# syzhang092218-source/dgppo

Hardware: AMD Instinct MI355X
Metric: env-steps/sec whole node, LidarSpread n=8 4096 envs, 1/2/4/8 GPUs (higher is better)
Workload: dtype f32

## Files before the change

dgppo_amd/csrc/nn_graph.hip:

```cpp
#include "common.h"

struct Topo {
  int n, ng, gs, os, per, lidar, spread;
  int S, Ns;
};

static Topo make_topo(const dgppo_env_cfg& c) {
  Topo t;
  t.n = c.n_agents; t.ng = c.n_goals; t.gs = cfg_goal_slots(c); t.os = cfg_obs_slots(c);
  t.lidar = cfg_is_lidar(c) ? 1 : 0; t.spread = cfg_is_spread(c) ? 1 : 0;
  t.per = t.os;
  t.S = t.n + t.gs + t.os;
  t.Ns = t.n + t.ng + cfg_obs_nodes(c);
  return t;
}

__device__ inline int sender_node(const Topo& t, int i, int s) {
  if (s < t.n) return s;
  if (s < t.n + t.gs) return t.spread ? t.n + (s - t.n) : t.n + i;
  const int m = s - t.n - t.gs;
  return t.lidar ? t.n + t.ng + i * t.per + m : t.n + t.ng + m;
}
__device__ inline int slot_of(const Topo& t, int nd, int i) {
  if (nd < t.n) return nd;
  if (nd < t.n + t.ng) {
    const int g = nd - t.n;
    return t.spread ? t.n + g : (g == i ? t.n : -1);
  }
  const int q = nd - t.n - t.ng;
  if (t.lidar) return (q / t.per == i) ? t.n + t.gs + (q - i * t.per) : -1;
  return t.n + t.gs + q;
}

struct FeatArgs {
  dgppo_env_cfg cfg;
  Topo t;
  const float* agent; long agent_se, agent_st;
  const float* goal;
  const float* obst;
  const float* hits; long hits_se, hits_st;
  const int32_t* env_ids;
  int n_env, n_time;
  float* Xa;
  float* Xo;
  float* efeat;
  float* emask;
  int Fp;
  uint32_t rcp_fp, rcp_S;
};

__device__ inline float dist_rn(float dx, float dy) { return __fsqrt_rn(__fadd_rn(__fmul_rn(dx, dx), __fmul_rn(dy, dy))); }

template <int SD>
__global__ void graph_feats_kernel(FeatArgs a) {
  extern __shared__ float sm[];
  const dgppo_env_cfg& c = a.cfg;
  const Topo& t = a.t;
  const int g = blockIdx.x;
  const int e = g / a.n_time, tt = g - e * a.n_time;
  const int env = a.env_ids ? a.env_ids[e] : e;
  const int tid = threadIdx.x, nt = blockDim.x;
  const int n = t.n, ng = t.ng, S = t.S, Fp = a.Fp;
  const int n_on = t.Ns - n - ng;
  float* s_ag = sm;
  float* s_go = s_ag + n * SD;
  float* s_ob = s_go + ng * SD;
  float* s_fa = s_ob + n_on * SD;
  float* s_fg = s_fa + n * 4;
  const float* ag = a.agent + (size_t)env * a.agent_se + (size_t)tt * a.agent_st;
  for (int i = tid; i < n * SD; i += nt) s_ag[i] = ag[i];
  for (int i = tid; i < ng * SD; i += nt) s_go[i] = a.goal[(size_t)env * ng * SD + i];
  if (n_on > 0) {
    if (t.lidar) {
      const float* hp = a.hits + (size_t)env * a.hits_se + (size_t)tt * a.hits_st;
      for (int i = tid; i < n_on * 2; i += nt) {
        const int q = i >> 1, d = i & 1;
        s_ob[q * SD + d] = hp[i];
      }
      for (int i = tid; i < n_on * (SD - 2); i += nt) {
        const int q = i / (SD - 2), d = i - q * (SD - 2);
        s_ob[q * SD + 2 + d] = 0.0f;
      }
    } else {
      for (int i = tid; i < n_on * SD; i += nt) s_ob[i] = a.obst[(size_t)env * n_on * SD + i];
    }
  }
  __syncthreads();
  for (int i = tid; i < n + ng; i += nt) {
    const float* s = (i < n) ? s_ag + i * SD : s_go + (i - n) * SD;
    float* f = (i < n) ? s_fa + i * 4 : s_fg + (i - n) * 4;
    if constexpr (SD == 5) {
      f[0] = s[0]; f[1] = s[1]; f[2] = __fmul_rn(s[4], s[2]); f[3] = __fmul_rn(s[4], s[3]);
    } else {
      f[0] = s[0]; f[1] = s[1]; f[2] = s[2]; f[3] = s[3];
    }
  }
  __syncthreads();
  constexpr int ND = SD + 3;
  for (int idx = tid; idx < t.Ns * Fp; idx += nt) {
    const int nd = (int)__umulhi((uint32_t)idx, a.rcp_fp), col = idx - nd * Fp;
    float v = 0.0f;
    if (nd < n) v = (col < SD) ? s_ag[nd * SD + col] : ((col == SD + 2) ? 1.0f : 0.0f);
    else if (nd < n + ng) v = (col < SD) ? s_go[(nd - n) * SD + col] : ((col == SD + 1) ? 1.0f : 0.0f);
    else v = (col < SD) ? s_ob[(nd - n - ng) * SD + col] : ((col == SD) ? 1.0f : 0.0f);
    if (col >= ND) v = 0.0f;
    if (nd < n) a.Xa[((size_t)g * n + nd) * Fp + col] = v;
    else a.Xo[((size_t)g * (t.Ns - n) + (nd - n)) * Fp + col] = v;
  }
  for (int idx = tid; idx < n * S; idx += nt) {
    const int i = (int)__umulhi((uint32_t)idx, a.rcp_S), s = idx - i * S;
    float4 f;
    bool mask;
    const float* fi = s_fa + i * 4;
    const float px = s_ag[i * SD], py = s_ag[i * SD + 1];
    if (s < n) {
      const float* fj = s_fa + s * 4;
      f = make_float4(__fsub_rn(fi[0], fj[0]), __fsub_rn(fi[1], fj[1]), __fsub_rn(fi[2], fj[2]), __fsub_rn(fi[3], fj[3]));
      float d = __fadd_rn(dist_rn(__fsub_rn(px, s_ag[s * SD]), __fsub_rn(py, s_ag[s * SD + 1])), (i == s) ? c.eye_offset : 0.0f);
      mask = d < c.comm_radius;
    } else if (s < n + t.gs) {
      const int gi = t.spread ? (s - n) : i;
      const float* fg = s_fg + gi * 4;
      f = make_float4(__fsub_rn(fi[0], fg[0]), __fsub_rn(fi[1], fg[1]), __fsub_rn(fi[2], fg[2]), __fsub_rn(fi[3], fg[3]));
      mask = true;
    } else {
      const int m = s - n - t.gs;
      if (t.lidar) {
        const float* hp = s_ob + (i * t.per + m) * SD;
        const float lx = __fsub_rn(px, hp[0]), ly = __fsub_rn(py, hp[1]);
        f = make_float4(lx, ly, 0.0f, 0.0f);
        mask = dist_rn(lx, ly) < c.lidar_mask_radius;
      } else {
        const float* xo = s_ob + m * SD;
        const float* xi = s_ag + i * SD;
        f = make_float4(__fsub_rn(xi[0], xo[0]), __fsub_rn(xi[1], xo[1]), __fsub_rn(xi[2], xo[2]), __fsub_rn(xi[3], xo[3]));
        mask = dist_rn(__fsub_rn(xi[0], xo[0]), __fsub_rn(xi[1], xo[1])) < c.obs_mask_radius;
      }
    }
    reinterpret_cast<float4*>(a.efeat)[(size_t)g * n * S + idx] = f;
    a.emask[(size_t)g * n * S + idx] = mask ? 1.0f : 0.0f;
  }
}

extern "C" int32_t dgppo_graph_feats(const dgppo_env_cfg* cfg, const float* agent, int64_t agent_se, int64_t agent_st,
                                     const float* goal, const float* obst, const float* hits, int64_t hits_se,
                                     int64_t hits_st, const int32_t* env_ids, int32_t n_env, int32_t n_time, float* Xa,
                                     float* Xo, float* efeat, float* emask, int32_t Fp, void* stream) {
  int32_t rc = dgppo_validate_cfg(cfg);
  if (rc) return rc;
  DGPPO_REQUIRE(n_env >= 0 && n_time >= 0, "graph_feats: negative counts");
  if (n_env == 0 || n_time == 0) return 0;
  DGPPO_REQUIRE(agent && goal && Xa && efeat && emask, "graph_feats: NULL operand");
  DGPPO_REQUIRE(Fp >= cfg->node_dim && Fp <= 32, "graph_feats: Fp must be in [node_dim, 32]");
  FeatArgs a;
  a.cfg = *cfg; a.t = make_topo(*cfg);
  const int n_on = a.t.Ns - a.t.n - a.t.ng;
  DGPPO_REQUIRE(n_on == 0 || Xo, "graph_feats: Xo is NULL");
  DGPPO_REQUIRE(a.t.Ns == a.t.n || Xo, "graph_feats: Xo is NULL");
  if (n_on > 0) {
    if (a.t.lidar) DGPPO_REQUIRE(hits, "graph_feats: hits is NULL");
    else DGPPO_REQUIRE(obst, "graph_feats: obst is NULL");
  }
  DGPPO_REQUIRE(((uintptr_t)efeat & 15) == 0, "graph_feats: efeat must be 16-byte aligned");
  a.agent = agent; a.agent_se = agent_se; a.agent_st = agent_st; a.goal = goal; a.obst = obst;
  a.hits = hits; a.hits_se = hits_se; a.hits_st = hits_st; a.env_ids = env_ids; a.n_env = n_env; a.n_time = n_time;
  a.Xa = Xa; a.Xo = Xo; a.efeat = efeat; a.emask = emask; a.Fp = Fp;
  a.rcp_fp = (uint32_t)((0x100000000ull + (uint64_t)Fp - 1) / (uint64_t)Fp);
  a.rcp_S = (uint32_t)((0x100000000ull + (uint64_t)a.t.S - 1) / (uint64_t)a.t.S);
  DGPPO_REQUIRE(Fp >= 2 && a.t.S >= 2 && (long)a.t.Ns * Fp < 65536 && (long)a.t.n * a.t.S < 65536, "graph_feats: sizes out of range");
  const int SD = cfg->state_dim;
  const size_t smem = sizeof(float) * ((size_t)a.t.n * SD + a.t.ng * SD + (size_t)n_on * SD + a.t.n * 4 + a.t.ng * 4);
  const long G = (long)n_env * n_time;
  if (SD == 5) hipLaunchKernelGGL(graph_feats_kernel<5>, dim3(G), dim3(128), smem, (hipStream_t)stream, a);
  else hipLaunchKernelGGL(graph_feats_kernel<4>, dim3(G), dim3(128), smem, (hipStream_t)stream, a);
  DGPPO_LAUNCH_CHECK();
  return 0;
}

struct AttnArgs {
  Topo t;
  int F, H, Kp;
  const float* qt;
  const float* Xa;
  const float* Xo;
  const float* efeat;
  const float* emask;
  float* zcat;
  float* attn;
  const float* dzcat;
  float* dqt;
  float* dXa;
  float* dXo;
  int relu_xo;
  int G;
  const float* Xo_raw; const float* Wo; const float* bo; int ldwo;
  float* dwo_slab;
};

__global__ void __launch_bounds__(256) attn_fwd_valu_kernel(AttnArgs a) {
  extern __shared__ float sm[];
  const Topo& t = a.t;
  const int g = blockIdx.x, tid = threadIdx.x, nt = blockDim.x;
  const int n = t.n, S = t.S, Ns = t.Ns, F = a.F, H = a.H, Fl = F + 1;
  float* s_x = sm;
  float* s_q = s_x + Ns * Fl;
  float* s_e = s_q + n * H * Fl;
  float* s_m = s_e + n * S * 4;
  float* s_a = s_m + n * S;
  for (int idx = tid; idx < Ns * F; idx += nt) {
    const int nd = idx / F, f = idx - nd * F;
    s_x[nd * Fl + f] = (nd < n) ? a.Xa[((size_t)g * n + nd) * F + f] : a.Xo[((size_t)g * (Ns - n) + (nd - n)) * F + f];
  }
  for (int idx = tid; idx < n * H * F; idx += nt) {
    const int ih = idx / F, f = idx - ih * F;
    s_q[ih * Fl + f] = a.qt[(size_t)g * n * H * F + idx];
  }
  for (int idx = tid; idx < n * S * 4; idx += nt) s_e[idx] = a.efeat[(size_t)g * n * S * 4 + idx];
  for (int idx = tid; idx < n * S; idx += nt) s_m[idx] = a.emask[(size_t)g * n * S + idx];
  __syncthreads();
  for (int idx = tid; idx < n * S * H; idx += nt) {
    const int h = idx % H, is = idx / H;
    const int i = is / S, s = is - i * S;
    const float* x = s_x + sender_node(t, i, s) * Fl;
    const float* q = s_q + (i * H + h) * Fl;
    float acc = 0.0f;
    for (int f = 0; f < F; ++f) acc = fmaf(q[f], x[f], acc);
    s_a[idx] = acc;
  }
  __syncthreads();
  for (int ih = tid; ih < n * H; ih += nt) {
    const int i = ih / H, h = ih - i * H;
    float mx = -INFINITY;
    for (int s = 0; s < S; ++s)
      if (s_m[i * S + s] != 0.0f) mx = fmaxf(mx, s_a[(i * S + s) * H + h]);
    float den = 0.0f;
    for (int s = 0; s < S; ++s) {
      float ev = 0.0f;
      if (s_m[i * S + s] != 0.0f) ev = expf(s_a[(i * S + s) * H + h] - mx);
      s_a[(i * S + s) * H + h] = ev;
      den += ev;
    }
    const float inv = (den > 0.0f) ? 1.0f / den : 0.0f;
    for (int s = 0; s < S; ++s) s_a[(i * S + s) * H + h] *= inv;
  }
  __syncthreads();
  if (a.attn != nullptr)
    for (int idx = tid; idx < n * S * H; idx += nt) a.attn[(size_t)g * n * S * H + idx] = s_a[idx];
  const int W = F + 4;
  for (int idx = tid; idx < n * H * W; idx += nt) {
    const int w = idx % W, ih = idx / W;
    const int i = ih / H, h = ih - i * H;
    float acc = 0.0f;
    if (w < F) {
      for (int s = 0; s < S; ++s) {
        const float av = s_a[(i * S + s) * H + h];
        if (av != 0.0f) acc = fmaf(av, s_x[sender_node(t, i, s) * Fl + w], acc);
      }
    } else {
      for (int s = 0; s < S; ++s) {
        const float av = s_a[(i * S + s) * H + h];
        if (av != 0.0f) acc = fmaf(av, s_e[(i * S + s) * 4 + (w - F)], acc);
      }
    }
    a.zcat[((size_t)g * n + i) * a.Kp + F + h * W + w] = acc;
  }
  for (int idx = tid; idx < n * F; idx += nt) {
    const int i = idx / F, f = idx - i * F;
    a.zcat[((size_t)g * n + i) * a.Kp + f] = s_x[i * Fl + f];
  }
  const int kc = F + H * W;
  for (int idx = tid; idx < n * (a.Kp - kc); idx += nt) {
    const int i = idx / (a.Kp - kc), c = kc + idx - i * (a.Kp - kc);
    a.zcat[((size_t)g * n + i) * a.Kp + c] = (c == kc) ? 1.0f : 0.0f;
  }
}

__global__ void __launch_bounds__(256) attn_bwd_valu_kernel(AttnArgs a) {
  extern __shared__ float sm[];
  const Topo& t = a.t;
  const int g = blockIdx.x, tid = threadIdx.x, nt = blockDim.x;
  const int n = t.n, S = t.S, Ns = t.Ns, F = a.F, H = a.H, Fl = F + 1, W = F + 4;
  float* s_x = sm;
  float* s_q = s_x + Ns * Fl;
  float* s_e = s_q + n * H * Fl;
  float* s_a = s_e + n * S * 4;
  float* s_d = s_a + n * S * H;
  float* s_z = s_d + n * S * H;
  const int Wl = W + 1;
  for (int idx = tid; idx < Ns * F; idx += nt) {
    const int nd = idx / F, f = idx - nd * F;
    s_x[nd * Fl + f] = (nd < n) ? a.Xa[((size_t)g * n + nd) * F + f] : a.Xo[((size_t)g * (Ns - n) + (nd - n)) * F + f];
  }
  for (int idx = tid; idx < n * H * F; idx += nt) {
    const int ih = idx / F, f = idx - ih * F;
    s_q[ih * Fl + f] = a.qt[(size_t)g * n * H * F + idx];
  }
  for (int idx = tid; idx < n * S * 4; idx += nt) s_e[idx] = a.efeat[(size_t)g * n * S * 4 + idx];
  for (int idx = tid; idx < n * S * H; idx += nt) s_a[idx] = a.attn[(size_t)g * n * S * H + idx];
  for (int idx = tid; idx < n * H * W; idx += nt) {
    const int w = idx % W, ih = idx / W;
    const int i = ih / H, h = ih - i * H;
    s_z[ih * Wl + w] = a.dzcat[((size_t)g * n + i) * a.Kp + F + h * W + w];
  }
  __syncthreads();
  for (int idx = tid; idx < n * S * H; idx += nt) {
    const int h = idx % H, is = idx / H;
    const int i = is / S, s = is - i * S;
    float acc = 0.0f;
    if (s_a[idx] != 0.0f) {
      const float* x = s_x + sender_node(t, i, s) * Fl;
      const float* dz = s_z + (i * H + h) * Wl;
      for (int f = 0; f < F; ++f) acc = fmaf(dz[f], x[f], acc);
      for (int c = 0; c < 4; ++c) acc = fmaf(dz[F + c], s_e[is * 4 + c], acc);
    }
    s_d[idx] = acc;
  }
  __syncthreads();
  for (int ih = tid; ih < n * H; ih += nt) {
    const int i = ih / H, h = ih - i * H;
    float dot = 0.0f;
    for (int s = 0; s < S; ++s) dot = fmaf(s_a[(i * S + s) * H + h], s_d[(i * S + s) * H + h], dot);
    for (int s = 0; s < S; ++s) {
      const int k = (i * S + s) * H + h;
      s_d[k] = s_a[k] * (s_d[k] - dot);
    }
  }
  __syncthreads();
  for (int idx = tid; idx < n * H * F; idx += nt) {
    const int f = idx % F, ih = idx / F;
    const int i = ih / H, h = ih - i * H;
    float acc = 0.0f;
    for (int s = 0; s < S; ++s) {
      const float dv = s_d[(i * S + s) * H + h];
      if (dv != 0.0f) acc = fmaf(dv, s_x[sender_node(t, i, s) * Fl + f], acc);
    }
    a.dqt[(size_t)g * n * H * F + idx] = acc;
  }
  if (a.dXa != nullptr) {
    for (int idx = tid; idx < Ns * F; idx += nt) {
      const int nd = idx / F, f = idx - nd * F;
      if (nd >= n && a.dXo == nullptr) continue;
      float acc = 0.0f;
      for (int i = 0; i < n; ++i) {
        const int s = slot_of(t, nd, i);
        if (s < 0) continue;
        for (int h = 0; h < H; ++h) {
          const int k = (i * S + s) * H + h;
          acc = fmaf(s_a[k], s_z[(i * H + h) * Wl + f], acc);
          acc = fmaf(s_d[k], s_q[(i * H + h) * Fl + f], acc);
        }
      }
      if (nd < n) a.dXa[((size_t)g * n + nd) * F + f] = acc + a.dzcat[((size_t)g * n + nd) * a.Kp + f];
      else a.dXo[((size_t)g * (Ns - n) + (nd - n)) * F + f] = acc;
    }
  }
}


using f32x4g = __attribute__((ext_vector_type(4))) float;
#ifdef DGPPO_STAMPS
__device__ unsigned long long g_astamps[32];
#define ASTAMP(i) do { if (blockIdx.x == 0 && threadIdx.x == 0) g_astamps[i] = __builtin_amdgcn_s_memtime(); } while (0)
extern "C" int32_t dgppo_debug_stamps_attn(unsigned long long* out) {
  return (int32_t)hipMemcpyFromSymbol(out, HIP_SYMBOL(g_astamps), sizeof(unsigned long long) * 32);
}
#else
#define ASTAMP(i)
#endif

struct AttnDims {
  int n, H, F, S, Ns, nH, RT, CT, Fl, Ll, W;
};
__host__ __device__ inline AttnDims attn_dims(const Topo& t, int F, int H) {
  AttnDims d;
  d.n = t.n; d.H = H; d.F = F; d.S = t.S; d.Ns = t.Ns; d.nH = t.n * H;
  d.RT = (d.nH + 15) / 16; d.CT = (d.Ns + 15) / 16;
  d.Fl = F + 1; d.Ll = d.CT * 16 + 1; d.W = (t.S > 32) ? 64 : 32;
  return d;
}
static size_t attn_mfma_smem(const AttnDims& d, bool bwd) {
  size_t fl = (size_t)d.CT * 16 * d.Fl
              + (size_t)d.RT * 16 * d.Fl
              + (size_t)d.RT * 16 * d.Ll
              + 8 + (size_t)d.n * d.S * 5
              + 2 * (size_t)d.nH * ((d.S + 3) & ~3);
  if (bwd) fl += (size_t)d.RT * 16 * d.Ll
                 + (size_t)d.RT * 16 * (d.F + 5);
  return fl * sizeof(float);
}

__device__ inline float red_max(float v, int W) {
  for (int o = W >> 1; o >= 1; o >>= 1) v = fmaxf(v, __shfl_xor(v, o, W));
  return v;
}
__device__ inline float red_sum(float v, int W) {
  for (int o = W >> 1; o >= 1; o >>= 1) v += __shfl_xor(v, o, W);
  return v;
}

template <typename FA, typename FB, typename FC>
__device__ inline void mfma_tiles(int RTn, int CTn, int K4, int wave, int lane, FA fa, FB fb, FC fc) {
  const int li = lane & 15, lq = lane >> 4;
  for (int tile = wave; tile < RTn * CTn; tile += 4) {
    const int rt = tile / CTn, ct = tile - rt * CTn;
    f32x4g acc = {0.f, 0.f, 0.f, 0.f};
    int k4 = 0;
    for (; k4 + 4 <= K4; k4 += 4) {
      float av[4], bv[4];
#pragma unroll
      for (int u = 0; u < 4; ++u) { av[u] = fa(rt * 16 + li, (k4 + u) * 4 + lq); bv[u] = fb((k4 + u) * 4 + lq, ct * 16 + li); }
#pragma unroll
      for (int u = 0; u < 4; ++u) acc = __builtin_amdgcn_mfma_f32_16x16x4f32(av[u], bv[u], acc, 0, 0, 0);
    }
    for (; k4 < K4; ++k4) acc = __builtin_amdgcn_mfma_f32_16x16x4f32(fa(rt * 16 + li, k4 * 4 + lq), fb(k4 * 4 + lq, ct * 16 + li), acc, 0, 0, 0);
#pragma unroll
    for (int r = 0; r < 4; ++r) fc(rt * 16 + lq * 4 + r, ct * 16 + li, acc[r]);
  }
}


template <int MAXIT, typename FL, typename FP>
__device__ inline void stage4(int count4, int tid, FL load, FP put) {
  float4 v[MAXIT];
#pragma unroll
  for (int it = 0; it < MAXIT; ++it) {
    const int idx = tid + it * 256;
    v[it] = (idx < count4) ? load(idx) : make_float4(0.f, 0.f, 0.f, 0.f);
  }
#pragma unroll
  for (int it = 0; it < MAXIT; ++it) {
    const int idx = tid + it * 256;
    if (idx < count4) put(idx, v[it]);
  }
  for (int idx = tid + MAXIT * 256; idx < count4; idx += 256) put(idx, load(idx));
}
__device__ inline void put4(float* d, float4 v) { d[0] = v.x; d[1] = v.y; d[2] = v.z; d[3] = v.w; }

#define ATT_SMAX 64

__global__ void __launch_bounds__(256) attn_fwd_kernel(AttnArgs a) {
  extern __shared__ float sm[];
  const Topo& t = a.t;
  const AttnDims d = attn_dims(t, a.F, a.H);
  const int g = blockIdx.x, tid = threadIdx.x, lane = tid & 63, wave = tid >> 6;
  const int n = d.n, S = d.S, Ns = d.Ns, F = d.F, H = d.H, Fl = d.Fl, Ll = d.Ll, nH = d.nH;
  const int Sp = (S + 3) & ~3;
  float* s_x = sm;
  float* s_q = s_x + d.CT * 16 * Fl;
  float* s_L = s_q + d.RT * 16 * Fl;
  float* s_e = sm + (((d.CT * 16 * Fl + d.RT * 16 * Fl + d.RT * 16 * Ll) + 3) & ~3);
  float* s_m = s_e + n * S * 4;
  float* s_a = s_m + n * S;
  ASTAMP(0);
  {
    const int F4 = F >> 2;
    const float4* xa = reinterpret_cast<const float4*>(a.Xa + (size_t)g * n * F);
    const float4* xo = reinterpret_cast<const float4*>(a.Xo + (size_t)g * (Ns - n) * F);
    const float4* q4 = reinterpret_cast<const float4*>(a.qt + (size_t)g * nH * F);
    const float4* e4 = reinterpret_cast<const float4*>(a.efeat + (size_t)g * n * S * 4);
    const float* mk = a.emask + (size_t)g * n * S;
    const int nA = n * F4, nX = Ns * F4, nXp = d.CT * 16 * F4, nQ = nH * F4, nQp = d.RT * 16 * F4, nE = n * S;
    float4 vx[4], vq[2], ve[2];
    float vm[2];
    const float4 z4 = make_float4(0.f, 0.f, 0.f, 0.f);
#pragma unroll
    for (int it = 0; it < 4; ++it) { const int idx = tid + it * 256; vx[it] = (idx < nA) ? xa[idx] : ((idx < nX) ? xo[idx - nA] : z4); }
#pragma unroll
    for (int it = 0; it < 2; ++it) { const int idx = tid + it * 256; vq[it] = (idx < nQ) ? q4[idx] : z4; ve[it] = (idx < nE) ? e4[idx] : z4; vm[it] = (idx < nE) ? mk[idx] : 0.0f; }
#pragma unroll
    for (int it = 0; it < 4; ++it) { const int idx = tid + it * 256; if (idx < nXp) { const int nd = idx / F4, q = idx - nd * F4; put4(s_x + nd * Fl + 4 * q, vx[it]); } }
#pragma unroll
    for (int it = 0; it < 2; ++it) {
      const int idx = tid + it * 256;
      if (idx < nQp) { const int row = idx / F4, q = idx - row * F4; put4(s_q + row * Fl + 4 * q, vq[it]); }
      if (idx < nE) { const float4 ev = ve[it]; reinterpret_cast<float4*>(s_e)[idx] = make_float4(ev.x, ev.y, ev.z, ev.w); s_m[idx] = vm[it]; }
    }
    for (int idx = tid + 1024; idx < nXp; idx += 256) { const int nd = idx / F4, q = idx - nd * F4; put4(s_x + nd * Fl + 4 * q, (idx < nA) ? xa[idx] : ((idx < nX) ? xo[idx - nA] : z4)); }
    for (int idx = tid + 512; idx < nQp; idx += 256) { const int row = idx / F4, q = idx - row * F4; put4(s_q + row * Fl + 4 * q, (idx < nQ) ? q4[idx] : z4); }
    for (int idx = tid + 512; idx < nE; idx += 256) { reinterpret_cast<float4*>(s_e)[idx] = e4[idx]; s_m[idx] = mk[idx]; }
  }
  __syncthreads();
  ASTAMP(1);
  mfma_tiles(d.RT, d.CT, F / 4, wave, lane,
             [&](int row, int k) { return s_q[row * Fl + k]; },
             [&](int k, int col) { return s_x[col * Fl + k]; },
             [&](int row, int col, float v) { s_L[row * Ll + col] = v; });
  __syncthreads();
  ASTAMP(2);
  for (int idx = tid; idx < nH * Sp; idx += 256) {
    const int pair = idx / Sp, s = idx - pair * Sp, i = pair / H;
    float l = -INFINITY;
    if (s < S && s_m[i * S + s] != 0.0f) l = s_L[pair * Ll + sender_node(t, i, s)];
    s_a[idx] = l;
  }
  __syncthreads();
  ASTAMP(3);
  const int Wd = F + 4;
  float* zc = a.zcat + (size_t)g * n * a.Kp;
  for (int p0 = 0; p0 < nH; p0 += 32) {
    const int pair = p0 + (tid >> 3), sub = tid & 7;
    const bool live = pair < nH;
    const int i = live ? pair / H : 0, h = live ? pair - (pair / H) * H : 0;
    float l[ATT_SMAX / 8];
    float mx = -INFINITY;
#pragma unroll
    for (int j = 0; j < ATT_SMAX / 8; ++j) {
      const int sl = sub + 8 * j;
      l[j] = (live && sl < S) ? s_a[pair * Sp + sl] : -INFINITY;
      mx = fmaxf(mx, l[j]);
    }
    mx = fmaxf(mx, __shfl_xor(mx, 1, 8)); mx = fmaxf(mx, __shfl_xor(mx, 2, 8)); mx = fmaxf(mx, __shfl_xor(mx, 4, 8));
    float den = 0.0f;
#pragma unroll
    for (int j = 0; j < ATT_SMAX / 8; ++j) {
      if (sub + 8 * j < S) { const float ev = (l[j] == -INFINITY) ? 0.0f : expf(l[j] - mx); l[j] = ev; den += ev; }
    }
    den += __shfl_xor(den, 1, 8); den += __shfl_xor(den, 2, 8); den += __shfl_xor(den, 4, 8);
    const float inv = (den > 0.0f) ? 1.0f / den : 0.0f;
    float z0 = 0.f, z1 = 0.f, z2 = 0.f, z3 = 0.f;
#pragma unroll
    for (int j = 0; j < ATT_SMAX / 8; ++j) {
      const int sl = sub + 8 * j;
      if (live && sl < S) {
        const float av = l[j] * inv;
        s_a[pair * Sp + sl] = av;
        if (av != 0.0f) {
          const float4 e = reinterpret_cast<const float4*>(s_e)[i * S + sl];
          z0 = fmaf(av, e.x, z0); z1 = fmaf(av, e.y, z1); z2 = fmaf(av, e.z, z2); z3 = fmaf(av, e.w, z3);
        }
      }
    }
#pragma unroll
    for (int o = 1; o < 8; o <<= 1) { z0 += __shfl_xor(z0, o, 8); z1 += __shfl_xor(z1, o, 8); z2 += __shfl_xor(z2, o, 8); z3 += __shfl_xor(z3, o, 8); }
    if (live && sub == 0) *reinterpret_cast<float4*>(zc + i * a.Kp + F + h * Wd + F) = make_float4(z0, z1, z2, z3);
  }
  for (int idx = tid; idx < d.RT * 16 * Ll; idx += 256) s_L[idx] = 0.0f;
  __syncthreads();
  ASTAMP(4);
  for (int idx = tid; idx < n * S * H; idx += 256) {
    const int h = idx % H, is = idx / H, i = is / S, s = is - i * S;
    const float av = s_a[(i * H + h) * Sp + s];
    if (a.attn != nullptr) a.attn[(size_t)g * n * S * H + idx] = av;
    if (av != 0.0f) s_L[(i * H + h) * Ll + sender_node(t, i, s)] = av;
  }
  __syncthreads();
  ASTAMP(5);
  mfma_tiles(d.RT, (F + 15) / 16, d.CT * 4, wave, lane,
             [&](int row, int k) { return s_L[row * Ll + k]; },
             [&](int k, int col) { return (col < F) ? s_x[k * Fl + col] : 0.0f; },
             [&](int row, int col, float v) {
               if (row < nH && col < F) { const int i = row / H, h = row - i * H; zc[i * a.Kp + F + h * Wd + col] = v; }
             });
  for (int idx = tid; idx < n * F; idx += 256) {
    const int i = idx / F, f = idx - i * F;
    zc[i * a.Kp + f] = s_x[i * Fl + f];
  }
  const int kc = F + H * Wd;
  for (int idx = tid; idx < n * (a.Kp - kc); idx += 256) {
    const int i = idx / (a.Kp - kc), c = kc + idx - i * (a.Kp - kc);
    zc[i * a.Kp + c] = (c == kc) ? 1.0f : 0.0f;
  }
  ASTAMP(6);
}

template <int CTRL> __device__ inline float dpp_f(float v) {
  return __int_as_float(__builtin_amdgcn_update_dpp(0, __float_as_int(v), CTRL, 0xf, 0xf, false));
}
__device__ inline float grp8_sum(float v) {
  v += dpp_f<0xB1>(v);
  v += dpp_f<0x4E>(v);
  v += dpp_f<0x141>(v);
  return v;
}
__device__ inline float grp8_max(float v) {
  v = fmaxf(v, dpp_f<0xB1>(v));
  v = fmaxf(v, dpp_f<0x4E>(v));
  v = fmaxf(v, dpp_f<0x141>(v));
  return v;
}

template <int H, int NPA, int SJ>
__global__ void __launch_bounds__(256) attn_fwd_slot8_kernel(AttnArgs a) {
  constexpr int F = 8, Wd = F + 4;
  const Topo& t = a.t;
  const int lane = threadIdx.x & 63, wave = threadIdx.x >> 6, sub = lane & 7, grp = lane >> 3;
  const int g = __builtin_amdgcn_readfirstlane(blockIdx.x * 4 + wave);
  if (g >= a.G) return;
  const int n = t.n, S = t.S, Ns = t.Ns, Kp = a.Kp, kc = F + H * Wd;
  const float* Xa = a.Xa + (size_t)g * n * F;
  const float* Xo = a.Xo + (size_t)g * (Ns - n) * F - (size_t)n * F;
  const float* qt = a.qt + (size_t)g * n * H * F;
  const float* ef = a.efeat + (size_t)g * n * S * 4;
  const float* mk = a.emask + (size_t)g * n * S;
  float* zc = a.zcat + (size_t)g * n * Kp;
  float* at = a.attn + (size_t)g * n * S * H;
  for (int idx = lane; idx < n * 2; idx += 64)
    *reinterpret_cast<float4*>(zc + (idx >> 1) * Kp + 4 * (idx & 1)) = reinterpret_cast<const float4*>(Xa)[idx];
  for (int i = lane; i < n; i += 64)
    for (int c = kc; c < Kp; ++c) zc[i * Kp + c] = (c == kc) ? 1.0f : 0.0f;
#pragma unroll
  for (int p = 0; p < NPA; ++p) {
    const int ia = grp + 8 * p;
    const bool live = ia < n;
    const int i = live ? ia : n - 1;
    float4 q[H][2], x[SJ][2], e[SJ];
    float m[SJ];
#pragma unroll
    for (int h = 0; h < H; ++h) {
      const float4* qp = reinterpret_cast<const float4*>(qt + (i * H + h) * F);
      q[h][0] = qp[0]; q[h][1] = qp[1];
    }
#pragma unroll
    for (int j = 0; j < SJ; ++j) {
      int sl = sub + 8 * j;
      sl = sl < S ? sl : S - 1;
      const int nd = sender_node(t, i, sl);
      const float4* xp = reinterpret_cast<const float4*>((nd < n ? Xa : Xo) + (size_t)nd * F);
      x[j][0] = xp[0]; x[j][1] = xp[1];
      e[j] = reinterpret_cast<const float4*>(ef)[i * S + sl];
      m[j] = mk[i * S + sl];
    }
    float av[SJ][H];
#pragma unroll
    for (int h = 0; h < H; ++h) {
      float mx = -INFINITY;
#pragma unroll
      for (int j = 0; j < SJ; ++j) {
        const bool ok = live && (sub + 8 * j) < S && m[j] != 0.0f;
        float acc = q[h][0].x * x[j][0].x;
        acc = fmaf(q[h][0].y, x[j][0].y, acc); acc = fmaf(q[h][0].z, x[j][0].z, acc); acc = fmaf(q[h][0].w, x[j][0].w, acc);
        acc = fmaf(q[h][1].x, x[j][1].x, acc); acc = fmaf(q[h][1].y, x[j][1].y, acc);
        acc = fmaf(q[h][1].z, x[j][1].z, acc); acc = fmaf(q[h][1].w, x[j][1].w, acc);
        av[j][h] = ok ? acc : -INFINITY;
        mx = fmaxf(mx, av[j][h]);
      }
      mx = grp8_max(mx);
      float den = 0.0f;
#pragma unroll
      for (int j = 0; j < SJ; ++j) {
        const float ev = (av[j][h] == -INFINITY) ? 0.0f : __expf(av[j][h] - mx);
        av[j][h] = ev;
        den += ev;
      }
      den = grp8_sum(den);
      const float inv = (den > 0.0f) ? 1.0f / den : 0.0f;
#pragma unroll
      for (int j = 0; j < SJ; ++j) av[j][h] *= inv;
    }
#pragma unroll
    for (int j = 0; j < SJ; ++j) {
      const int sl = sub + 8 * j;
      if (live && sl < S) {
#pragma unroll
        for (int h = 0; h < H; ++h) if (a.attn != nullptr) at[(i * S + sl) * H + h] = av[j][h];
      }
    }
#pragma unroll
    for (int h = 0; h < H; ++h) {
      float z[Wd];
#pragma unroll
      for (int c = 0; c < Wd; ++c) z[c] = 0.0f;
#pragma unroll
      for (int j = 0; j < SJ; ++j) {
        const float w = av[j][h];
        if (w != 0.0f) {
          z[0] = fmaf(w, x[j][0].x, z[0]); z[1] = fmaf(w, x[j][0].y, z[1]); z[2] = fmaf(w, x[j][0].z, z[2]); z[3] = fmaf(w, x[j][0].w, z[3]);
          z[4] = fmaf(w, x[j][1].x, z[4]); z[5] = fmaf(w, x[j][1].y, z[5]); z[6] = fmaf(w, x[j][1].z, z[6]); z[7] = fmaf(w, x[j][1].w, z[7]);
          z[8] = fmaf(w, e[j].x, z[8]); z[9] = fmaf(w, e[j].y, z[9]); z[10] = fmaf(w, e[j].z, z[10]); z[11] = fmaf(w, e[j].w, z[11]);
        }
      }
#pragma unroll
      for (int c = 0; c < Wd; ++c) z[c] = grp8_sum(z[c]);
      if (live && sub == h) {
        float4* o = reinterpret_cast<float4*>(zc + i * Kp + F + h * Wd);
        o[0] = make_float4(z[0], z[1], z[2], z[3]);
        o[1] = make_float4(z[4], z[5], z[6], z[7]);
        o[2] = make_float4(z[8], z[9], z[10], z[11]);
      }
    }
  }
}

template <int H, int NPA, int SJ>
__global__ void __launch_bounds__(256) attn_bwd_slot8_kernel(AttnArgs a) {
  constexpr int F = 8, Wd = F + 4;
  const Topo& t = a.t;
  const int lane = threadIdx.x & 63, wave = threadIdx.x >> 6, sub = lane & 7, grp = lane >> 3;
  const int g = __builtin_amdgcn_readfirstlane(blockIdx.x * 4 + wave);
  if (g >= a.G) return;
  const int n = t.n, S = t.S, Ns = t.Ns, Kp = a.Kp;
  const float* Xa = a.Xa + (size_t)g * n * F;
  const float* Xo = a.Xo + (size_t)g * (Ns - n) * F - (size_t)n * F;
  const float* ef = a.efeat + (size_t)g * n * S * 4;
  const float* at = a.attn + (size_t)g * n * S * H;
  const float* dzc = a.dzcat + (size_t)g * n * Kp;
  float* dq = a.dqt + (size_t)g * n * H * F;
#pragma unroll
  for (int p = 0; p < NPA; ++p) {
    const int ia = grp + 8 * p;
    const bool live = ia < n;
    const int i = live ? ia : n - 1;
    float4 dz[H][3], x[SJ][2], e[SJ];
    float av[SJ][H];
#pragma unroll
    for (int h = 0; h < H; ++h) {
      const float4* zp = reinterpret_cast<const float4*>(dzc + i * Kp + F + h * Wd);
      dz[h][0] = zp[0]; dz[h][1] = zp[1]; dz[h][2] = zp[2];
    }
#pragma unroll
    for (int j = 0; j < SJ; ++j) {
      int sl = sub + 8 * j;
      const bool in = live && sl < S;
      sl = sl < S ? sl : S - 1;
      const int nd = sender_node(t, i, sl);
      const float4* xp = reinterpret_cast<const float4*>((nd < n ? Xa : Xo) + (size_t)nd * F);
      x[j][0] = xp[0]; x[j][1] = xp[1];
      e[j] = reinterpret_cast<const float4*>(ef)[i * S + sl];
#pragma unroll
      for (int h = 0; h < H; ++h) {
        const float w = at[(i * S + sl) * H + h];
        av[j][h] = in ? w : 0.0f;
      }
    }
#pragma unroll
    for (int h = 0; h < H; ++h) {
      float dA[SJ];
      float dot = 0.0f;
#pragma unroll
      for (int j = 0; j < SJ; ++j) {
        float acc = 0.0f;
        if (av[j][h] != 0.0f) {
          acc = dz[h][0].x * x[j][0].x;
          acc = fmaf(dz[h][0].y, x[j][0].y, acc); acc = fmaf(dz[h][0].z, x[j][0].z, acc); acc = fmaf(dz[h][0].w, x[j][0].w, acc);
          acc = fmaf(dz[h][1].x, x[j][1].x, acc); acc = fmaf(dz[h][1].y, x[j][1].y, acc);
          acc = fmaf(dz[h][1].z, x[j][1].z, acc); acc = fmaf(dz[h][1].w, x[j][1].w, acc);
          acc = fmaf(dz[h][2].x, e[j].x, acc); acc = fmaf(dz[h][2].y, e[j].y, acc);
          acc = fmaf(dz[h][2].z, e[j].z, acc); acc = fmaf(dz[h][2].w, e[j].w, acc);
          dot = fmaf(av[j][h], acc, dot);
        }
        dA[j] = acc;
      }
      dot = grp8_sum(dot);
      float o[F];
#pragma unroll
      for (int c = 0; c < F; ++c) o[c] = 0.0f;
#pragma unroll
      for (int j = 0; j < SJ; ++j) {
        if (av[j][h] != 0.0f) {
          const float dl = av[j][h] * (dA[j] - dot);
          o[0] = fmaf(dl, x[j][0].x, o[0]); o[1] = fmaf(dl, x[j][0].y, o[1]); o[2] = fmaf(dl, x[j][0].z, o[2]); o[3] = fmaf(dl, x[j][0].w, o[3]);
          o[4] = fmaf(dl, x[j][1].x, o[4]); o[5] = fmaf(dl, x[j][1].y, o[5]); o[6] = fmaf(dl, x[j][1].z, o[6]); o[7] = fmaf(dl, x[j][1].w, o[7]);
        }
      }
#pragma unroll
      for (int c = 0; c < F; ++c) o[c] = grp8_sum(o[c]);
      if (live && sub == h) {
        float4* op = reinterpret_cast<float4*>(dq + (i * H + h) * F);
        op[0] = make_float4(o[0], o[1], o[2], o[3]);
        op[1] = make_float4(o[4], o[5], o[6], o[7]);
      }
    }
  }
}

template <int H, int NPA>
static bool launch_attn_slot8_sj(const AttnArgs& a, int SJ, int grid, hipStream_t s, bool bwd) {
#define DGPPO_SJ(J)                                                                                              \
  case J:                                                                                                        \
    if (bwd) hipLaunchKernelGGL((attn_bwd_slot8_kernel<H, NPA, J>), dim3(grid), dim3(256), 0, s, a);             \
    else hipLaunchKernelGGL((attn_fwd_slot8_kernel<H, NPA, J>), dim3(grid), dim3(256), 0, s, a);                 \
    return true;
  switch (SJ) {
    DGPPO_SJ(1) DGPPO_SJ(2) DGPPO_SJ(3) DGPPO_SJ(4) DGPPO_SJ(5) DGPPO_SJ(6) DGPPO_SJ(7) DGPPO_SJ(8)
    default: return false;
  }
#undef DGPPO_SJ
}
static bool attn_slot8_shape(const Topo& t, int F, int H) { return F == 8 && H == 3 && t.n <= 32 && t.S <= 64; }
static bool launch_attn_slot8(const AttnArgs& a, hipStream_t s, bool bwd) {
  if (!attn_slot8_shape(a.t, a.F, a.H)) return false;
  const int grid = (a.G + 3) / 4, NPA = (a.t.n + 7) / 8, SJ = (a.t.S + 7) / 8;
  switch (NPA) {
    case 1: return launch_attn_slot8_sj<3, 1>(a, SJ, grid, s, bwd);
    case 2: return launch_attn_slot8_sj<3, 2>(a, SJ, grid, s, bwd);
    case 3: return launch_attn_slot8_sj<3, 3>(a, SJ, grid, s, bwd);
    case 4: return launch_attn_slot8_sj<3, 4>(a, SJ, grid, s, bwd);
    default: return false;
  }
}

#define ABD_XL 36
#define ABD_DZL 40
typedef float4 abd_f4;
__device__ inline f32x4g mfma4(float a_, float b_, f32x4g c_) { return __builtin_amdgcn_mfma_f32_4x4x1f32(a_, b_, c_, 0, 0, 0); }
__device__ inline const float* f4e(const float4& v) { return reinterpret_cast<const float*>(&v); }
__device__ inline float4 ld4_if(bool ok, const float4* p) {
  float4 v = make_float4(0.f, 0.f, 0.f, 0.f);
  if (ok) v = *p;
  return v;
}

__device__ inline int opaque_zero(int bits) {
  asm("v_and_b32 %0, 0, %0" : "+v"(bits));
  return bits;
}
__device__ inline int f4bits(const float4& v) { return __float_as_int(v.x) | __float_as_int(v.y) | __float_as_int(v.z) | __float_as_int(v.w); }

template <int PS, bool HITS> struct AbdLds {
  static constexpr int NSP = PS * 8, PC = NSP + (HITS ? 8 : 0), PL = PC + 4;
  static constexpr int XS = NSP * ABD_XL, XH = HITS ? 64 * ABD_XL + 64 : 0;
  static constexpr int QP = (32 * ABD_XL > 32 * PL) ? 32 * ABD_XL : 32 * PL;
  static constexpr int FWD = XS + XH + QP;
  static constexpr int DZ = 32 * ABD_DZL, PTL = NSP + 1, PT = 32 * PTL, DL = 32 * PL;
  static constexpr int BWD = XS + XH + DZ + PT + DL;
};

#define ABD_KR 8
#define ABD_DW_STRIDE 320
template <int GT> struct AbdXoRegs { float ag[GT][2], ah[4][2], wo[2][2], bo[2]; };
template <int GT, bool HITS>
__device__ inline void abd_xo_load(AbdXoRegs<GT>& x, const AttnArgs& a, const float* raw, int n_shared_other, int ng, int hit0,
                                   int n_hits, int li, int lq, bool first) {
  if (first) {
#pragma unroll
    for (int s_ = 0; s_ < 2; ++s_)
#pragma unroll
      for (int ct = 0; ct < 2; ++ct) x.wo[s_][ct] = a.Wo[(lq + 4 * s_) * a.ldwo + ct * 16 + li];
#pragma unroll
    for (int ct = 0; ct < 2; ++ct) x.bo[ct] = a.bo[ct * 16 + li];
#pragma unroll
    for (int t = 0; t < GT; ++t) {
      int o = t * 16 + li;
      o = o < n_shared_other ? o : n_shared_other - 1;
      o = o < 0 ? 0 : o;
#pragma unroll
      for (int s_ = 0; s_ < 2; ++s_) x.ag[t][s_] = raw[o * ABD_KR + lq + 4 * s_];
    }
  }
  if constexpr (HITS) {
#pragma unroll
    for (int t = 0; t < 4; ++t) {
      int hb = hit0 + t * 16 + li;
      hb = hb < n_hits ? hb : n_hits - 1;
#pragma unroll
      for (int s_ = 0; s_ < 2; ++s_) x.ah[t][s_] = raw[(ng + hb) * ABD_KR + lq + 4 * s_];
    }
  }
}
template <int GT, bool HITS>
__device__ inline void abd_xo_emit(const AbdXoRegs<GT>& x, float* XS, float* XH, int n, int n_shared_other, int li, int lq, bool first) {
  auto tile = [&](const float (&ar)[2], f32x4g (&v)[2]) {
#pragma unroll
    for (int ct = 0; ct < 2; ++ct) {
      v[ct] = f32x4g{0.f, 0.f, 0.f, 0.f};
      v[ct] = __builtin_amdgcn_mfma_f32_16x16x4f32(ar[0], x.wo[0][ct], v[ct], 0, 0, 0);
      v[ct] = __builtin_amdgcn_mfma_f32_16x16x4f32(ar[1], x.wo[1][ct], v[ct], 0, 0, 0);
    }
  };
  if (first) {
#pragma unroll
    for (int t = 0; t < GT; ++t) {
      f32x4g v[2];
      tile(x.ag[t], v);
#pragma unroll
      for (int ct = 0; ct < 2; ++ct)
#pragma unroll
        for (int r = 0; r < 4; ++r) {
          const int o = t * 16 + lq * 4 + r;
          if (o < n_shared_other) XS[(n + o) * ABD_XL + ct * 16 + li] = fmaxf(v[ct][r] + x.bo[ct], 0.0f);
        }
    }
  }
  if constexpr (HITS) {
#pragma unroll
    for (int t = 0; t < 4; ++t) {
      f32x4g v[2];
      tile(x.ah[t], v);
#pragma unroll
      for (int ct = 0; ct < 2; ++ct)
#pragma unroll
        for (int r = 0; r < 4; ++r) {
          const int hr = t * 16 + lq * 4 + r;
          XH[hr * ABD_XL + (hr >> 3) * 8 + ct * 16 + li] = fmaxf(v[ct][r] + x.bo[ct], 0.0f);
        }
    }
  }
}
template <int GT> __device__ inline int abd_xo_bits(const AbdXoRegs<GT>& x, bool hits) {
  int b = 0;
#pragma unroll
  for (int t = 0; t < GT; ++t) b |= __float_as_int(x.ag[t][0]) | __float_as_int(x.ag[t][1]);
  if (hits) {
#pragma unroll
    for (int t = 0; t < 4; ++t) b |= __float_as_int(x.ah[t][0]) | __float_as_int(x.ah[t][1]);
  }
  b |= __float_as_int(x.wo[0][0]) | __float_as_int(x.wo[0][1]) | __float_as_int(x.wo[1][0]) | __float_as_int(x.wo[1][1]);
  b |= __float_as_int(x.bo[0]) | __float_as_int(x.bo[1]);
  return b;
}

template <int PS, bool HITS, int AB, bool XOF>
__global__ void __launch_bounds__(128) attn_fwd_bd_kernel(AttnArgs a) {
  extern __shared__ float4 abd_sm[];
  using L = AbdLds<PS, HITS>;
  constexpr int F = 32, NSP = L::NSP, PC = L::PC, PL = L::PL, NPR = PS + (HITS ? 1 : 0), Wd = F + 4;
  const Topo& t = a.t;
  const int lane = threadIdx.x & 63, wave = threadIdx.x >> 6;
  const int g = __builtin_amdgcn_readfirstlane(blockIdx.x * 2 + wave);
  if (g >= a.G) return;
  const int n = t.n, S = t.S, Ns = t.Ns, H = a.H, Kp = a.Kp;
  const int NSH = HITS ? t.n + t.ng : Ns;
  const int kc = F + H * Wd;
  float* XS = reinterpret_cast<float*>(abd_sm) + wave * L::FWD;
  float* XH = XS + L::XS;
  float* QP = XH + L::XH;
  const float4* Xa4 = reinterpret_cast<const float4*>(a.Xa + (size_t)g * n * F);
  const float4* Xo4 = reinterpret_cast<const float4*>(a.Xo + (size_t)g * (Ns - n) * F);
  const float4* qt4 = reinterpret_cast<const float4*>(a.qt + (size_t)g * n * H * F);
  float* zc = a.zcat + (size_t)g * n * Kp;
  const int il = lane >> 3, sub = lane & 7, g2 = (lane >> 2) & 1, c = lane & 3, hA = lane & 3;
  ASTAMP(0);
  float4 vs[PS];
#pragma unroll
  for (int p = 0; p < PS; ++p) {
    const int row = p * 8 + il;
    const int ra = row < n ? row : n - 1, ro = (row < NSH ? row : NSH - 1) - n;
    const float4* src = (XOF || row < n || NSH == n) ? Xa4 + ra * 8 + sub : Xo4 + ro * 8 + sub;
    vs[p] = *src;
  }
  constexpr int GT = (NSP + 15) / 16;
  AbdXoRegs<GT> xo;
  const float* raw = XOF ? a.Xo_raw + (size_t)g * (Ns - n) * ABD_KR : nullptr;
  const int li_ = lane & 15, lq_ = lane >> 4;
  const float* mk = a.emask + (size_t)g * n * S;
  const float4* ef4 = reinterpret_cast<const float4*>(a.efeat + (size_t)g * n * S * 4);
  float* at = a.attn + (size_t)g * n * S * H;
#pragma unroll
  for (int ab = 0; ab < AB; ++ab) {
    const int i = ab * 8 + il;
    const bool live = i < n;
    const int ic = live ? i : n - 1;
    float4 vh[HITS ? 8 : 1], vq[4];
    if constexpr (XOF) abd_xo_load<GT, HITS>(xo, a, raw, NSH - n, t.ng, ab * 64, n * 8, li_, lq_, ab == 0);
    if constexpr (HITS && !XOF) {
#pragma unroll
      for (int k = 0; k < 8; ++k) {
        int hb = ab * 64 + k * 8 + il;
        hb = hb < n * 8 ? hb : n * 8 - 1;
        vh[k] = Xo4[(t.ng + hb) * 8 + sub];
      }
    }
#pragma unroll
    for (int k = 0; k < 4; ++k) {
      const int row = k * 8 + il;
      int ri = ab * 8 + (row >> 2), rh = row & 3;
      ri = ri < n ? ri : n - 1; rh = rh < H ? rh : H - 1;
      vq[k] = qt4[(ri * H + rh) * 8 + sub];
    }
    int slot[NPR];
    float mkv[NPR];
    float4 efv[NPR];
#pragma unroll
    for (int p = 0; p < NPR; ++p) {
      int sl;
      if (HITS && p == PS) sl = n + t.gs + sub;
      else { const int j = p * 8 + sub; sl = (j < NSH) ? slot_of(t, j, ic) : -1; }
      slot[p] = live ? sl : -1;
      const int sc = sl < 0 ? 0 : sl;
      mkv[p] = mk[ic * S + sc];
      efv[p] = ef4[ic * S + sc];
    }
    ASTAMP(1);
    int pin = 0;
#pragma unroll
    for (int p = 0; p < NPR; ++p) pin |= __float_as_int(mkv[p]) | f4bits(efv[p]);
    if constexpr (XOF) pin |= abd_xo_bits<GT>(xo, HITS);
    const int pin0 = opaque_zero(pin);
    if (ab == 0) {
#pragma unroll
      for (int p = 0; p < PS; ++p) {
        float4 v = vs[p];
        if (XOF && p * 8 + il >= n) v = make_float4(0.f, 0.f, 0.f, 0.f);
        *reinterpret_cast<float4*>(XS + pin0 + (p * 8 + il) * ABD_XL + sub * 4) = v;
      }
    }
    if constexpr (XOF) abd_xo_emit<GT, HITS>(xo, XS + pin0, XH + pin0, n, NSH - n, li_, lq_, ab == 0);
    if constexpr (HITS && !XOF) {
#pragma unroll
      for (int k = 0; k < 8; ++k) *reinterpret_cast<float4*>(XH + pin0 + (k * 8 + il) * ABD_XL + k * 8 + sub * 4) = vh[k];
    }
#pragma unroll
    for (int k = 0; k < 4; ++k) *reinterpret_cast<float4*>(QP + pin0 + (k * 8 + il) * ABD_XL + sub * 4) = vq[k];
#pragma unroll
    for (int p = 0; p < NPR; ++p) mkv[p] = (slot[p] >= 0) ? mkv[p] : 0.0f;
    ASTAMP(2);
    f32x4g acc[NPR];
#pragma unroll
    for (int p = 0; p < NPR; ++p) acc[p] = f32x4g{0.f, 0.f, 0.f, 0.f};
    {
      const float* qrow = QP + (il * 4 + hA) * ABD_XL;
#pragma unroll
      for (int k = 0; k < 8; ++k) {
        const float4 q = *reinterpret_cast<const float4*>(qrow + k * 4);
        float4 x[NPR];
#pragma unroll
        for (int p = 0; p < NPR; ++p) {
          if (HITS && p == PS) x[p] = *reinterpret_cast<const float4*>(XH + lane * ABD_XL + il * 8 + k * 4);
          else x[p] = *reinterpret_cast<const float4*>(XS + (p * 8 + sub) * ABD_XL + k * 4);
        }
#pragma unroll
        for (int u = 0; u < 4; ++u)
#pragma unroll
          for (int p = 0; p < NPR; ++p) acc[p] = mfma4(f4e(q)[u], f4e(x[p])[u], acc[p]);
      }
    }
    ASTAMP(3);
    float* PT = QP;
#pragma unroll
    for (int h = 0; h < 4; ++h) {
      if (h < H) {
        float l[NPR];
        float mx = -INFINITY;
#pragma unroll
        for (int p = 0; p < NPR; ++p) { l[p] = (mkv[p] != 0.0f) ? acc[p][h] : -INFINITY; mx = fmaxf(mx, l[p]); }
        mx = grp8_max(mx);
        float den = 0.0f;
#pragma unroll
        for (int p = 0; p < NPR; ++p) { l[p] = (l[p] == -INFINITY) ? 0.0f : __expf(l[p] - mx); den += l[p]; }
        den = grp8_sum(den);
        const float inv = (den > 0.0f) ? 1.0f / den : 0.0f;
        float z0 = 0.f, z1 = 0.f, z2 = 0.f, z3 = 0.f;
#pragma unroll
        for (int p = 0; p < NPR; ++p) {
          const float av = l[p] * inv;
          acc[p][h] = av;
          if (slot[p] >= 0) {
            if (a.attn != nullptr) at[(i * S + slot[p]) * H + h] = av;
            if (av != 0.0f) {
              const float4 e = efv[p];
              z0 = fmaf(av, e.x, z0); z1 = fmaf(av, e.y, z1); z2 = fmaf(av, e.z, z2); z3 = fmaf(av, e.w, z3);
            }
          }
        }
        z0 = grp8_sum(z0); z1 = grp8_sum(z1); z2 = grp8_sum(z2); z3 = grp8_sum(z3);
        if (live && sub == 0) *reinterpret_cast<float4*>(zc + i * Kp + F + h * Wd + F) = make_float4(z0, z1, z2, z3);
      } else {
#pragma unroll
        for (int p = 0; p < NPR; ++p) acc[p][h] = 0.0f;
      }
#pragma unroll
      for (int p = 0; p < NPR; ++p) PT[(il * 4 + h) * PL + p * 8 + sub] = acc[p][h];
    }
    ASTAMP(4);
    {
      float pa[PC];
#pragma unroll
      for (int k = 0; k < PC / 4; ++k) {
        const float4 v = *reinterpret_cast<const float4*>(PT + (il * 4 + hA) * PL + k * 4);
        pa[k * 4] = v.x; pa[k * 4 + 1] = v.y; pa[k * 4 + 2] = v.z; pa[k * 4 + 3] = v.w;
      }
      f32x4g az[4];
#pragma unroll
      for (int q = 0; q < 4; ++q) az[q] = f32x4g{0.f, 0.f, 0.f, 0.f};
      const int fq = (g2 * 4 + c) * 4;
#pragma unroll
      for (int kk = 0; kk < NSP; ++kk) {
        const float4 b = *reinterpret_cast<const float4*>(XS + kk * ABD_XL + fq);
#pragma unroll
        for (int q = 0; q < 4; ++q) az[q] = mfma4(pa[kk], f4e(b)[q], az[q]);
      }
      if constexpr (HITS) {
#pragma unroll
        for (int m = 0; m < 8; ++m) {
          const float4 b = *reinterpret_cast<const float4*>(XH + (il * 8 + m) * ABD_XL + il * 8 + fq);
#pragma unroll
          for (int q = 0; q < 4; ++q) az[q] = mfma4(pa[NSP + m], f4e(b)[q], az[q]);
        }
      }
      if (live) {
#pragma unroll
        for (int h = 0; h < 4; ++h)
          if (h < H) *reinterpret_cast<float4*>(zc + i * Kp + F + h * Wd + fq) = make_float4(az[0][h], az[1][h], az[2][h], az[3][h]);
      }
    }
  }
  ASTAMP(5);
#pragma unroll
  for (int p = 0; p < PS; ++p) {
    const int row = p * 8 + il;
    if (row < n) *reinterpret_cast<float4*>(zc + row * Kp + sub * 4) = *reinterpret_cast<const float4*>(XS + row * ABD_XL + sub * 4);
  }
  {
    const int wpad = Kp - kc;
    for (int i = lane; i < n; i += 64)
      for (int cc = 0; cc < wpad; ++cc) zc[i * Kp + kc + cc] = (cc == 0) ? 1.0f : 0.0f;
  }
  ASTAMP(6);
}

template <int PS, bool HITS, bool XOF>
struct AbdFwdRegs {
  float4 vs[PS], vq[4], vh[(HITS && !XOF) ? 8 : 1];
  AbdXoRegs<(PS * 8 + 15) / 16> xo;
  float mkv[PS + (HITS ? 1 : 0)];
  float4 efv[PS + (HITS ? 1 : 0)];
};
template <int PS, bool HITS, bool XOF>
__global__ void __launch_bounds__(128) attn_fwd_bdp_kernel(AttnArgs a) {
  extern __shared__ float4 abd_sm[];
  using L = AbdLds<PS, HITS>;
  constexpr int F = 32, NSP = L::NSP, PC = L::PC, PL = L::PL, NPR = PS + (HITS ? 1 : 0), Wd = F + 4, GT = (NSP + 15) / 16;
  const Topo& t = a.t;
  const int lane = threadIdx.x & 63, wave = threadIdx.x >> 6;
  int g = __builtin_amdgcn_readfirstlane(blockIdx.x * 2 + wave);
  const int stride = gridDim.x * 2;
  if (g >= a.G) return;
  const int n = t.n, S = t.S, Ns = t.Ns, H = a.H, Kp = a.Kp;
  const int NSH = HITS ? t.n + t.ng : Ns;
  const int kc = F + H * Wd;
  float* XS = reinterpret_cast<float*>(abd_sm) + wave * L::FWD;
  float* XH = XS + L::XS;
  float* QP = XH + L::XH;
  const int il = lane >> 3, sub = lane & 7, g2 = (lane >> 2) & 1, c = lane & 3, hA = lane & 3;
  const int li_ = lane & 15, lq_ = lane >> 4;
  const int i = il;
  const bool live = i < n;
  const int ic = live ? i : n - 1;
  int slot[NPR], sc[NPR];
#pragma unroll
  for (int p = 0; p < NPR; ++p) {
    int sl;
    if (HITS && p == PS) sl = n + t.gs + sub;
    else { const int j = p * 8 + sub; sl = (j < NSH) ? slot_of(t, j, ic) : -1; }
    slot[p] = live ? sl : -1;
    sc[p] = sl < 0 ? 0 : sl;
  }
  using Regs = AbdFwdRegs<PS, HITS, XOF>;
  auto load = [&](int gg, Regs& R) {
    const float4* Xa4 = reinterpret_cast<const float4*>(a.Xa + (size_t)gg * n * F);
    const float4* Xo4 = reinterpret_cast<const float4*>(a.Xo + (size_t)gg * (Ns - n) * F);
    const float4* qt4 = reinterpret_cast<const float4*>(a.qt + (size_t)gg * n * H * F);
#pragma unroll
    for (int p = 0; p < PS; ++p) {
      const int row = p * 8 + il;
      const int ra = row < n ? row : n - 1, ro = (row < NSH ? row : NSH - 1) - n;
      const float4* src = (XOF || row < n || NSH == n) ? Xa4 + ra * 8 + sub : Xo4 + ro * 8 + sub;
      R.vs[p] = *src;
    }
    if constexpr (XOF) abd_xo_load<GT, HITS>(R.xo, a, a.Xo_raw + (size_t)gg * (Ns - n) * ABD_KR, NSH - n, t.ng, 0, n * 8, li_, lq_, true);
    if constexpr (HITS && !XOF) {
#pragma unroll
      for (int k = 0; k < 8; ++k) {
        int hb = k * 8 + il;
        hb = hb < n * 8 ? hb : n * 8 - 1;
        R.vh[k] = Xo4[(t.ng + hb) * 8 + sub];
      }
    }
#pragma unroll
    for (int k = 0; k < 4; ++k) {
      const int row = k * 8 + il;
      int ri = row >> 2, rh = row & 3;
      ri = ri < n ? ri : n - 1; rh = rh < H ? rh : H - 1;
      R.vq[k] = qt4[(ri * H + rh) * 8 + sub];
    }
    const float* mk = a.emask + (size_t)gg * n * S;
    const float4* ef4 = reinterpret_cast<const float4*>(a.efeat + (size_t)gg * n * S * 4);
#pragma unroll
    for (int p = 0; p < NPR; ++p) {
      R.mkv[p] = mk[ic * S + sc[p]];
      R.efv[p] = ef4[ic * S + sc[p]];
    }
  };
  auto stage = [&](Regs& R) {
    int pin = 0;
#pragma unroll
    for (int p = 0; p < NPR; ++p) pin |= __float_as_int(R.mkv[p]) | f4bits(R.efv[p]);
    if constexpr (XOF) pin |= abd_xo_bits<GT>(R.xo, HITS);
    const int pin0 = opaque_zero(pin);
#pragma unroll
    for (int p = 0; p < PS; ++p) {
      float4 v = R.vs[p];
      if (XOF && p * 8 + il >= n) v = make_float4(0.f, 0.f, 0.f, 0.f);
      *reinterpret_cast<float4*>(XS + pin0 + (p * 8 + il) * ABD_XL + sub * 4) = v;
    }
    if constexpr (XOF) abd_xo_emit<GT, HITS>(R.xo, XS + pin0, XH + pin0, n, NSH - n, li_, lq_, true);
    if constexpr (HITS && !XOF) {
#pragma unroll
      for (int k = 0; k < 8; ++k) *reinterpret_cast<float4*>(XH + pin0 + (k * 8 + il) * ABD_XL + k * 8 + sub * 4) = R.vh[k];
    }
#pragma unroll
    for (int k = 0; k < 4; ++k) *reinterpret_cast<float4*>(QP + pin0 + (k * 8 + il) * ABD_XL + sub * 4) = R.vq[k];
#pragma unroll
    for (int p = 0; p < NPR; ++p) R.mkv[p] = (slot[p] >= 0) ? R.mkv[p] : 0.0f;
  };
  auto compute = [&](int gg, const Regs& R) {
    float* zc = a.zcat + (size_t)gg * n * Kp;
    float* at = a.attn + (size_t)gg * n * S * H;
    f32x4g acc[NPR];
#pragma unroll
    for (int p = 0; p < NPR; ++p) acc[p] = f32x4g{0.f, 0.f, 0.f, 0.f};
    {
      const float* qrow = QP + (il * 4 + hA) * ABD_XL;
#pragma unroll
      for (int k = 0; k < 8; ++k) {
        const float4 q = *reinterpret_cast<const float4*>(qrow + k * 4);
        float4 x[NPR];
#pragma unroll
        for (int p = 0; p < NPR; ++p) {
          if (HITS && p == PS) x[p] = *reinterpret_cast<const float4*>(XH + lane * ABD_XL + il * 8 + k * 4);
          else x[p] = *reinterpret_cast<const float4*>(XS + (p * 8 + sub) * ABD_XL + k * 4);
        }
#pragma unroll
        for (int u = 0; u < 4; ++u)
#pragma unroll
          for (int p = 0; p < NPR; ++p) acc[p] = mfma4(f4e(q)[u], f4e(x[p])[u], acc[p]);
      }
    }
    float* PT = QP;
#pragma unroll
    for (int h = 0; h < 4; ++h) {
      if (h < H) {
        float l[NPR];
        float mx = -INFINITY;
#pragma unroll
        for (int p = 0; p < NPR; ++p) { l[p] = (R.mkv[p] != 0.0f) ? acc[p][h] : -INFINITY; mx = fmaxf(mx, l[p]); }
        mx = grp8_max(mx);
        float den = 0.0f;
#pragma unroll
        for (int p = 0; p < NPR; ++p) { l[p] = (l[p] == -INFINITY) ? 0.0f : __expf(l[p] - mx); den += l[p]; }
        den = grp8_sum(den);
        const float inv = (den > 0.0f) ? 1.0f / den : 0.0f;
        float z0 = 0.f, z1 = 0.f, z2 = 0.f, z3 = 0.f;
#pragma unroll
        for (int p = 0; p < NPR; ++p) {
          const float av = l[p] * inv;
          acc[p][h] = av;
          if (slot[p] >= 0) {
            if (a.attn != nullptr) at[(i * S + slot[p]) * H + h] = av;
            if (av != 0.0f) {
              const float4 e = R.efv[p];
              z0 = fmaf(av, e.x, z0); z1 = fmaf(av, e.y, z1); z2 = fmaf(av, e.z, z2); z3 = fmaf(av, e.w, z3);
            }
          }
        }
        z0 = grp8_sum(z0); z1 = grp8_sum(z1); z2 = grp8_sum(z2); z3 = grp8_sum(z3);
        if (live && sub == 0) *reinterpret_cast<float4*>(zc + i * Kp + F + h * Wd + F) = make_float4(z0, z1, z2, z3);
      } else {
#pragma unroll
        for (int p = 0; p < NPR; ++p) acc[p][h] = 0.0f;
      }
#pragma unroll
      for (int p = 0; p < NPR; ++p) PT[(il * 4 + h) * PL + p * 8 + sub] = acc[p][h];
    }
    {
      float pa[PC];
#pragma unroll
      for (int k = 0; k < PC / 4; ++k) {
        const float4 v = *reinterpret_cast<const float4*>(PT + (il * 4 + hA) * PL + k * 4);
        pa[k * 4] = v.x; pa[k * 4 + 1] = v.y; pa[k * 4 + 2] = v.z; pa[k * 4 + 3] = v.w;
      }
      f32x4g az[4];
#pragma unroll
      for (int q = 0; q < 4; ++q) az[q] = f32x4g{0.f, 0.f, 0.f, 0.f};
      const int fq = (g2 * 4 + c) * 4;
#pragma unroll
      for (int kk = 0; kk < NSP; ++kk) {
        const float4 b = *reinterpret_cast<const float4*>(XS + kk * ABD_XL + fq);
#pragma unroll
        for (int q = 0; q < 4; ++q) az[q] = mfma4(pa[kk], f4e(b)[q], az[q]);
      }
      if constexpr (HITS) {
#pragma unroll
        for (int m = 0; m < 8; ++m) {
          const float4 b = *reinterpret_cast<const float4*>(XH + (il * 8 + m) * ABD_XL + il * 8 + fq);
#pragma unroll
          for (int q = 0; q < 4; ++q) az[q] = mfma4(pa[NSP + m], f4e(b)[q], az[q]);
        }
      }
      if (live) {
#pragma unroll
        for (int h = 0; h < 4; ++h)
          if (h < H) *reinterpret_cast<float4*>(zc + i * Kp + F + h * Wd + fq) = make_float4(az[0][h], az[1][h], az[2][h], az[3][h]);
      }
    }
#pragma unroll
    for (int p = 0; p < PS; ++p) {
      const int row = p * 8 + il;
      if (row < n) *reinterpret_cast<float4*>(zc + row * Kp + sub * 4) = *reinterpret_cast<const float4*>(XS + row * ABD_XL + sub * 4);
    }
    {
      const int wpad = Kp - kc;
      for (int ii = lane; ii < n; ii += 64)
        for (int cc = 0; cc < wpad; ++cc) zc[ii * Kp + kc + cc] = (cc == 0) ? 1.0f : 0.0f;
    }
  };
  Regs cur;
  load(g, cur);
  for (;;) {
    stage(cur);
    const int gn = g + stride;
    const bool more = gn < a.G;
    Regs nxt;
    if (more) load(gn, nxt);
    compute(g, cur);
    if (!more) break;
    cur = nxt;
    g = gn;
  }
}

template <int PS, bool HITS, int AB, bool XOF>
__global__ void __launch_bounds__(64) attn_bwd_bd_kernel(AttnArgs a) {
  extern __shared__ float4 abd_sm[];
  using L = AbdLds<PS, HITS>;
  constexpr int F = 32, NSP = L::NSP, PC = L::PC, PL = L::PL, PTL = L::PTL, NPR = PS + (HITS ? 1 : 0), Wd = F + 4;
  constexpr int RTS = (NSP + 15) / 16;
  const Topo& t = a.t;
  const int lane = threadIdx.x & 63;
  const int g = blockIdx.x;
  if (g >= a.G) return;
  const int n = t.n, S = t.S, Ns = t.Ns, H = a.H, Kp = a.Kp;
  const int NSH = HITS ? t.n + t.ng : Ns;
  float* XS = reinterpret_cast<float*>(abd_sm);
  float* XH = XS + L::XS;
  float* DZ = XH + L::XH;
  float* PT = DZ + L::DZ;
  float* DL = PT + L::PT;
  const float4* Xa4 = reinterpret_cast<const float4*>(a.Xa + (size_t)g * n * F);
  const float4* Xo4 = reinterpret_cast<const float4*>(a.Xo + (size_t)g * (Ns - n) * F);
  const float* qt = a.qt + (size_t)g * n * H * F;
  const float* dzc = a.dzcat + (size_t)g * n * Kp;
  const bool want_dx = a.dXa != nullptr;
  const int il = lane >> 3, sub = lane & 7, g2 = (lane >> 2) & 1, c = lane & 3, hA = lane & 3;
  const int li = lane & 15, lq = lane >> 4;
  float4 vs[PS];
#pragma unroll
  for (int p = 0; p < PS; ++p) {
    const int row = p * 8 + il;
    const int ra = row < n ? row : n - 1, ro = (row < NSH ? row : NSH - 1) - n;
    const float4* src = (XOF || row < n || NSH == n) ? Xa4 + ra * 8 + sub : Xo4 + ro * 8 + sub;
    vs[p] = *src;
  }
  constexpr int GT = (NSP + 15) / 16;
  AbdXoRegs<GT> xo;
  const float* raw = XOF ? a.Xo_raw + (size_t)g * (Ns - n) * ABD_KR : nullptr;
  const int li_ = lane & 15, lq_ = lane >> 4;
  float dir[RTS][2][4];
#pragma unroll
  for (int rt = 0; rt < RTS; ++rt)
#pragma unroll
    for (int ft = 0; ft < 2; ++ft)
#pragma unroll
      for (int r = 0; r < 4; ++r) {
        const int node = rt * 16 + lq * 4 + r;
        dir[rt][ft][r] = dzc[(node < n ? node : n - 1) * Kp + ft * 16 + li];
      }
  f32x4g dxs[RTS][2];
#pragma unroll
  for (int rt = 0; rt < RTS; ++rt)
#pragma unroll
    for (int ft = 0; ft < 2; ++ft) dxs[rt][ft] = f32x4g{0.f, 0.f, 0.f, 0.f};
  f32x4g dwacc[2] = {f32x4g{0.f, 0.f, 0.f, 0.f}, f32x4g{0.f, 0.f, 0.f, 0.f}};
  float rbg[NSP / 4];
  const float4* ef4 = reinterpret_cast<const float4*>(a.efeat + (size_t)g * n * S * 4);
  const float* at = a.attn + (size_t)g * n * S * H;
#pragma unroll
  for (int ab = 0; ab < AB; ++ab) {
    const int i = ab * 8 + il;
    const bool live = i < n;
    const int ic = live ? i : n - 1;
    float4 vh[HITS ? 8 : 1], vz[5];
    if constexpr (XOF) abd_xo_load<GT, HITS>(xo, a, raw, NSH - n, t.ng, ab * 64, n * 8, li_, lq_, ab == 0);
    float rbh[HITS ? 16 : 1];
    if constexpr (XOF && HITS) {
#pragma unroll
      for (int s_ = 0; s_ < 16; ++s_) {
        int hb = ab * 64 + s_ * 4 + lq;
        hb = hb < n * 8 ? hb : n * 8 - 1;
        rbh[s_] = raw[(t.ng + hb) * ABD_KR + (li & 7)];
      }
    }
    if constexpr (XOF) {
      if (ab == 0) {
#pragma unroll
        for (int s_ = 0; s_ < NSP / 4; ++s_) {
          int o = s_ * 4 + lq;
          o = o < NSH - n ? o : NSH - n - 1;
          o = o < 0 ? 0 : o;
          rbg[s_] = raw[o * ABD_KR + (li & 7)];
        }
      }
    }
    if constexpr (HITS && !XOF) {
#pragma unroll
      for (int k = 0; k < 8; ++k) {
        int hb = ab * 64 + k * 8 + il;
        hb = hb < n * 8 ? hb : n * 8 - 1;
        vh[k] = Xo4[(t.ng + hb) * 8 + sub];
      }
    }
#pragma unroll
    for (int k = 0; k < 5; ++k) {
      int tt = k * 64 + lane;
      tt = tt < 288 ? tt : 287;
      const int row = tt / 9, ch = tt - row * 9;
      int ri = ab * 8 + (row >> 2), rh = row & 3;
      ri = ri < n ? ri : n - 1; rh = rh < H ? rh : H - 1;
      vz[k] = *reinterpret_cast<const float4*>(dzc + ri * Kp + F + rh * Wd + ch * 4);
    }
    int slot[NPR];
    float4 efv[NPR];
    float av[NPR][4];
#pragma unroll
    for (int p = 0; p < NPR; ++p) {
      int sl;
      if (HITS && p == PS) sl = n + t.gs + sub;
      else { const int j = p * 8 + sub; sl = (j < NSH) ? slot_of(t, j, ic) : -1; }
      slot[p] = live ? sl : -1;
      const int sc = sl < 0 ? 0 : sl;
      efv[p] = ef4[ic * S + sc];
#pragma unroll
      for (int h = 0; h < 4; ++h) av[p][h] = at[(ic * S + sc) * H + (h < H ? h : H - 1)];
    }
    float4 q8[4][2];
    if constexpr (HITS) {
#pragma unroll
      for (int h = 0; h < 4; ++h) {
        const float4* qr = reinterpret_cast<const float4*>(qt + (size_t)(ic * H + (h < H ? h : H - 1)) * F + c * 8);
        q8[h][0] = qr[0]; q8[h][1] = qr[1];
      }
    }
    float bQ[8][2];
#pragma unroll
    for (int ks = 0; ks < 8; ++ks) {
      const int ri = ab * 8 + ks;
      const float* qr = qt + (size_t)((ri < n ? ri : n - 1) * H + (lq < H ? lq : H - 1)) * F;
#pragma unroll
      for (int ft = 0; ft < 2; ++ft) bQ[ks][ft] = qr[ft * 16 + li];
    }
    int pin = 0;
#pragma unroll
    for (int p = 0; p < NPR; ++p) {
      pin |= f4bits(efv[p]);
#pragma unroll
      for (int h = 0; h < 4; ++h) pin |= __float_as_int(av[p][h]);
    }
    if constexpr (HITS) {
#pragma unroll
      for (int h = 0; h < 4; ++h) pin |= f4bits(q8[h][0]) | f4bits(q8[h][1]);
    }
#pragma unroll
    for (int ks = 0; ks < 8; ++ks) pin |= __float_as_int(bQ[ks][0]) | __float_as_int(bQ[ks][1]);
    if (ab == 0) {
#pragma unroll
      for (int rt = 0; rt < RTS; ++rt)
#pragma unroll
        for (int ft = 0; ft < 2; ++ft)
#pragma unroll
          for (int r = 0; r < 4; ++r) pin |= __float_as_int(dir[rt][ft][r]);
    }
    if constexpr (XOF) pin |= abd_xo_bits<GT>(xo, HITS);
    if constexpr (XOF && HITS) {
#pragma unroll
      for (int s_ = 0; s_ < 16; ++s_) pin |= __float_as_int(rbh[s_]);
    }
    if constexpr (XOF) {
      if (ab == 0) {
#pragma unroll
        for (int s_ = 0; s_ < NSP / 4; ++s_) pin |= __float_as_int(rbg[s_]);
      }
    }
    const int pin0 = opaque_zero(pin);
    if (ab == 0) {
#pragma unroll
      for (int p = 0; p < PS; ++p) {
        float4 v = vs[p];
        if (XOF && p * 8 + il >= n) v = make_float4(0.f, 0.f, 0.f, 0.f);
        *reinterpret_cast<float4*>(XS + pin0 + (p * 8 + il) * ABD_XL + sub * 4) = v;
      }
    }
    if constexpr (XOF) abd_xo_emit<GT, HITS>(xo, XS + pin0, XH + pin0, n, NSH - n, li_, lq_, ab == 0);
    if constexpr (HITS && !XOF) {
#pragma unroll
      for (int k = 0; k < 8; ++k) *reinterpret_cast<float4*>(XH + pin0 + (k * 8 + il) * ABD_XL + k * 8 + sub * 4) = vh[k];
    }
#pragma unroll
    for (int k = 0; k < 5; ++k) {
      const int tt = k * 64 + lane, row = tt / 9, ch = tt - row * 9;
      if (tt < 288) *reinterpret_cast<float4*>(DZ + pin0 + row * ABD_DZL + ch * 4) = vz[k];
    }
#pragma unroll
    for (int p = 0; p < NPR; ++p)
#pragma unroll
      for (int h = 0; h < 4; ++h) av[p][h] = (slot[p] >= 0 && h < H) ? av[p][h] : 0.0f;
    f32x4g acc[NPR];
#pragma unroll
    for (int p = 0; p < NPR; ++p) acc[p] = f32x4g{0.f, 0.f, 0.f, 0.f};
    {
      const float* zrow = DZ + (il * 4 + hA) * ABD_DZL;
#pragma unroll
      for (int k = 0; k < 8; ++k) {
        const float4 q = *reinterpret_cast<const float4*>(zrow + k * 4);
        float4 x[NPR];
#pragma unroll
        for (int p = 0; p < NPR; ++p) {
          if (HITS && p == PS) x[p] = *reinterpret_cast<const float4*>(XH + lane * ABD_XL + il * 8 + k * 4);
          else x[p] = *reinterpret_cast<const float4*>(XS + (p * 8 + sub) * ABD_XL + k * 4);
        }
#pragma unroll
        for (int u = 0; u < 4; ++u)
#pragma unroll
          for (int p = 0; p < NPR; ++p) acc[p] = mfma4(f4e(q)[u], f4e(x[p])[u], acc[p]);
      }
    }
#pragma unroll
    for (int h = 0; h < 4; ++h) {
      const float4 dze = *reinterpret_cast<const float4*>(DZ + (il * 4 + h) * ABD_DZL + F);
      float dot = 0.0f;
#pragma unroll
      for (int p = 0; p < NPR; ++p) {
        const float w = av[p][h];
        const float4 e = efv[p];
        const float dA = (w != 0.0f) ? acc[p][h] + fmaf(dze.x, e.x, fmaf(dze.y, e.y, fmaf(dze.z, e.z, dze.w * e.w))) : 0.0f;
        acc[p][h] = dA;
        dot = fmaf(w, dA, dot);
      }
      dot = grp8_sum(dot);
#pragma unroll
      for (int p = 0; p < NPR; ++p) {
        acc[p][h] = av[p][h] * (acc[p][h] - dot);
        DL[(il * 4 + h) * PL + p * 8 + sub] = acc[p][h];
        if (p < PS) PT[(il * 4 + h) * PTL + p * 8 + sub] = av[p][h];
      }
    }
    {
      float pa[PC];
#pragma unroll
      for (int k = 0; k < PC / 4; ++k) {
        const float4 v = *reinterpret_cast<const float4*>(DL + (il * 4 + hA) * PL + k * 4);
        pa[k * 4] = v.x; pa[k * 4 + 1] = v.y; pa[k * 4 + 2] = v.z; pa[k * 4 + 3] = v.w;
      }
      f32x4g az[4];
#pragma unroll
      for (int q = 0; q < 4; ++q) az[q] = f32x4g{0.f, 0.f, 0.f, 0.f};
      const int fq = (g2 * 4 + c) * 4;
#pragma unroll
      for (int kk = 0; kk < NSP; ++kk) {
        const float4 b = *reinterpret_cast<const float4*>(XS + kk * ABD_XL + fq);
#pragma unroll
        for (int q = 0; q < 4; ++q) az[q] = mfma4(pa[kk], f4e(b)[q], az[q]);
      }
      if constexpr (HITS) {
#pragma unroll
        for (int m = 0; m < 8; ++m) {
          const float4 b = *reinterpret_cast<const float4*>(XH + (il * 8 + m) * ABD_XL + il * 8 + fq);
#pragma unroll
          for (int q = 0; q < 4; ++q) az[q] = mfma4(pa[NSP + m], f4e(b)[q], az[q]);
        }
      }
      if (live) {
        float* dq = a.dqt + ((size_t)g * n + i) * H * F;
#pragma unroll
        for (int h = 0; h < 4; ++h)
          if (h < H) *reinterpret_cast<float4*>(dq + h * F + fq) = make_float4(az[0][h], az[1][h], az[2][h], az[3][h]);
      }
    }
    if (want_dx) {
#pragma unroll
      for (int ks = 0; ks < 8; ++ks) {
        const int prow = ks * 4 + lq;
        float bD[2];
#pragma unroll
        for (int ft = 0; ft < 2; ++ft) bD[ft] = DZ[prow * ABD_DZL + ft * 16 + li];
#pragma unroll
        for (int rt = 0; rt < RTS; ++rt) {
          const int col = (rt * 16 + li < NSP) ? rt * 16 + li : NSP - 1;
          const float aP = PT[prow * PTL + col], aL = DL[prow * PL + col];
#pragma unroll
          for (int ft = 0; ft < 2; ++ft) {
            dxs[rt][ft] = __builtin_amdgcn_mfma_f32_16x16x4f32(aP, bD[ft], dxs[rt][ft], 0, 0, 0);
            dxs[rt][ft] = __builtin_amdgcn_mfma_f32_16x16x4f32(aL, bQ[ks][ft], dxs[rt][ft], 0, 0, 0);
          }
        }
      }
      if constexpr (HITS) {
        if (a.dXo != nullptr || (XOF && a.dwo_slab != nullptr)) {
          f32x4g af[8];
#pragma unroll
          for (int q = 0; q < 8; ++q) af[q] = f32x4g{0.f, 0.f, 0.f, 0.f};
#pragma unroll
          for (int h = 0; h < 4; ++h) {
            const float4 d0 = *reinterpret_cast<const float4*>(DZ + (il * 4 + h) * ABD_DZL + c * 8);
            const float4 d1 = *reinterpret_cast<const float4*>(DZ + (il * 4 + h) * ABD_DZL + c * 8 + 4);
            const float pw = av[PS][h], dw = acc[PS][h];
#pragma unroll
            for (int q = 0; q < 4; ++q) {
              af[q] = mfma4(pw, f4e(d0)[q], af[q]);
              af[q + 4] = mfma4(pw, f4e(d1)[q], af[q + 4]);
              af[q] = mfma4(dw, f4e(q8[h][0])[q], af[q]);
              af[q + 4] = mfma4(dw, f4e(q8[h][1])[q], af[q + 4]);
            }
          }
          float4 x0[4], x1[4];
#pragma unroll
          for (int m = 0; m < 4; ++m) {
            const float* xr = XH + (il * 8 + g2 * 4 + m) * ABD_XL + il * 8 + c * 8;
            x0[m] = *reinterpret_cast<const float4*>(xr);
            x1[m] = *reinterpret_cast<const float4*>(xr + 4);
          }
          const bool to_slab = XOF && a.dwo_slab != nullptr;
#pragma unroll
          for (int m = 0; m < 4; ++m) {
            const int hb = ab * 64 + il * 8 + g2 * 4 + m;
            float4 v0 = make_float4(af[0][m], af[1][m], af[2][m], af[3][m]);
            float4 v1 = make_float4(af[4][m], af[5][m], af[6][m], af[7][m]);
            if (a.relu_xo || to_slab) {
              v0.x = x0[m].x > 0.f ? v0.x : 0.f; v0.y = x0[m].y > 0.f ? v0.y : 0.f; v0.z = x0[m].z > 0.f ? v0.z : 0.f; v0.w = x0[m].w > 0.f ? v0.w : 0.f;
              v1.x = x1[m].x > 0.f ? v1.x : 0.f; v1.y = x1[m].y > 0.f ? v1.y : 0.f; v1.z = x1[m].z > 0.f ? v1.z : 0.f; v1.w = x1[m].w > 0.f ? v1.w : 0.f;
            }
            if (to_slab) {
              float* xr = XH + (il * 8 + g2 * 4 + m) * ABD_XL + il * 8 + c * 8;
              *reinterpret_cast<float4*>(xr) = v0;
              *reinterpret_cast<float4*>(xr + 4) = v1;
            } else if (hb < n * 8) {
              float* o = a.dXo + ((size_t)g * (Ns - n) + t.ng + hb) * F + c * 8;
              *reinterpret_cast<float4*>(o) = v0;
              *reinterpret_cast<float4*>(o + 4) = v1;
            }
          }
          if constexpr (XOF) {
            if (to_slab) {
#pragma unroll
              for (int s_ = 0; s_ < 16; ++s_) {
                const int hr = s_ * 4 + lq;
                const float bv = li < 8 ? rbh[s_] : (li == 8 ? 1.0f : 0.0f);
#pragma unroll
                for (int ft = 0; ft < 2; ++ft) {
                  const float av_ = XH[hr * ABD_XL + (hr >> 3) * 8 + ft * 16 + li];
                  dwacc[ft] = __builtin_amdgcn_mfma_f32_16x16x4f32(av_, bv, dwacc[ft], 0, 0, 0);
                }
              }
            }
          }
        }
      }
    }
  }
  if (want_dx) {
    float xm[RTS][2][4];
#pragma unroll
    for (int rt = 0; rt < RTS; ++rt)
#pragma unroll
      for (int ft = 0; ft < 2; ++ft)
#pragma unroll
        for (int r = 0; r < 4; ++r) {
          const int node = rt * 16 + lq * 4 + r;
          xm[rt][ft][r] = (node < NSP) ? XS[node * ABD_XL + ft * 16 + li] : 0.0f;
        }
#pragma unroll
    for (int rt = 0; rt < RTS; ++rt)
#pragma unroll
      for (int ft = 0; ft < 2; ++ft)
#pragma unroll
        for (int r = 0; r < 4; ++r) {
          const int node = rt * 16 + lq * 4 + r, f = ft * 16 + li;
          float v = dxs[rt][ft][r];
          if (node < n) a.dXa[((size_t)g * n + node) * F + f] = v + dir[rt][ft][r];
          else if (XOF && a.dwo_slab != nullptr) {
            if (node < NSP) XS[node * ABD_XL + f] = (node < NSH && xm[rt][ft][r] > 0.0f) ? v : 0.0f;
          } else if (node < NSH && a.dXo != nullptr) {
            if (a.relu_xo) v = (xm[rt][ft][r] > 0.0f) ? v : 0.0f;
            a.dXo[((size_t)g * (Ns - n) + (node - n)) * F + f] = v;
          }
        }
    if constexpr (XOF) {
      if (a.dwo_slab != nullptr) {
        const int nsho = NSH - n;
#pragma unroll
        for (int s_ = 0; s_ < NSP / 4; ++s_) {
          const int o = s_ * 4 + lq;
          const float bv = li < 8 ? rbg[s_] : (li == 8 ? 1.0f : 0.0f);
#pragma unroll
          for (int ft = 0; ft < 2; ++ft) {
            const int node = n + o;
            const float av_ = (o < nsho && node < NSP) ? XS[(node < NSP ? node : NSP - 1) * ABD_XL + ft * 16 + li] : 0.0f;
            dwacc[ft] = __builtin_amdgcn_mfma_f32_16x16x4f32(av_, bv, dwacc[ft], 0, 0, 0);
          }
        }
        if (li <= 8) {
          float* o = a.dwo_slab + (size_t)g * ABD_DW_STRIDE + li * 32 + lq * 4;
#pragma unroll
          for (int ft = 0; ft < 2; ++ft)
            *reinterpret_cast<float4*>(o + ft * 16) = make_float4(dwacc[ft][0], dwacc[ft][1], dwacc[ft][2], dwacc[ft][3]);
        }
      }
    }
  }
}

static bool attn_bd_shape(const Topo& t, int F, int H, int& PS, bool& hits) {
  if (F != 32 || H < 1 || H > 4 || t.n > 16) return false;
  const int n_priv = t.Ns - t.n - t.ng;
  hits = t.lidar && n_priv > 0;
  if (hits && (t.per != 8 || n_priv != t.n * 8)) return false;
  const int nsh = hits ? t.n + t.ng : t.Ns;
  PS = (nsh + 7) / 8;
  return PS >= 1 && PS <= 4;
}
template <int PS, bool HITS, int AB, bool XOF>
static void launch_attn_bd_x(const AttnArgs& a, hipStream_t s, bool bwd) {
  using L = AbdLds<PS, HITS>;
  if (bwd) { hipLaunchKernelGGL((attn_bwd_bd_kernel<PS, HITS, AB, XOF>), dim3(a.G), dim3(64), sizeof(float) * L::BWD, s, a); return; }
  if constexpr (AB == 1) {
    static thread_local int cap = 0;
    if (cap == 0) {
      int per_cu = 0, dev = 0, cus = 256;
      if (hipOccupancyMaxActiveBlocksPerMultiprocessor(&per_cu, reinterpret_cast<const void*>(&attn_fwd_bdp_kernel<PS, HITS, XOF>), 128,
                                                       sizeof(float) * 2 * L::FWD) != hipSuccess || per_cu < 1) per_cu = 1;
      if (hipGetDevice(&dev) != hipSuccess || hipDeviceGetAttribute(&cus, hipDeviceAttributeMultiprocessorCount, dev) != hipSuccess ||
          cus < 1) cus = 256;
      cap = per_cu * cus;
    }
    if ((a.G + 1) / 2 > 2 * cap) {
      hipLaunchKernelGGL((attn_fwd_bdp_kernel<PS, HITS, XOF>), dim3(cap), dim3(128), sizeof(float) * 2 * L::FWD, s, a);
      return;
    }
  }
  hipLaunchKernelGGL((attn_fwd_bd_kernel<PS, HITS, AB, XOF>), dim3((a.G + 1) / 2), dim3(128), sizeof(float) * 2 * L::FWD, s, a);
}
template <int PS, bool HITS, int AB>
static void launch_attn_bd_one(const AttnArgs& a, hipStream_t s, bool bwd) {
  if (a.Xo_raw != nullptr) launch_attn_bd_x<PS, HITS, AB, true>(a, s, bwd);
  else launch_attn_bd_x<PS, HITS, AB, false>(a, s, bwd);
}
static bool launch_attn_bd(const AttnArgs& a, hipStream_t s, bool bwd) {
  int PS = 0;
  bool hits = false;
  if (!attn_bd_shape(a.t, a.F, a.H, PS, hits)) return false;
  const int AB = (a.t.n + 7) / 8;
  switch ((PS * 2 + (hits ? 1 : 0)) * 4 + AB) {
#define DGPPO_BD(P, HT, B) case ((P) * 2 + (HT)) * 4 + (B): launch_attn_bd_one<P, (HT) != 0, B>(a, s, bwd); return true;
    DGPPO_BD(1, 0, 1) DGPPO_BD(1, 1, 1) DGPPO_BD(2, 0, 1) DGPPO_BD(2, 1, 1) DGPPO_BD(2, 0, 2) DGPPO_BD(2, 1, 2)
    DGPPO_BD(3, 0, 1) DGPPO_BD(3, 1, 1) DGPPO_BD(3, 0, 2) DGPPO_BD(3, 1, 2)
    DGPPO_BD(4, 0, 1) DGPPO_BD(4, 1, 1) DGPPO_BD(4, 0, 2) DGPPO_BD(4, 1, 2)
#undef DGPPO_BD
    default: return false;
  }
}

__global__ void __launch_bounds__(256) attn_bwd_kernel(AttnArgs a) {
  extern __shared__ float sm[];
  const Topo& t = a.t;
  const AttnDims d = attn_dims(t, a.F, a.H);
  const int g = blockIdx.x, tid = threadIdx.x, lane = tid & 63, wave = tid >> 6;
  const int n = d.n, S = d.S, Ns = d.Ns, F = d.F, H = d.H, Fl = d.Fl, Ll = d.Ll, nH = d.nH;
  const int Wd = F + 4, Zl = F + 5, Sp = (S + 3) & ~3;
  float* s_x = sm;
  float* s_q = s_x + d.CT * 16 * Fl;
  float* s_P = s_q + d.RT * 16 * Fl;
  float* s_e = sm + (((d.CT * 16 * Fl + d.RT * 16 * Fl + d.RT * 16 * Ll) + 3) & ~3);
  float* s_c = s_e + n * S * 4;
  float* s_a = s_c + nH * Sp;
  float* s_D = s_a + nH * Sp;
  float* s_z = s_D + d.RT * 16 * Ll;
  const float* dzc = a.dzcat + (size_t)g * n * a.Kp;
  {
    const int F4 = F >> 2, W4 = Wd >> 2;
    const float4* xa = reinterpret_cast<const float4*>(a.Xa + (size_t)g * n * F);
    const float4* xo = reinterpret_cast<const float4*>(a.Xo + (size_t)g * (Ns - n) * F);
    const float4* q4 = reinterpret_cast<const float4*>(a.qt + (size_t)g * nH * F);
    const float4* e4 = reinterpret_cast<const float4*>(a.efeat + (size_t)g * n * S * 4);
    const float* at = a.attn + (size_t)g * n * S * H;
    const int nA = n * F4, nX = Ns * F4, nXp = d.CT * 16 * F4, nQ = nH * F4, nQp = d.RT * 16 * F4, nE = n * S;
    const int nZp = d.RT * 16 * W4, nAt = n * S * H;
    const float4 z4 = make_float4(0.f, 0.f, 0.f, 0.f);
    auto ldz = [&](int idx) {
      const int row = idx / W4, q = idx - row * W4;
      if (row >= nH) return z4;
      const int i = row / H, h = row - i * H;
      return *reinterpret_cast<const float4*>(dzc + i * a.Kp + F + h * Wd + 4 * q);
    };
    float4 vx[4], vq[2], ve[2], vz[2];
    float va[3];
#pragma unroll
    for (int it = 0; it < 4; ++it) { const int idx = tid + it * 256; vx[it] = (idx < nA) ? xa[idx] : ((idx < nX) ? xo[idx - nA] : z4); }
#pragma unroll
    for (int it = 0; it < 2; ++it) { const int idx = tid + it * 256; vq[it] = (idx < nQ) ? q4[idx] : z4; ve[it] = (idx < nE) ? e4[idx] : z4; vz[it] = (idx < nZp) ? ldz(idx) : z4; }
#pragma unroll
    for (int it = 0; it < 3; ++it) { const int idx = tid + it * 256; va[it] = (idx < nAt) ? at[idx] : 0.0f; }
#pragma unroll
    for (int it = 0; it < 4; ++it) { const int idx = tid + it * 256; if (idx < nXp) { const int nd = idx / F4, q = idx - nd * F4; put4(s_x + nd * Fl + 4 * q, vx[it]); } }
#pragma unroll
    for (int it = 0; it < 2; ++it) {
      const int idx = tid + it * 256;
      if (idx < nQp) { const int row = idx / F4, q = idx - row * F4; put4(s_q + row * Fl + 4 * q, vq[it]); }
      if (idx < nE) reinterpret_cast<float4*>(s_e)[idx] = ve[it];
      if (idx < nZp) { const int row = idx / W4, q = idx - row * W4; put4(s_z + row * Zl + 4 * q, vz[it]); }
    }
    auto puta = [&](int idx, float v) { const int h = idx % H, is = idx / H, i = is / S, s = is - i * S; s_a[(i * H + h) * Sp + s] = v; };
#pragma unroll
    for (int it = 0; it < 3; ++it) { const int idx = tid + it * 256; if (idx < nAt) puta(idx, va[it]); }
    for (int idx = tid + 1024; idx < nXp; idx += 256) { const int nd = idx / F4, q = idx - nd * F4; put4(s_x + nd * Fl + 4 * q, (idx < nA) ? xa[idx] : ((idx < nX) ? xo[idx - nA] : z4)); }
    for (int idx = tid + 512; idx < nQp; idx += 256) { const int row = idx / F4, q = idx - row * F4; put4(s_q + row * Fl + 4 * q, (idx < nQ) ? q4[idx] : z4); }
    for (int idx = tid + 512; idx < nE; idx += 256) reinterpret_cast<float4*>(s_e)[idx] = e4[idx];
    for (int idx = tid + 512; idx < nZp; idx += 256) { const int row = idx / W4, q = idx - row * W4; put4(s_z + row * Zl + 4 * q, ldz(idx)); }
    for (int idx = tid + 768; idx < nAt; idx += 256) puta(idx, at[idx]);
    for (int idx = tid; idx < d.RT * 16 * Ll; idx += 256) s_P[idx] = 0.0f;
    if (Sp != S) for (int idx = tid; idx < nH; idx += 256) for (int s = S; s < Sp; ++s) s_a[idx * Sp + s] = 0.0f;
  }
  __syncthreads();
  for (int idx = tid; idx < nH * S; idx += 256) {
    const int pair = idx / S, s = idx - pair * S, i = pair / H;
    const float av = s_a[pair * Sp + s];
    if (av != 0.0f) s_P[pair * Ll + sender_node(t, i, s)] = av;
  }
  mfma_tiles(d.RT, d.CT, F / 4, wave, lane,
             [&](int row, int k) { return s_z[row * Zl + k]; },
             [&](int k, int col) { return s_x[col * Fl + k]; },
             [&](int row, int col, float v) { s_D[row * Ll + col] = v; });
  __syncthreads();
  for (int idx = tid; idx < nH * Sp; idx += 256) {
    const int pair = idx / Sp, s = idx - pair * Sp, i = pair / H;
    float dA = 0.0f;
    if (s < S && s_a[idx] != 0.0f) {
      dA = s_D[pair * Ll + sender_node(t, i, s)];
      const float* dz = s_z + pair * Zl + F;
      const float4 e = reinterpret_cast<const float4*>(s_e)[i * S + s];
      dA = fmaf(dz[0], e.x, fmaf(dz[1], e.y, fmaf(dz[2], e.z, fmaf(dz[3], e.w, dA))));
    }
    s_c[idx] = dA;
  }
  __syncthreads();
  for (int p0 = 0; p0 < nH; p0 += 32) {
    const int pair = p0 + (tid >> 3), sub = tid & 7;
    const bool live = pair < nH;
    float av[ATT_SMAX / 8], dA[ATT_SMAX / 8];
    float dot = 0.0f;
#pragma unroll
    for (int j = 0; j < ATT_SMAX / 8; ++j) {
      const int sl = sub + 8 * j;
      av[j] = (live && sl < S) ? s_a[pair * Sp + sl] : 0.0f;
      dA[j] = (live && sl < S) ? s_c[pair * Sp + sl] : 0.0f;
      dot = fmaf(av[j], dA[j], dot);
    }
    dot = grp8_sum(dot);
#pragma unroll
    for (int j = 0; j < ATT_SMAX / 8; ++j) {
      const int sl = sub + 8 * j;
      if (live && sl < S) s_c[pair * Sp + sl] = av[j] * (dA[j] - dot);
    }
  }
  for (int idx = tid; idx < d.RT * 16 * Ll; idx += 256) s_D[idx] = 0.0f;
  __syncthreads();
  for (int idx = tid; idx < nH * S; idx += 256) {
    const int pair = idx / S, s = idx - pair * S, i = pair / H;
    const float dl = s_c[pair * Sp + s];
    if (dl != 0.0f) s_D[pair * Ll + sender_node(t, i, s)] = dl;
  }
  __syncthreads();
  float* dq = a.dqt + (size_t)g * nH * F;
  mfma_tiles(d.RT, (F + 15) / 16, d.CT * 4, wave, lane,
             [&](int row, int k) { return s_D[row * Ll + k]; },
             [&](int k, int col) { return (col < F) ? s_x[k * Fl + col] : 0.0f; },
             [&](int row, int col, float v) { if (row < nH && col < F) dq[row * F + col] = v; });
  if (a.dXa != nullptr) {
    const int li = lane & 15, lq = lane >> 4;
    const int FT = (F + 15) / 16;
    for (int tile = wave; tile < d.CT * FT; tile += 4) {
      const int rt = tile / FT, ct = tile - rt * FT;
      f32x4g acc = {0.f, 0.f, 0.f, 0.f};
      const int nd_a = rt * 16 + li, col_b = ct * 16 + li;
#pragma unroll 4
      for (int k4 = 0; k4 < d.RT * 4; ++k4) {
        const int kk = k4 * 4 + lq;
        const float bz = (col_b < F) ? s_z[kk * Zl + col_b] : 0.0f;
        const float bq = (col_b < F) ? s_q[kk * Fl + col_b] : 0.0f;
        acc = __builtin_amdgcn_mfma_f32_16x16x4f32(s_P[kk * Ll + nd_a], bz, acc, 0, 0, 0);
        acc = __builtin_amdgcn_mfma_f32_16x16x4f32(s_D[kk * Ll + nd_a], bq, acc, 0, 0, 0);
      }
#pragma unroll
      for (int r = 0; r < 4; ++r) {
        const int nd = rt * 16 + lq * 4 + r, f = ct * 16 + li;
        if (nd >= Ns || f >= F) continue;
        if (nd < n) a.dXa[((size_t)g * n + nd) * F + f] = acc[r] + dzc[nd * a.Kp + f];
        else if (a.dXo != nullptr) a.dXo[((size_t)g * (Ns - n) + (nd - n)) * F + f] = acc[r];
      }
    }
  }
}

static int32_t attn_check(const dgppo_env_cfg* cfg, int F, int H, int Kp, int G, AttnArgs& a) {
  int32_t rc = dgppo_validate_cfg(cfg);
  if (rc) return rc;
  a.t = make_topo(*cfg);
  DGPPO_REQUIRE(F >= 1 && F <= 64 && H >= 1 && H <= 8, "attn: bad F=%d H=%d", F, H);
  DGPPO_REQUIRE(Kp >= F + H * (F + 4) + 1, "attn: Kp=%d too small", Kp);
  DGPPO_REQUIRE(G >= 0, "attn: G < 0");
  a.F = F; a.H = H; a.Kp = Kp; a.G = G;
  return 0;
}

enum class AttnFamily { SLOT8, BD, MFMA, VALU };
static AttnFamily attn_family(const Topo& t, int F, int H, int Kp, bool bwd, bool dXa) {
  int PS = 0;
  bool hits = false;
  if ((Kp & 3) == 0 && attn_slot8_shape(t, F, H) && !(bwd && dXa)) return AttnFamily::SLOT8;
  if ((Kp & 3) == 0 && attn_bd_shape(t, F, H, PS, hits)) return AttnFamily::BD;
  if ((F & 3) == 0 && t.S <= 64 && attn_mfma_smem(attn_dims(t, F, H), bwd) <= 64 * 1024 && (!bwd || F >= 16)) return AttnFamily::MFMA;
  return AttnFamily::VALU;
}

extern "C" int32_t dgppo_attn_fwd(const dgppo_env_cfg* cfg, int32_t F, int32_t H, int32_t Kp, const float* qt,
                                  const float* Xa, const float* Xo, const float* efeat, const float* emask, float* zcat,
                                  float* attn, int32_t G, void* stream) {
  AttnArgs a{};
  int32_t rc = attn_check(cfg, F, H, Kp, G, a);
  if (rc) return rc;
  if (G == 0) return 0;
  DGPPO_REQUIRE(qt && Xa && efeat && emask && zcat, "attn_fwd: NULL operand");
  DGPPO_REQUIRE(a.t.Ns == a.t.n || Xo, "attn_fwd: Xo is NULL");
  a.qt = qt; a.Xa = Xa; a.Xo = Xo; a.efeat = efeat; a.emask = emask; a.zcat = zcat; a.attn = attn;
  const Topo& t = a.t;
  const hipStream_t s = (hipStream_t)stream;
  const size_t smem = sizeof(float) * ((size_t)t.Ns * (F + 1) + (size_t)t.n * H * (F + 1) + (size_t)t.n * t.S * 5 +
                                       (size_t)t.n * t.S * H);
  DGPPO_REQUIRE(smem <= 64 * 1024, "attn_fwd: graph too large for LDS (%zu B)", smem);
  bool launched = true;
  switch (attn_family(t, F, H, Kp, false, false)) {
    case AttnFamily::SLOT8: launched = launch_attn_slot8(a, s, false); break;
    case AttnFamily::BD: launched = launch_attn_bd(a, s, false); break;
    case AttnFamily::MFMA:
      hipLaunchKernelGGL(attn_fwd_kernel, dim3(G), dim3(256), attn_mfma_smem(attn_dims(t, F, H), false), s, a);
      break;
    case AttnFamily::VALU: hipLaunchKernelGGL(attn_fwd_valu_kernel, dim3(G), dim3(256), smem, s, a); break;
  }
  DGPPO_REQUIRE(launched, "attn_fwd: dispatch failed");
  DGPPO_LAUNCH_CHECK();
  return 0;
}

extern "C" int32_t dgppo_attn_bwd(const dgppo_env_cfg* cfg, int32_t F, int32_t H, int32_t Kp, const float* dzcat,
                                  const float* attn, const float* qt, const float* Xa, const float* Xo,
                                  const float* efeat, float* dqt, float* dXa, float* dXo, int32_t relu_xo, int32_t G,
                                  void* stream) {
  AttnArgs a{};
  int32_t rc = attn_check(cfg, F, H, Kp, G, a);
  if (rc) return rc;
  if (G == 0) return 0;
  DGPPO_REQUIRE(dzcat && attn && qt && Xa && efeat && dqt, "attn_bwd: NULL operand");
  DGPPO_REQUIRE(a.t.Ns == a.t.n || Xo, "attn_bwd: Xo is NULL");
  DGPPO_REQUIRE(!(dXo && !dXa), "attn_bwd: dXo needs dXa");
  a.dzcat = dzcat; a.attn = (float*)attn; a.qt = qt; a.Xa = Xa; a.Xo = Xo; a.efeat = efeat; a.dqt = dqt; a.dXa = dXa; a.dXo = dXo;
  const Topo& t = a.t;
  const hipStream_t s = (hipStream_t)stream;
  const size_t smem = sizeof(float) * ((size_t)t.Ns * (F + 1) + (size_t)t.n * H * (F + 1) + (size_t)t.n * t.S * 4 +
                                       2 * (size_t)t.n * t.S * H + (size_t)t.n * H * (F + 5));
  DGPPO_REQUIRE(smem <= 64 * 1024, "attn_bwd: graph too large for LDS (%zu B)", smem);
  const AttnFamily fam = attn_family(t, F, H, Kp, true, dXa != nullptr);
  a.relu_xo = (relu_xo && dXo && fam == AttnFamily::BD) ? 1 : 0;
  bool launched = true;
  switch (fam) {
    case AttnFamily::SLOT8: launched = launch_attn_slot8(a, s, true); break;
    case AttnFamily::BD: launched = launch_attn_bd(a, s, true); break;
    case AttnFamily::MFMA:
      hipLaunchKernelGGL(attn_bwd_kernel, dim3(G), dim3(256), attn_mfma_smem(attn_dims(t, F, H), true), s, a);
      break;
    case AttnFamily::VALU: hipLaunchKernelGGL(attn_bwd_valu_kernel, dim3(G), dim3(256), smem, s, a); break;
  }
  DGPPO_REQUIRE(launched, "attn_bwd: dispatch failed");
  DGPPO_LAUNCH_CHECK();
  if (relu_xo && dXo && !a.relu_xo)
    return dgppo_relu_bwd(dXo, Xo, (int64_t)G * (t.Ns - t.n) * F, stream);
  return 0;
}

static bool attn_xo_ok(const Topo& t, int F, int H, int Kp) {
  return t.Ns > t.n && attn_family(t, F, H, Kp, true, true) == AttnFamily::BD;
}
extern "C" int32_t dgppo_attn_xo_supported(const dgppo_env_cfg* cfg, int32_t F, int32_t H, int32_t Kp) {
  AttnArgs a{};
  if (attn_check(cfg, F, H, Kp, 0, a)) return 0;
  return attn_xo_ok(a.t, F, H, Kp) ? 1 : 0;
}
extern "C" int32_t dgppo_attn_fwd_xo(const dgppo_env_cfg* cfg, int32_t F, int32_t H, int32_t Kp, const float* qt, const float* Xa,
                                     const float* Xo_raw, const float* Wo, int32_t ldwo, const float* bo, const float* efeat,
                                     const float* emask, float* zcat, float* attn, int32_t G, void* stream) {
  AttnArgs a{};
  int32_t rc = attn_check(cfg, F, H, Kp, G, a);
  if (rc) return rc;
  if (G == 0) return 0;
  DGPPO_REQUIRE(qt && Xa && Xo_raw && Wo && bo && efeat && emask && zcat, "attn_fwd_xo: NULL operand");
  DGPPO_REQUIRE(ldwo >= 32, "attn_fwd_xo: ldwo=%d < 32", ldwo);
  DGPPO_REQUIRE(attn_xo_ok(a.t, F, H, Kp), "attn_fwd_xo: no fused kernel for this topology (ask dgppo_attn_xo_supported)");
  a.qt = qt; a.Xa = Xa; a.Xo = nullptr; a.efeat = efeat; a.emask = emask; a.zcat = zcat; a.attn = attn;
  a.Xo_raw = Xo_raw; a.Wo = Wo; a.ldwo = ldwo; a.bo = bo;
  const bool launched = launch_attn_bd(a, (hipStream_t)stream, false);
  DGPPO_REQUIRE(launched, "attn_fwd_xo: dispatch failed");
  DGPPO_LAUNCH_CHECK();
  return 0;
}
extern "C" int32_t dgppo_attn_bwd_xo(const dgppo_env_cfg* cfg, int32_t F, int32_t H, int32_t Kp, const float* dzcat,
                                     const float* attn, const float* qt, const float* Xa, const float* Xo_raw, const float* Wo,
                                     int32_t ldwo, const float* bo, const float* efeat, float* dqt, float* dXa, float* dXo,
                                     int32_t relu_xo, int32_t G, void* stream) {
  AttnArgs a{};
  int32_t rc = attn_check(cfg, F, H, Kp, G, a);
  if (rc) return rc;
  if (G == 0) return 0;
  DGPPO_REQUIRE(dzcat && attn && qt && Xa && Xo_raw && Wo && bo && efeat && dqt, "attn_bwd_xo: NULL operand");
  DGPPO_REQUIRE(ldwo >= 32, "attn_bwd_xo: ldwo=%d < 32", ldwo);
  DGPPO_REQUIRE(!(dXo && !dXa), "attn_bwd_xo: dXo needs dXa");
  DGPPO_REQUIRE(attn_xo_ok(a.t, F, H, Kp), "attn_bwd_xo: no fused kernel for this topology (ask dgppo_attn_xo_supported)");
  a.dzcat = dzcat; a.attn = (float*)attn; a.qt = qt; a.Xa = Xa; a.Xo = nullptr; a.efeat = efeat; a.dqt = dqt; a.dXa = dXa; a.dXo = dXo;
  a.relu_xo = (relu_xo && dXo) ? 1 : 0;
  a.Xo_raw = Xo_raw; a.Wo = Wo; a.ldwo = ldwo; a.bo = bo;
  const bool launched = launch_attn_bd(a, (hipStream_t)stream, true);
  DGPPO_REQUIRE(launched, "attn_bwd_xo: dispatch failed");
  DGPPO_LAUNCH_CHECK();
  return 0;
}

__global__ void __launch_bounds__(320) attn_xo_dw_reduce_kernel(const float* slab, int G, float* dWo, int lddwo, float* dbo) {
  const int e = threadIdx.x;
  if (e >= 288) return;
  const int per = (G + gridDim.x - 1) / gridDim.x;
  const int g0 = blockIdx.x * per, g1 = min(G, g0 + per);
  float sacc[8] = {0.f, 0.f, 0.f, 0.f, 0.f, 0.f, 0.f, 0.f};
  int g = g0;
  for (; g + 7 < g1; g += 8) {
#pragma unroll
    for (int u = 0; u < 8; ++u) sacc[u] += slab[(size_t)(g + u) * ABD_DW_STRIDE + e];
  }
  for (; g < g1; ++g) sacc[0] += slab[(size_t)g * ABD_DW_STRIDE + e];
  const float sum = ((sacc[0] + sacc[1]) + (sacc[2] + sacc[3])) + ((sacc[4] + sacc[5]) + (sacc[6] + sacc[7]));
  if (g0 >= g1) return;
  if (e < 256) atomicAdd(dWo + (size_t)(e >> 5) * lddwo + (e & 31), sum);
  else atomicAdd(dbo + (e - 256), sum);
}
extern "C" int64_t dgppo_attn_xo_workspace_bytes(int32_t G) { return G < 0 ? 0 : (int64_t)G * ABD_DW_STRIDE * (int64_t)sizeof(float); }
extern "C" int32_t dgppo_attn_bwd_xo_dw(const dgppo_env_cfg* cfg, int32_t F, int32_t H, int32_t Kp, const float* dzcat,
                                        const float* attn, const float* qt, const float* Xa, const float* Xo_raw, const float* Wo,
                                        int32_t ldwo, const float* bo, const float* efeat, float* dqt, float* dXa, float* dWo,
                                        int32_t lddwo, float* dbo, float* workspace, int64_t workspace_bytes, int32_t G,
                                        void* stream) {
  AttnArgs a{};
  int32_t rc = attn_check(cfg, F, H, Kp, G, a);
  if (rc) return rc;
  if (G == 0) return 0;
  DGPPO_REQUIRE(dzcat && attn && qt && Xa && Xo_raw && Wo && bo && efeat && dqt && dXa && dWo && dbo && workspace,
                "attn_bwd_xo_dw: NULL operand");
  DGPPO_REQUIRE(ldwo >= 32 && lddwo >= 32, "attn_bwd_xo_dw: ldwo=%d lddwo=%d < 32", ldwo, lddwo);
  DGPPO_REQUIRE(workspace_bytes >= dgppo_attn_xo_workspace_bytes(G) && (reinterpret_cast<uintptr_t>(workspace) & 15) == 0,
                "attn_bwd_xo_dw: workspace too small or not 16-byte aligned");
  DGPPO_REQUIRE(attn_xo_ok(a.t, F, H, Kp), "attn_bwd_xo_dw: no fused kernel for this topology (ask dgppo_attn_xo_supported)");
  a.dzcat = dzcat; a.attn = (float*)attn; a.qt = qt; a.Xa = Xa; a.Xo = nullptr; a.efeat = efeat; a.dqt = dqt; a.dXa = dXa; a.dXo = nullptr;
  a.relu_xo = 1;
  a.Xo_raw = Xo_raw; a.Wo = Wo; a.ldwo = ldwo; a.bo = bo; a.dwo_slab = workspace;
  const bool launched = launch_attn_bd(a, (hipStream_t)stream, true);
  DGPPO_REQUIRE(launched, "attn_bwd_xo_dw: dispatch failed");
  int blocks = (G + 31) / 32;
  blocks = blocks < 1 ? 1 : (blocks > 1024 ? 1024 : blocks);
  hipLaunchKernelGGL(attn_xo_dw_reduce_kernel, dim3(blocks), dim3(320), 0, (hipStream_t)stream, workspace, G, dWo, lddwo, dbo);
  DGPPO_LAUNCH_CHECK();
  return 0;
}
```

dgppo_amd/nets.py:

```python
from __future__ import annotations

import math
from typing import Dict, List, Optional, Tuple

import numpy as np
import torch

from . import _native as N
from . import ops_nn as K

H_HEADS = 3
MSG_DIM = 32
OUT_DIM = 64
HID = 64


def _ceil4(x):
    return (x + 3) // 4 * 4


class Layout:
    def __init__(self):
        self.entries: Dict[str, Tuple[int, Tuple[int, ...]]] = {}
        self.size = 0

    def add(self, name, *shape):
        n = int(np.prod(shape))
        self.size = (self.size + 3) // 4 * 4
        self.entries[name] = (self.size, tuple(shape))
        self.size += n

    def view(self, flat: torch.Tensor, name: str) -> torch.Tensor:
        off, shape = self.entries[name]
        return flat[off:off + math.prod(shape)].view(shape)


def make_layout(kind: str, node_dim: int, gnn_layers: int, n_out: int, rnn: str = "gru", rnn_layers: int = 1) -> Layout:
    L = Layout()
    f = node_dim
    for l in range(gnn_layers):
        d = OUT_DIM if l == gnn_layers - 1 else MSG_DIM
        hd = H_HEADS * d
        for nm, shp in (("Wq", (f, hd)), ("bq", (hd,)), ("Wk", (f, hd)), ("bk", (hd,)), ("Wv", (f, hd)), ("bv", (hd,)),
                        ("We", (4, hd)), ("Wu", (f, d)), ("bu", (d,))):
            L.add(f"gnn{l}.{nm}", *shp)
        f = d
    for i in (1, 2):
        L.add(f"mlp.W{i}", 2 * HID if (kind == "Vhg" and i == 1) else HID, HID)
        L.add(f"mlp.b{i}", HID)
        L.add(f"mlp.g{i}", HID)
        L.add(f"mlp.be{i}", HID)
    assert rnn in ("gru", "lstm", "none"), rnn
    for l in range(rnn_layers if rnn == "lstm" else 0):
        L.add(f"lstm{l}.Wi", HID, 4 * HID)
        L.add(f"lstm{l}.Wh", HID, 4 * HID)
        L.add(f"lstm{l}.bh", 4 * HID)
    for l in range(rnn_layers if rnn == "gru" else 0):
        pre = "gru" if l == 0 else f"gru{l}"
        L.add(f"{pre}.Wi", HID, 3 * HID)
        L.add(f"{pre}.bi", 3 * HID)
        L.add(f"{pre}.Wh", HID, 3 * HID)
        L.add(f"{pre}.bhn", HID)
    if kind == "policy":
        L.add("head.Ws", HID, HID)
        L.add("head.bs", HID)
        L.add("head.Wms", HID, 2 * n_out)
        L.add("head.bms", 2 * n_out)
    else:
        L.add("head.Wo", HID, n_out)
        L.add("head.bo", n_out)
    return L


class Arena:

    def __init__(self, device):
        self.device = device
        self.bufs: Dict[str, torch.Tensor] = {}
        self.generation = 0

    def get(self, name: str, *shape, dtype=torch.float32, zero=False) -> torch.Tensor:
        n = math.prod(shape)
        b = self.bufs.get(name)
        if b is None or b.numel() < n or b.dtype != dtype:
            if b is not None:
                self.generation += 1
            b = torch.empty(max(n, 1), dtype=dtype, device=self.device)
            self.bufs[name] = b
        v = b[:n].view(shape)
        if zero:
            v.zero_()
        return v


class GraphFeats:

    def __init__(self, cfg: N.EnvCfg, G: int, arena: Arena, tag: str):
        self.cfg, self.G = cfg, G
        n, S = cfg.n_agents, cfg.fan_in
        self.n_other = cfg.num_nodes - 1 - n
        self.Fp = 8
        self.Xa = arena.get(f"{tag}.Xa0", G * n, self.Fp)
        self.Xo = arena.get(f"{tag}.Xo0", max(G * self.n_other, 1), self.Fp)[:G * self.n_other]
        self.efeat = arena.get(f"{tag}.efeat", G * n, S, 4)
        self.emask = arena.get(f"{tag}.emask", G * n, S)

    def compute(self, agent, agent_se, agent_st, goal, obst, hits, hits_se, hits_st, env_ids, n_env, n_time):
        assert n_env * n_time == self.G
        K.graph_feats(self.cfg, agent, agent_se, agent_st, goal, obst, hits, hits_se, hits_st, env_ids, n_env, n_time,
                      self.Xa, self.Xo if self.n_other > 0 else None, self.efeat, self.emask, self.Fp)
        return self


class Net:

    def __init__(self, kind: str, cfg: N.EnvCfg, gnn_layers: int, n_out: int, device, grads: Optional[torch.Tensor] = None,
                 rnn: str = "gru", rnn_layers: int = 1):
        assert kind in ("policy", "Vl", "Vh", "Vhg")
        self.kind, self.cfg, self.gnn_layers, self.n_out, self.device = kind, cfg, gnn_layers, n_out, device
        self.rnn, self.rnn_layers = rnn, (rnn_layers if rnn != "none" else 0)
        self.carry_dim = HID * max(self.rnn_layers, 1) * (2 if rnn == "lstm" else 1)
        self.layout = make_layout(kind, cfg.node_dim, gnn_layers, n_out, rnn, rnn_layers)
        self.params = torch.zeros(self.layout.size, device=device)
        if grads is None:
            grads = torch.zeros(self.layout.size, device=device)
        assert grads.shape == (self.layout.size,) and grads.is_contiguous() and grads.data_ptr() % 16 == 0
        self.grads = grads
        self.arena = Arena(device)
        self.ws_arena = Arena(device)
        self._views: Dict[tuple, torch.Tensor] = {}
        self.dims = []
        f = cfg.node_dim
        for l in range(gnn_layers):
            d = OUT_DIM if l == gnn_layers - 1 else MSG_DIM
            fp = 8 if l == 0 else f
            kp = _ceil4(fp + H_HEADS * (fp + 4) + 1)
            self.dims.append((f, fp, d, kp))
            f = d
        self.prep_layout = Layout()
        for l, (f, fp, d, kp) in enumerate(self.dims):
            self.prep_layout.add(f"gnn{l}.Mcat", fp, H_HEADS * fp)
            self.prep_layout.add(f"gnn{l}.cvec", H_HEADS * fp)
            self.prep_layout.add(f"gnn{l}.Wout", kp, d)
        self.prep = torch.zeros(self.prep_layout.size, device=device)
        self.prep_grads = torch.zeros(self.prep_layout.size, device=device)

    def _cached(self, kind: str, layout, flat, name):
        key = (kind, name)
        v = self._views.get(key)
        if v is None:
            v = self._views[key] = layout.view(flat, name)
        return v

    def p(self, name):
        return self._cached("p", self.layout, self.params, name)

    def g(self, name):
        return self._cached("g", self.layout, self.grads, name)

    def pp(self, name):
        return self._cached("pp", self.prep_layout, self.prep, name)

    def pg(self, name):
        return self._cached("pg", self.prep_layout, self.prep_grads, name)

    def prepare(self):
        for l, (f, fp, d, kp) in enumerate(self.dims):
            q = lambda nm: self.p(f"gnn{l}.{nm}")
            K.gnn_prep(q("Wq"), q("bq"), q("Wk"), q("Wv"), q("bv"), q("We"), q("Wu"), self.pp(f"gnn{l}.Mcat"),
                       self.pp(f"gnn{l}.cvec"), self.pp(f"gnn{l}.Wout"), f, fp, d, H_HEADS, kp)

    def _xo_fusable(self, l: int) -> bool:
        if l != 0 or self.gnn_layers != 2:
            return False
        key = "_xo_ok"
        if not hasattr(self, key):
            f1, fp1, d1, kp1 = self.dims[1]
            setattr(self, key, self.dims[0][1] == 8 and self.dims[0][2] == 32 and fp1 == 32 and
                    K.attn_xo_supported(self.cfg, fp1, H_HEADS, kp1))
        return getattr(self, key)

    def zero_grads(self):
        self.grads.zero_()

    def forward(self, feats: GraphFeats, n_seq: int, T: int, h0: Optional[torch.Tensor], tag: str = "f",
                hs_out: Optional[torch.Tensor] = None, train: bool = True):
        cfg, G, A = self.cfg, feats.G, self.arena
        n = cfg.n_agents
        R = G * n
        Ro = G * feats.n_other
        act = {"feats": feats, "G": G, "n_seq": n_seq, "T": T}
        Xa, Xo = feats.Xa, feats.Xo
        xo_fused = None
        for l, (f, fp, d, kp) in enumerate(self.dims):
            qt = A.get(f"{tag}.qt{l}", R, H_HEADS * fp)
            K.dense_fwd(Xa, self.pp(f"gnn{l}.Mcat"), self.pp(f"gnn{l}.cvec"), qt)
            zcat = A.get(f"{tag}.zcat{l}", R, kp)
            attn = A.get(f"{tag}.attn{l}", R, cfg.fan_in, H_HEADS) if train else None
            if xo_fused is not None:
                K.attn_fwd_xo(cfg, fp, H_HEADS, kp, qt, Xa, xo_fused[0], xo_fused[1], xo_fused[2], feats.efeat, feats.emask, zcat, attn, G)
            else:
                K.attn_fwd(cfg, fp, H_HEADS, kp, qt, Xa, Xo if Ro > 0 else None, feats.efeat, feats.emask, zcat, attn, G)
            act[f"xo_fused{l}"] = xo_fused
            xo_fused = None
            Xa_n = A.get(f"{tag}.Xa{l + 1}", R, d)
            K.dense_fwd(zcat, self.pp(f"gnn{l}.Wout"), self.p(f"gnn{l}.bu"), Xa_n, act=1)
            act[f"Xa{l}"], act[f"Xo{l}"], act[f"qt{l}"], act[f"zcat{l}"], act[f"attn{l}"] = Xa, Xo, qt, zcat, attn
            if l < self.gnn_layers - 1 and Ro > 0:
                if self._xo_fusable(l):
                    xo_fused = (Xo, self.pp(f"gnn{l}.Wout")[:fp], self.p(f"gnn{l}.bu"))
                    Xo = None
                else:
                    Xo_n = A.get(f"{tag}.Xo{l + 1}", Ro, d)
                    K.dense_fwd(Xo, self.pp(f"gnn{l}.Wout")[:fp], self.p(f"gnn{l}.bu"), Xo_n, act=1)
                    Xo = Xo_n
            Xa = Xa_n
        act[f"Xa{self.gnn_layers}"] = Xa
        if self.kind == "Vl":
            pooled = A.get(f"{tag}.pool", G, OUT_DIM)
            K.mean_agents(Xa, pooled, G, n, OUT_DIM)
            x, Rh, n_inner = pooled, G, 1
        else:
            x, Rh, n_inner = Xa, R, n
        if self.kind == "Vhg":
            pooled = A.get(f"{tag}.pool", G, OUT_DIM)
            K.mean_agents(Xa, pooled, G, n, OUT_DIM)
            xcat = A.get(f"{tag}.xcat", R, 2 * OUT_DIM)
            xcat[:, :OUT_DIM].copy_(Xa)
            xcat.view(G, n, 2 * OUT_DIM)[:, :, OUT_DIM:].copy_(pooled.view(G, 1, OUT_DIM).expand(G, n, OUT_DIM))
            x = xcat
        act["Rh"], act["n_inner"], act["mlp_in"] = Rh, n_inner, x
        gi = A.get(f"{tag}.gi", Rh, 3 * HID)
        if self.kind == "Vhg" or self.rnn != "gru":
            sv = {nm: A.get(f"{tag}.{nm}", Rh, w) for nm, w in (("p1", HID), ("y1", HID), ("st1", 2), ("p2", HID), ("y2", HID), ("st2", 2))}
            K.dense_fwd(x, self.p("mlp.W1"), self.p("mlp.b1"), sv["p1"])
            K.ln_relu_fwd(sv["p1"], self.p("mlp.g1"), self.p("mlp.be1"), sv["y1"], sv["st1"])
            K.dense_fwd(sv["y1"], self.p("mlp.W2"), self.p("mlp.b2"), sv["p2"])
            K.ln_relu_fwd(sv["p2"], self.p("mlp.g2"), self.p("mlp.be2"), sv["y2"], sv["st2"])
            if self.rnn == "gru":
                K.dense_fwd(sv["y2"], self.p("gru.Wi"), self.p("gru.bi"), gi)
            act.update(sv)
        else:
            saves = None
            if train:
                saves = tuple(A.get(f"{tag}.{nm}{i}", Rh, w) for i in (1, 2) for nm, w in (("p", HID), ("y", HID), ("st", 2)))
                for i in (1, 2):
                    act[f"p{i}"], act[f"y{i}"], act[f"st{i}"] = saves[3 * (i - 1):3 * i]
            K.mlp_gi_fwd(x, self.p("mlp.W1"), self.p("mlp.b1"), self.p("mlp.g1"), self.p("mlp.be1"), self.p("mlp.W2"),
                         self.p("mlp.b2"), self.p("mlp.g2"), self.p("mlp.be2"), self.p("gru.Wi"), self.p("gru.bi"), gi, saves)
        assert n_seq * T == Rh, (n_seq, T, Rh)
        L, CD = self.rnn_layers, self.carry_dim
        if h0 is not None:
            assert tuple(h0.shape) == (n_seq, CD), (tuple(h0.shape), n_seq, CD)
        if hs_out is not None:
            assert tuple(hs_out.shape) == (Rh, CD), (tuple(hs_out.shape), Rh, CD)
        act["gi"] = gi
        simple = (self.rnn == "gru" and L == 1)
        if simple:
            hs = hs_out if hs_out is not None else A.get(f"{tag}.hs", Rh, HID)
            hprev = A.get(f"{tag}.hprev", Rh, HID) if train else None
            gates = A.get(f"{tag}.gates", Rh, 4 * HID) if train else None
            feat = hs
            act["hs"], act["hprev"], act["gates"] = hs, hprev, gates
        fused_tail = (simple and T == 1 and self.kind == "policy")
        if simple and not fused_tail:
            K.gru_fwd(gi, self.p("gru.Wh"), self.p("gru.bhn"), h0, hs, hprev, gates, n_seq, T, n_inner)
        if self.rnn == "none":
            feat = act["y2"]
            if hs_out is not None:
                if h0 is not None and T == 1:
                    hs_out.copy_(h0)
                else:
                    hs_out.zero_()
        elif self.rnn == "lstm":
            x_l = act["y2"]
            act["stack"] = []
            for l in range(L):
                zi = A.get(f"{tag}.zi{l}", Rh, 4 * HID)
                for half in (slice(0, 2 * HID), slice(2 * HID, 4 * HID)):
                    K.dense_fwd(x_l, self.p(f"lstm{l}.Wi")[:, half], None, zi[:, half])
                c0_l = h0_l = None
                if h0 is not None:
                    c0_l, h0_l = A.get(f"{tag}.c0_{l}", n_seq, HID), A.get(f"{tag}.h0_{l}", n_seq, HID)
                    c0_l.copy_(h0[:, (2 * l) * HID:(2 * l + 1) * HID])
                    h0_l.copy_(h0[:, (2 * l + 1) * HID:(2 * l + 2) * HID])
                cs_l, hs_l = A.get(f"{tag}.cs{l}", Rh, HID), A.get(f"{tag}.hs{l}", Rh, HID)
                cprev_l = A.get(f"{tag}.cprev{l}", Rh, HID) if train else None
                hprev_l = A.get(f"{tag}.hprev{l}", Rh, HID) if train else None
                gates_l = A.get(f"{tag}.gates{l}", Rh, 4 * HID) if train else None
                K.lstm_fwd(zi, self.p(f"lstm{l}.Wh"), self.p(f"lstm{l}.bh"), c0_l, h0_l, cs_l, hs_l, cprev_l, hprev_l, gates_l,
                           n_seq, T, n_inner)
                if hs_out is not None:
                    hs_out[:, (2 * l) * HID:(2 * l + 1) * HID].copy_(cs_l)
                    hs_out[:, (2 * l + 1) * HID:(2 * l + 2) * HID].copy_(hs_l)
                act["stack"].append(dict(x=x_l, hs=hs_l, cprev=cprev_l, hprev=hprev_l, gates=gates_l))
                x_l = hs_l
            feat = x_l
        elif not simple:
            x_l = None
            act["stack"] = []
            for l in range(L):
                pre = "gru" if l == 0 else f"gru{l}"
                gi_l = gi if l == 0 else A.get(f"{tag}.gi{l}", Rh, 3 * HID)
                if l > 0:
                    K.dense_fwd(x_l, self.p(f"{pre}.Wi"), self.p(f"{pre}.bi"), gi_l)
                h0_l = None
                if h0 is not None:
                    h0_l = A.get(f"{tag}.h0_{l}", n_seq, HID)
                    h0_l.copy_(h0[:, l * HID:(l + 1) * HID])
                hs_l = A.get(f"{tag}.hs{l}", Rh, HID)
                hprev_l = A.get(f"{tag}.hprev{l}", Rh, HID) if train else None
                gates_l = A.get(f"{tag}.gates{l}", Rh, 4 * HID) if train else None
                K.gru_fwd(gi_l, self.p(f"{pre}.Wh"), self.p(f"{pre}.bhn"), h0_l, hs_l, hprev_l, gates_l, n_seq, T, n_inner)
                if hs_out is not None:
                    hs_out[:, l * HID:(l + 1) * HID].copy_(hs_l)
                act["stack"].append(dict(x=x_l, gi=gi_l, hs=hs_l, hprev=hprev_l, gates=gates_l))
                x_l = hs_l
            feat = x_l
        act["feat"] = feat
        if self.kind == "policy":
            u = A.get(f"{tag}.u", Rh, HID) if (train or not fused_tail) else None
            ms = A.get(f"{tag}.ms", Rh, 4)
            if fused_tail:
                K.gru1_head_fwd(gi, self.p("gru.Wh"), self.p("gru.bhn"), h0, self.p("head.Ws"), self.p("head.bs"),
                                self.p("head.Wms"), self.p("head.bms"), hs, hprev, gates, u, ms)
            else:
                K.dense_fwd(feat, self.p("head.Ws"), self.p("head.bs"), u)
                K.dense_fwd(u, self.p("head.Wms"), self.p("head.bms"), ms)
            act["u"], act["ms"] = u, ms
        else:
            v = A.get(f"{tag}.v", Rh, self.n_out)
            K.dense_fwd(feat, self.p("head.Wo"), self.p("head.bo"), v)
            act["v"] = v
        return act

    def backward(self, act, dout: torch.Tensor, tag: str = "b"):
        A = self.arena
        ws_floats = getattr(self, "_bwdw_floats", 16 << 20)

        def _alloc(n_floats):
            self._bwdw_floats = max(ws_floats, n_floats)
            return self.ws_arena.get(f"{tag}.bwdw_ws", self._bwdw_floats)
        batch = K.BwdWBatch(self.device, _alloc) if dout.is_cuda else None
        if batch is not None:
            batch.__enter__()
        try:
            self._backward_body(act, dout, tag)
        except BaseException:
            if batch is not None:
                batch.__exit__(RuntimeError, None, None)
            raise
        if batch is not None:
            batch.__exit__(None, None, None)
        for l, (f, fp, d, kp) in enumerate(self.dims):
            q = lambda nm: self.p(f"gnn{l}.{nm}")
            gq = lambda nm: self.g(f"gnn{l}.{nm}")
            K.gnn_unprep(self.pg(f"gnn{l}.Mcat"), self.pg(f"gnn{l}.cvec"), self.pg(f"gnn{l}.Wout"), q("Wq"), q("bq"), q("Wk"),
                         gq("Wq"), gq("bq"), gq("Wk"), gq("Wv"), gq("bv"), gq("We"), gq("Wu"), f, fp, d, H_HEADS, kp)
        self.prep_grads.zero_()

    def _backward_body(self, act, dout: torch.Tensor, tag: str):
        cfg, A = self.cfg, self.arena
        G, Rh, n_inner, n_seq, T = act["G"], act["Rh"], act["n_inner"], act["n_seq"], act["T"]
        n = cfg.n_agents
        R = G * n
        feats: GraphFeats = act["feats"]
        Ro = G * feats.n_other
        feat = act["feat"]
        fused_trunk = self.rnn == "gru" and self.rnn_layers == 1 and self.kind != "Vhg" and dout.is_cuda
        dgi0 = None
        dhs = A.get(f"{tag}.dhs", Rh, HID)
        if self.kind == "policy":
            K.dense_bwd_w(act["u"], dout, self.g("head.Wms"), self.g("head.bms"))
            du = A.get(f"{tag}.du", Rh, HID)
            K.dense_fwd(dout, self.p("head.Wms"), None, du, trans_w=True)
            K.dense_bwd_w(feat, du, self.g("head.Ws"), self.g("head.bs"))
            K.dense_fwd(du, self.p("head.Ws"), None, dhs, trans_w=True)
        else:
            K.dense_bwd_w(feat, dout, self.g("head.Wo"), self.g("head.bo"))
            K.dense_fwd(dout, self.p("head.Wo"), None, dhs, trans_w=True)
        if self.rnn == "none":
            dy = dhs
        elif self.rnn == "lstm":
            stack = act["stack"]
            for l in range(len(stack) - 1, -1, -1):
                st = stack[l]
                dz = A.get(f"{tag}.dz_lstm{l}", Rh, 4 * HID)
                K.lstm_bwd(dhs, self.p(f"lstm{l}.Wh"), st["cprev"], st["gates"], dz, n_seq, T, n_inner)
                for half in (slice(0, 2 * HID), slice(2 * HID, 4 * HID)):
                    K.dense_bwd_w(st["hprev"], dz[:, half], self.g(f"lstm{l}.Wh")[:, half], self.g(f"lstm{l}.bh")[half])
                    K.dense_bwd_w(st["x"], dz[:, half], self.g(f"lstm{l}.Wi")[:, half], None)
                dx = A.get(f"{tag}.dy" if l == 0 else f"{tag}.dx{l}", Rh, HID)
                K.dense_fwd(dz, self.p(f"lstm{l}.Wi"), None, dx, trans_w=True)
                dhs = dx
            dy = dhs
        else:
            stack = act.get("stack") or [dict(x=None, gi=act["gi"], hs=act["hs"], hprev=act["hprev"], gates=act["gates"])]
            for l in range(len(stack) - 1, -1, -1):
                st = stack[l]
                pre = "gru" if l == 0 else f"gru{l}"
                dgi = A.get(f"{tag}.dgi{l}", Rh, 3 * HID)
                dgh = A.get(f"{tag}.dgh{l}", Rh, 3 * HID)
                K.gru_bwd(dhs, self.p(f"{pre}.Wh"), st["hprev"], st["gates"], dgi, dgh, n_seq, T, n_inner)
                K.dense_bwd_w(st["hprev"], dgh[:, :2 * HID], self.g(f"{pre}.Wh")[:, :2 * HID], None)
                K.dense_bwd_w(st["hprev"], dgh[:, 2 * HID:], self.g(f"{pre}.Wh")[:, 2 * HID:], self.g(f"{pre}.bhn"))
                x_l = act["y2"] if l == 0 else st["x"]
                K.dense_bwd_w(x_l, dgi, self.g(f"{pre}.Wi"), self.g(f"{pre}.bi"))
                if l == 0 and fused_trunk:
                    dgi0 = dgi
                    break
                dx = A.get(f"{tag}.dy" if l == 0 else f"{tag}.dx{l}", Rh, HID)
                K.dense_fwd(dgi, self.p(f"{pre}.Wi"), None, dx, trans_w=True)
                dhs = dx
            dy = dhs
        x_in = {1: act["mlp_in"], 2: act["y1"]}
        top = act[f"Xa{self.gnn_layers}"]
        if fused_trunk:
            dpre2, dpre1 = A.get(f"{tag}.dpre2", Rh, HID), A.get(f"{tag}.dpre1", Rh, HID)
            dy = A.get(f"{tag}.dyy1", Rh, HID)
            K.mlp_gi_bwd(dgi0, self.p("gru.Wi"), self.p("mlp.W2"), self.p("mlp.W1"), self.p("mlp.g2"), self.p("mlp.g1"),
                         act["p2"], act["y2"], act["st2"], act["p1"], act["y1"], act["st1"],
                         top if self.kind in ("policy", "Vh") else None, dpre2, dpre1, dy,
                         self.g("mlp.g2"), self.g("mlp.be2"), self.g("mlp.g1"), self.g("mlp.be1"))
            K.dense_bwd_w(x_in[2], dpre2, self.g("mlp.W2"), self.g("mlp.b2"))
            K.dense_bwd_w(x_in[1], dpre1, self.g("mlp.W1"), self.g("mlp.b1"))
        for i in (() if fused_trunk else (2, 1)):
            dpre = A.get(f"{tag}.dpre{i}", Rh, HID)
            K.ln_relu_bwd(act[f"p{i}"], act[f"y{i}"], act[f"st{i}"], self.p(f"mlp.g{i}"), dy, dpre, self.g(f"mlp.g{i}"),
                          self.g(f"mlp.be{i}"))
            K.dense_bwd_w(x_in[i], dpre, self.g(f"mlp.W{i}"), self.g(f"mlp.b{i}"))
            dy = A.get(f"{tag}.dyy{i}", Rh, HID if not (self.kind == "Vhg" and i == 1) else 2 * HID)
            K.dense_fwd(dpre, self.p(f"mlp.W{i}"), None, dy, trans_w=True,
                        relu_mask=top if (i == 1 and self.kind in ("policy", "Vh")) else None)
        if self.kind == "Vl":
            dXa = A.get(f"{tag}.dXaL", R, OUT_DIM)
            K.mean_agents(dy, dXa, G, n, OUT_DIM, backward=True, relu_mask=top)
        elif self.kind == "Vhg":
            dXa = A.get(f"{tag}.dXaL", R, OUT_DIM)
            dXa.copy_(dy[:, :OUT_DIM])
            dglob = A.get(f"{tag}.dglob", R, OUT_DIM)
            dglob.copy_(dy[:, OUT_DIM:])
            dpool = A.get(f"{tag}.dpool", G, OUT_DIM)
            K.mean_agents(dglob, dpool, G, n, OUT_DIM)
            K.mean_agents(dpool, dXa, G, n, OUT_DIM, backward=2, relu_mask=top)
        else:
            dXa = dy
        dXo = None
        for l in range(self.gnn_layers - 1, -1, -1):
            f, fp, d, kp = self.dims[l]
            K.dense_bwd_w(act[f"zcat{l}"], dXa, self.pg(f"gnn{l}.Wout"), self.g(f"gnn{l}.bu"))
            dz = A.get(f"{tag}.dz{l}", R, kp)
            K.dense_fwd(dXa, self.pp(f"gnn{l}.Wout"), None, dz, trans_w=True)
            if dXo is not None:
                K.dense_bwd_w(act[f"Xo{l}"], dXo, self.pg(f"gnn{l}.Wout")[:fp], self.g(f"gnn{l}.bu"))
            dqt = A.get(f"{tag}.dqt{l}", R, H_HEADS * fp)
            need_dx = l > 0
            dXa_l = A.get(f"{tag}.dXa{l}", R, fp) if need_dx else None
            dXo_prev = dXo
            dXo_l = A.get(f"{tag}.dXo{l}", Ro, fp) if (need_dx and Ro > 0) else None
            more_dXo = dXo_prev is not None and dXo_l is not None
            xf = act.get(f"xo_fused{l}")
            if xf is not None and dXa_l is not None and not more_dXo:
                ws = A.get(f"{tag}.xo_ws", K.attn_xo_workspace_floats(G), 1).view(-1)
                K.attn_bwd_xo_dw(cfg, fp, H_HEADS, kp, dz, act[f"attn{l}"], act[f"qt{l}"], act[f"Xa{l}"], xf[0], xf[1], xf[2],
                                 feats.efeat, dqt, dXa_l, self.pg(f"gnn{l - 1}.Wout")[:self.dims[l - 1][1]], self.g(f"gnn{l - 1}.bu"), ws, G)
                dXo_l = None
            elif xf is not None:
                K.attn_bwd_xo(cfg, fp, H_HEADS, kp, dz, act[f"attn{l}"], act[f"qt{l}"], act[f"Xa{l}"], xf[0], xf[1], xf[2],
                              feats.efeat, dqt, dXa_l, dXo_l, G, relu_xo=(dXo_l is not None and not more_dXo))
            else:
                K.attn_bwd(cfg, fp, H_HEADS, kp, dz, act[f"attn{l}"], act[f"qt{l}"], act[f"Xa{l}"],
                           act[f"Xo{l}"] if Ro > 0 else None, feats.efeat, dqt, dXa_l, dXo_l, G,
                           relu_xo=(dXo_l is not None and not more_dXo))
            K.dense_bwd_w(act[f"Xa{l}"], dqt, self.pg(f"gnn{l}.Mcat"), self.pg(f"gnn{l}.cvec"))
            if need_dx:
                K.dense_fwd(dqt, self.pp(f"gnn{l}.Mcat"), None, dXa_l, accumulate=True, trans_w=True, relu_mask=act[f"Xa{l}"])
                if more_dXo:
                    K.dense_fwd(dXo_prev, self.pp(f"gnn{l}.Wout")[:fp], None, dXo_l, accumulate=True, trans_w=True,
                                relu_mask=act[f"Xo{l}"])
            dXa, dXo = dXa_l, dXo_l

    def load_tree(self, tree: dict):
        t = tree["params"]
        to = lambda x: torch.as_tensor(np.asarray(x), dtype=torch.float32).to(self.device)
        if self.kind == "policy":
            base, gnn, head_name = t["PolicyNet_0"], t["PolicyNet_0"]["GraphTransformerGNN_0"], "PolicyGNNHead"
        else:
            base, gnn, head_name = t, t["GraphTransformerGNN_0"], "ValueGNNHead"
        for l in range(self.gnn_layers):
            gl = gnn[f"GraphTransformer_{l}"]
            for nm, dn, key in (("Wq", "Dense_0", "kernel"), ("bq", "Dense_0", "bias"), ("Wk", "Dense_1", "kernel"),
                                ("bk", "Dense_1", "bias"), ("Wv", "Dense_2", "kernel"), ("bv", "Dense_2", "bias"),
                                ("We", "Dense_3", "kernel"), ("Wu", "Dense_4", "kernel"), ("bu", "Dense_4", "bias")):
                self.p(f"gnn{l}.{nm}").copy_(to(gl[dn][key]))
        hd = base[head_name]
        for i in (1, 2):
            self.p(f"mlp.W{i}").copy_(to(hd[f"Dense_{i - 1}"]["kernel"]))
            self.p(f"mlp.b{i}").copy_(to(hd[f"Dense_{i - 1}"]["bias"]))
            self.p(f"mlp.g{i}").copy_(to(hd[f"LayerNorm_{i - 1}"]["scale"]))
            self.p(f"mlp.be{i}").copy_(to(hd[f"LayerNorm_{i - 1}"]["bias"]))
        for l in range(self.rnn_layers if self.rnn == "lstm" else 0):
            lc = base["RNN_0"][f"LSTMCell_{3 * l + 2}"]
            self.p(f"lstm{l}.Wi").copy_(torch.cat([to(lc[k]["kernel"]) for k in ("ii", "if", "ig", "io")], dim=1))
            self.p(f"lstm{l}.Wh").copy_(torch.cat([to(lc[k]["kernel"]) for k in ("hi", "hf", "hg", "ho")], dim=1))
            self.p(f"lstm{l}.bh").copy_(torch.cat([to(lc[k]["bias"]) for k in ("hi", "hf", "hg", "ho")]))
        for l in range(self.rnn_layers if self.rnn == "gru" else 0):
            pre = "gru" if l == 0 else f"gru{l}"
            gr = base["RNN_0"][f"GRUCell_{2 * l + 1}"]
            self.p(f"{pre}.Wi").copy_(torch.cat([to(gr[k]["kernel"]) for k in ("ir", "iz", "in")], dim=1))
            self.p(f"{pre}.bi").copy_(torch.cat([to(gr[k]["bias"]) for k in ("ir", "iz", "in")]))
            self.p(f"{pre}.Wh").copy_(torch.cat([to(gr[k]["kernel"]) for k in ("hr", "hz", "hn")], dim=1))
            self.p(f"{pre}.bhn").copy_(to(gr["hn"]["bias"]))
        if self.kind == "policy":
            self.p("head.Ws").copy_(to(t["ScaleHid"]["kernel"]))
            self.p("head.bs").copy_(to(t["ScaleHid"]["bias"]))
            self.p("head.Wms").copy_(torch.cat([to(t["OutputDenseMean"]["kernel"]), to(t["OutputDenseStdTrans"]["kernel"])], 1))
            self.p("head.bms").copy_(torch.cat([to(t["OutputDenseMean"]["bias"]), to(t["OutputDenseStdTrans"]["bias"])]))
        else:
            self.p("head.Wo").copy_(to(t["Dense_0"]["kernel"]))
            self.p("head.bo").copy_(to(t["Dense_0"]["bias"]))
        self.prepare()

    def to_tree(self, flat: Optional[torch.Tensor] = None) -> dict:
        flat = self.params if flat is None else flat
        v = lambda nm: self.layout.view(flat, nm).detach().cpu().numpy().copy()
        gnn = {}
        for l in range(self.gnn_layers):
            gnn[f"GraphTransformer_{l}"] = {
                "Dense_0": {"kernel": v(f"gnn{l}.Wq"), "bias": v(f"gnn{l}.bq")},
                "Dense_1": {"kernel": v(f"gnn{l}.Wk"), "bias": v(f"gnn{l}.bk")},
                "Dense_2": {"kernel": v(f"gnn{l}.Wv"), "bias": v(f"gnn{l}.bv")},
                "Dense_3": {"kernel": v(f"gnn{l}.We")},
                "Dense_4": {"kernel": v(f"gnn{l}.Wu"), "bias": v(f"gnn{l}.bu")},
            }
        head = {}
        for i in (1, 2):
            head[f"Dense_{i - 1}"] = {"kernel": v(f"mlp.W{i}"), "bias": v(f"mlp.b{i}")}
            head[f"LayerNorm_{i - 1}"] = {"scale": v(f"mlp.g{i}"), "bias": v(f"mlp.be{i}")}
        rnn = {}
        for l in range(self.rnn_layers if self.rnn == "lstm" else 0):
            Wi, Wh, bh = v(f"lstm{l}.Wi"), v(f"lstm{l}.Wh"), v(f"lstm{l}.bh")
            cell = {}
            for q, g_ in enumerate("ifgo"):
                cell["i" + g_] = {"kernel": Wi[:, q * 64:(q + 1) * 64]}
                cell["h" + g_] = {"kernel": Wh[:, q * 64:(q + 1) * 64], "bias": bh[q * 64:(q + 1) * 64]}
            rnn[f"LSTMCell_{3 * l + 2}"] = cell
        for l in range(self.rnn_layers if self.rnn == "gru" else 0):
            pre = "gru" if l == 0 else f"gru{l}"
            Wi, bi, Wh = v(f"{pre}.Wi"), v(f"{pre}.bi"), v(f"{pre}.Wh")
            rnn[f"GRUCell_{2 * l + 1}"] = {
                "ir": {"kernel": Wi[:, :64], "bias": bi[:64]}, "iz": {"kernel": Wi[:, 64:128], "bias": bi[64:128]},
                "in": {"kernel": Wi[:, 128:], "bias": bi[128:]}, "hr": {"kernel": Wh[:, :64]}, "hz": {"kernel": Wh[:, 64:128]},
                "hn": {"kernel": Wh[:, 128:], "bias": v(f"{pre}.bhn")}}
        if self.kind == "policy":
            Wms, bms = v("head.Wms"), v("head.bms")
            k = self.n_out
            return {"params": {
                "PolicyNet_0": dict({"GraphTransformerGNN_0": gnn, "PolicyGNNHead": head}, **({"RNN_0": rnn} if rnn else {})),
                "ScaleHid": {"kernel": v("head.Ws"), "bias": v("head.bs")},
                "OutputDenseMean": {"kernel": Wms[:, :k], "bias": bms[:k]},
                "OutputDenseStdTrans": {"kernel": Wms[:, k:], "bias": bms[k:]}}}
        return {"params": dict({"GraphTransformerGNN_0": gnn, "ValueGNNHead": head, "Dense_0": {"kernel": v("head.Wo"), "bias": v("head.bo")}},
                               **({"RNN_0": rnn} if rnn else {}))}
```

dgppo_amd/ops_nn.py:

```python
from __future__ import annotations

import ctypes as C
from typing import Optional

import torch

from . import _native as N

FLOPS = [0.0]


def _mat(t: torch.Tensor, name: str):
    if t.dim() != 2:
        raise ValueError(f"{name} must be 2-D, got {tuple(t.shape)}")
    if not t.is_cuda:
        raise RuntimeError(f"{name} must live on the GPU (the HIP path has no CPU fallback)")
    if t.dtype != torch.float32:
        raise TypeError(f"{name} must be float32")
    if t.shape[1] > 1 and t.stride(1) != 1:
        raise ValueError(f"{name} must have unit inner stride")
    ld = t.stride(0) if t.shape[0] > 1 else max(t.shape[1], t.stride(0))
    return C.c_void_p(t.data_ptr()), int(ld), int(t.shape[0]), int(t.shape[1])


def _p(t: Optional[torch.Tensor], name="tensor", dtype=torch.float32):
    return N.ptr(t, dtype, name)


def dense_fwd(X, W, bias, Y, act: int = 0, accumulate: bool = False, trans_w: bool = False, relu_mask=None):
    xp, ldx, M, K = _mat(X, "X")
    wp, ldw, wr, wc = _mat(W, "W")
    yp, ldy, My, Ncol = _mat(Y, "Y")
    Kw, Nw = (wc, wr) if trans_w else (wr, wc)
    if Kw != K or Nw != Ncol or My != M:
        raise ValueError(f"dense_fwd: shape mismatch X{tuple(X.shape)} W{tuple(W.shape)} trans={trans_w} Y{tuple(Y.shape)}")
    if bias is not None:
        N.expect_shape(bias, (Ncol,), "bias")
    mp, ldm = C.c_void_p(0), 0
    if relu_mask is not None:
        mp, ldm, Mm, Nm = _mat(relu_mask, "relu_mask")
        if (Mm, Nm) != (M, Ncol):
            raise ValueError(f"dense_fwd: relu_mask {tuple(relu_mask.shape)} does not match Y {tuple(Y.shape)}")
    FLOPS[0] += 2.0 * M * K * Ncol
    rc = N.lib().dgppo_dense_fwd(xp, ldx, wp, ldw, _p(bias, "bias"), yp, ldy, M, K, Ncol, int(act), int(accumulate),
                                 int(trans_w), mp, ldm, N.stream_ptr())
    N.check(rc, "dgppo_dense_fwd")


def mlp_gi_fwd(X, W1, b1, g1, be1, W2, b2, g2, be2, Wi, bi, gi, saves=None):
    xp, ldx, M, K = _mat(X, "X")
    if K != 64:
        raise ValueError(f"mlp_gi_fwd: X must be [M, 64], got {tuple(X.shape)}")
    for t, shp, nm in ((W1, (64, 64), "W1"), (W2, (64, 64), "W2"), (Wi, (64, 192), "Wi"), (b1, (64,), "b1"), (g1, (64,), "g1"),
                       (be1, (64,), "be1"), (b2, (64,), "b2"), (g2, (64,), "g2"), (be2, (64,), "be2"), (bi, (192,), "bi"),
                       (gi, (M, 192), "gi")):
        N.expect_shape(t, shp, nm)
    sv = [None] * 6
    if saves is not None:
        for t, shp, nm in zip(saves, ((M, 64), (M, 64), (M, 2), (M, 64), (M, 64), (M, 2)), ("p1", "y1", "st1", "p2", "y2", "st2")):
            N.expect_shape(t, shp, nm)
        sv = list(saves)
    FLOPS[0] += 2.0 * M * (64 * 64 * 2 + 64 * 192)
    rc = N.lib().dgppo_mlp_gi_fwd(xp, ldx, _p(W1), _p(b1), _p(g1), _p(be1), _p(W2), _p(b2), _p(g2), _p(be2), _p(Wi), _p(bi),
                                  *[_p(t) for t in sv], _p(gi), M, N.stream_ptr())
    N.check(rc, "dgppo_mlp_gi_fwd")


def mlp_gi_bwd(dgi, Wi, W2, W1, g2, g1, p2, y2, st2, p1, y1, st1, relu_mask, dpre2, dpre1, dx, dg2, db2, dg1, db1):
    M = dgi.shape[0]
    N.expect_shape(dgi, (M, 192), "dgi")
    for t, shp, nm in ((Wi, (64, 192), "Wi"), (W2, (64, 64), "W2"), (W1, (64, 64), "W1"), (g2, (64,), "g2"), (g1, (64,), "g1"),
                       (p2, (M, 64), "p2"), (y2, (M, 64), "y2"), (st2, (M, 2), "st2"), (p1, (M, 64), "p1"), (y1, (M, 64), "y1"),
                       (st1, (M, 2), "st1"), (dpre2, (M, 64), "dpre2"), (dpre1, (M, 64), "dpre1"), (dx, (M, 64), "dx"),
                       (dg2, (64,), "dg2"), (db2, (64,), "db2"), (dg1, (64,), "dg1"), (db1, (64,), "db1")):
        N.expect_shape(t, shp, nm)
    mp, ldm = (None, 0)
    if relu_mask is not None:
        mp, ldm, Mm, Km = _mat(relu_mask, "relu_mask")
        if (Mm, Km) != (M, 64):
            raise ValueError(f"mlp_gi_bwd: relu_mask must be [M, 64], got {tuple(relu_mask.shape)}")
    FLOPS[0] += 2.0 * M * (64 * 64 * 2 + 64 * 192)
    rc = N.lib().dgppo_mlp_gi_bwd(_p(dgi), _p(Wi), _p(W2), _p(W1), _p(g2), _p(g1), _p(p2), _p(y2), _p(st2), _p(p1), _p(y1), _p(st1),
                                  mp if mp is not None else C.c_void_p(0), ldm, _p(dpre2), _p(dpre1), _p(dx), 64,
                                  _p(dg2), _p(db2), _p(dg1), _p(db1), M, N.stream_ptr())
    N.check(rc, "dgppo_mlp_gi_bwd")


def gru1_head_fwd(gi, Wh, bhn, h0, W1, b1, W2, b2, hs, hprev, gates, u, out):
    M = gi.shape[0]
    n_out = out.shape[1]
    N.expect_shape(gi, (M, 192), "gi"); N.expect_shape(Wh, (64, 192), "Wh"); N.expect_shape(bhn, (64,), "bhn")
    N.expect_shape(hs, (M, 64), "hs"); N.expect_shape(out, (M, n_out), "out")
    if h0 is not None:
        N.expect_shape(h0, (M, 64), "h0")
    if W2 is not None:
        N.expect_shape(W1, (64, 64), "W1"); N.expect_shape(b1, (64,), "b1")
        N.expect_shape(W2, (64, n_out), "W2"); N.expect_shape(b2, (n_out,), "b2")
    else:
        N.expect_shape(W1, (64, n_out), "W1"); N.expect_shape(b1, (n_out,), "b1")
    for t, shp, nm in ((hprev, (M, 64), "hprev"), (gates, (M, 256), "gates"), (u, (M, 64), "u")):
        if t is not None:
            N.expect_shape(t, shp, nm)
    FLOPS[0] += 2.0 * M * (64 * 192 + (64 * 64 + 64 * n_out if W2 is not None else 64 * n_out))
    rc = N.lib().dgppo_gru1_head_fwd(_p(gi), _p(Wh), _p(bhn), _p(h0), _p(W1), _p(b1), _p(W2), _p(b2), _p(hs), _p(hprev),
                                     _p(gates), _p(u), _p(out), M, n_out, N.stream_ptr())
    N.check(rc, "dgppo_gru1_head_fwd")


_WS: dict = {}


def _bwd_w_workspace(device, K: int, Ncol: int) -> torch.Tensor:
    lib = N.lib()
    lib.dgppo_dense_bwd_w_workspace_bytes.restype = C.c_int64
    need = int(lib.dgppo_dense_bwd_w_workspace_bytes(C.c_int32(K), C.c_int32(Ncol)))
    need = min(need, 64 << 20)
    key = (device.index, torch.cuda.current_stream(device).cuda_stream)
    ws = _WS.get(key)
    if ws is None or ws.numel() * 4 < need:
        ws = torch.empty(need // 4, dtype=torch.float32, device=device)
        _WS[key] = ws
    return ws


class ReduceDesc(C.Structure):
    _fields_ = [("part", C.c_void_p), ("dW", C.c_void_p), ("db", C.c_void_p), ("part_stride", C.c_int32), ("slabs", C.c_int32),
                ("ldw", C.c_int32), ("K", C.c_int32), ("N", C.c_int32), ("pending", C.c_int32)]


class BwdWBatch:
    _active = {}

    def __init__(self, device, alloc):
        self.device, self.alloc = device, alloc
        self.key = None
        self.descs = []
        self.offset = 0
        self.ws = None

    def __enter__(self):
        self.key = (self.device.index, torch.cuda.current_stream(self.device).cuda_stream)
        if self.key in BwdWBatch._active:
            raise RuntimeError("BwdWBatch: nested batches on one stream")
        BwdWBatch._active[self.key] = self
        return self

    def region(self, nbytes: int):
        nbytes = (nbytes + 255) & ~255
        if self.ws is None or self.ws.numel() * 4 < self.offset + nbytes:
            if self.descs:
                self.flush()
            self.ws = self.alloc(max(self.offset + nbytes, 2 * (self.ws.numel() * 4 if self.ws is not None else 0)) // 4)
        view = self.ws[self.offset // 4:(self.offset + nbytes) // 4]
        self.offset += nbytes
        return view

    def flush(self):
        if self.descs:
            arr = (ReduceDesc * len(self.descs))(*self.descs)
            N.check(N.lib().dgppo_dense_bwd_w_reduce_batch(arr, C.c_int32(len(self.descs)), N.stream_ptr()),
                    "dgppo_dense_bwd_w_reduce_batch")
        self.descs = []
        self.offset = 0

    def __exit__(self, *exc):
        try:
            if exc[0] is None:
                self.flush()
        finally:
            BwdWBatch._active.pop(self.key, None)
        return False


def dense_bwd_w(X, dY, dW, db=None):
    xp, ldx, M, K = _mat(X, "X")
    yp, ldy, My, Ncol = _mat(dY, "dY")
    wp, ldw, Kw, Nw = _mat(dW, "dW")
    if My != M or Kw != K or Nw != Ncol:
        raise ValueError(f"dense_bwd_w: shape mismatch X{tuple(X.shape)} dY{tuple(dY.shape)} dW{tuple(dW.shape)}")
    if db is not None:
        N.expect_shape(db, (Ncol,), "db")
    FLOPS[0] += 2.0 * M * K * Ncol
    batch = BwdWBatch._active.get((X.device.index, torch.cuda.current_stream(X.device).cuda_stream)) if X.is_cuda else None
    if batch is not None:
        lib = N.lib()
        lib.dgppo_dense_bwd_w_workspace_bytes.restype = C.c_int64
        need = min(int(lib.dgppo_dense_bwd_w_workspace_bytes(C.c_int32(K), C.c_int32(Ncol))), 64 << 20)
        ws = batch.region(need)
        d = ReduceDesc()
        rc = lib.dgppo_dense_bwd_w_deferred(xp, ldx, yp, ldy, wp, ldw, _p(db, "db"), M, K, Ncol, _p(ws, "workspace"),
                                            C.c_int64(ws.numel() * 4), C.byref(d), N.stream_ptr())
        N.check(rc, "dgppo_dense_bwd_w_deferred")
        if d.pending:
            batch.descs.append(d)
        return
    ws = _bwd_w_workspace(X.device, K, Ncol)
    rc = N.lib().dgppo_dense_bwd_w(xp, ldx, yp, ldy, wp, ldw, _p(db, "db"), M, K, Ncol, _p(ws, "workspace"),
                                   C.c_int64(ws.numel() * 4), N.stream_ptr())
    N.check(rc, "dgppo_dense_bwd_w")


def graph_feats(cfg: N.EnvCfg, agent, agent_se, agent_st, goal, obst, hits, hits_se, hits_st, env_ids, n_env, n_time,
                Xa, Xo, efeat, emask, Fp):
    G = n_env * n_time
    n, S = cfg.n_agents, cfg.fan_in
    n_other = cfg.num_nodes - 1 - n
    N.expect_shape(Xa, (G * n, Fp), "Xa")
    if n_other > 0:
        N.expect_shape(Xo, (G * n_other, Fp), "Xo")
    N.expect_shape(efeat, (G * n, S, 4), "efeat")
    N.expect_shape(emask, (G * n, S), "emask")
    for name, t_, se, st, inner in (("agent", agent, agent_se, agent_st, (n, cfg.state_dim)),
                                    ("hits", hits, hits_se, hits_st, (n, cfg.top_k, 2))):
        if t_ is None:
            continue
        if not (t_.is_cuda and t_.dtype == torch.float32):
            raise ValueError(f"graph_feats: {name} must be a float32 CUDA tensor")
        want, acc = [], 1
        for d in reversed(inner):
            want.append(acc)
            acc *= d
        if tuple(t_.shape[-len(inner):]) != tuple(inner) or list(t_.stride()[-len(inner):]) != want[::-1]:
            raise ValueError(f"graph_feats: the trailing {inner} block of {name} must be dense (got shape {tuple(t_.shape)}, "
                             f"strides {t_.stride()})")
        avail = t_.untyped_storage().nbytes() // 4 - t_.storage_offset()
        if env_ids is None and (n_env - 1) * se + (n_time - 1) * st + acc > avail:
            raise ValueError(f"graph_feats: {name}: the strides reach beyond its storage")
    rc = N.lib().dgppo_graph_feats(
        C.byref(cfg), C.c_void_p(agent.data_ptr()), C.c_int64(agent_se), C.c_int64(agent_st), _p(goal, "goal"),
        _p(obst, "obst") if (obst is not None and not cfg.is_lidar) else C.c_void_p(0),
        C.c_void_p(hits.data_ptr()) if hits is not None else C.c_void_p(0), C.c_int64(hits_se), C.c_int64(hits_st),
        _p(env_ids, "env_ids", torch.int32), C.c_int32(n_env), C.c_int32(n_time), _p(Xa, "Xa"), _p(Xo, "Xo"),
        _p(efeat, "efeat"), _p(emask, "emask"), C.c_int32(Fp), N.stream_ptr())
    N.check(rc, "dgppo_graph_feats")


def attn_fwd(cfg, F, H, Kp, qt, Xa, Xo, efeat, emask, zcat, attn, G):
    n, S = cfg.n_agents, cfg.fan_in
    N.expect_shape(qt, (G * n, H * F), "qt")
    N.expect_shape(Xa, (G * n, F), "Xa")
    N.expect_shape(zcat, (G * n, Kp), "zcat")
    if attn is not None:
        N.expect_shape(attn, (G * n, S, H), "attn")
    FLOPS[0] += 2.0 * G * n * H * S * (2 * F + 4)
    rc = N.lib().dgppo_attn_fwd(C.byref(cfg), F, H, Kp, _p(qt), _p(Xa), _p(Xo), _p(efeat), _p(emask), _p(zcat), _p(attn),
                                G, N.stream_ptr())
    N.check(rc, "dgppo_attn_fwd")


def attn_bwd(cfg, F, H, Kp, dzcat, attn, qt, Xa, Xo, efeat, dqt, dXa, dXo, G, relu_xo: bool = False):
    n = cfg.n_agents
    N.expect_shape(dzcat, (G * n, Kp), "dzcat")
    N.expect_shape(dqt, (G * n, H * F), "dqt")
    if dXa is not None:
        N.expect_shape(dXa, (G * n, F), "dXa")
    FLOPS[0] += 4.0 * G * n * H * cfg.fan_in * (2 * F + 4)
    rc = N.lib().dgppo_attn_bwd(C.byref(cfg), F, H, Kp, _p(dzcat), _p(attn), _p(qt), _p(Xa), _p(Xo), _p(efeat), _p(dqt),
                                _p(dXa), _p(dXo), int(relu_xo), G, N.stream_ptr())
    N.check(rc, "dgppo_attn_bwd")


def attn_xo_supported(cfg, F, H, Kp) -> bool:
    return bool(N.lib().dgppo_attn_xo_supported(C.byref(cfg), F, H, Kp))


def _wo_ptr(Wo):
    if not Wo.is_cuda or Wo.dtype != torch.float32:
        raise TypeError("Wo must be a float32 GPU tensor")
    return C.c_void_p(Wo.data_ptr())


def _wo_ld(Wo):
    if Wo.dim() != 2 or Wo.shape[0] != 8 or Wo.shape[1] < 32 or Wo.stride(1) != 1:
        raise ValueError(f"Wo must be [8, >= 32] with contiguous rows, got {tuple(Wo.shape)} strides {Wo.stride()}")
    return int(Wo.stride(0))


def attn_fwd_xo(cfg, F, H, Kp, qt, Xa, Xo_raw, Wo, bo, efeat, emask, zcat, attn, G):
    n, S = cfg.n_agents, cfg.fan_in
    N.expect_shape(qt, (G * n, H * F), "qt")
    N.expect_shape(Xa, (G * n, F), "Xa")
    N.expect_shape(zcat, (G * n, Kp), "zcat")
    N.expect_shape(Xo_raw, (G * (cfg.num_nodes - 1 - n), 8), "Xo_raw")
    N.expect_shape(bo, (32,), "bo")
    if attn is not None:
        N.expect_shape(attn, (G * n, S, H), "attn")
    FLOPS[0] += 2.0 * G * n * H * S * (2 * F + 4) + 2.0 * G * (cfg.num_nodes - 1 - n) * 8 * 32
    rc = N.lib().dgppo_attn_fwd_xo(C.byref(cfg), F, H, Kp, _p(qt), _p(Xa), _p(Xo_raw), _wo_ptr(Wo),
                                   _wo_ld(Wo), _p(bo), _p(efeat), _p(emask), _p(zcat), _p(attn), G, N.stream_ptr())
    N.check(rc, "dgppo_attn_fwd_xo")


def attn_bwd_xo(cfg, F, H, Kp, dzcat, attn, qt, Xa, Xo_raw, Wo, bo, efeat, dqt, dXa, dXo, G, relu_xo: bool = False):
    n = cfg.n_agents
    N.expect_shape(dzcat, (G * n, Kp), "dzcat")
    N.expect_shape(dqt, (G * n, H * F), "dqt")
    N.expect_shape(Xo_raw, (G * (cfg.num_nodes - 1 - n), 8), "Xo_raw")
    if dXa is not None:
        N.expect_shape(dXa, (G * n, F), "dXa")
    FLOPS[0] += 4.0 * G * n * H * cfg.fan_in * (2 * F + 4) + 2.0 * G * (cfg.num_nodes - 1 - n) * 8 * 32
    rc = N.lib().dgppo_attn_bwd_xo(C.byref(cfg), F, H, Kp, _p(dzcat), _p(attn), _p(qt), _p(Xa), _p(Xo_raw),
                                   _wo_ptr(Wo), _wo_ld(Wo), _p(bo), _p(efeat), _p(dqt), _p(dXa), _p(dXo),
                                   int(relu_xo), G, N.stream_ptr())
    N.check(rc, "dgppo_attn_bwd_xo")


def attn_xo_workspace_floats(G: int) -> int:
    return int(N.lib().dgppo_attn_xo_workspace_bytes(int(G))) // 4


def attn_bwd_xo_dw(cfg, F, H, Kp, dzcat, attn, qt, Xa, Xo_raw, Wo, bo, efeat, dqt, dXa, dWo, dbo, workspace, G):
    n = cfg.n_agents
    N.expect_shape(dzcat, (G * n, Kp), "dzcat")
    N.expect_shape(dqt, (G * n, H * F), "dqt")
    N.expect_shape(dXa, (G * n, F), "dXa")
    N.expect_shape(Xo_raw, (G * (cfg.num_nodes - 1 - n), 8), "Xo_raw")
    N.expect_shape(dbo, (32,), "dbo")
    FLOPS[0] += 4.0 * G * n * H * cfg.fan_in * (2 * F + 4) + 4.0 * G * (cfg.num_nodes - 1 - n) * 8 * 32
    rc = N.lib().dgppo_attn_bwd_xo_dw(C.byref(cfg), F, H, Kp, _p(dzcat), _p(attn), _p(qt), _p(Xa), _p(Xo_raw), _wo_ptr(Wo), _wo_ld(Wo),
                                      _p(bo), _p(efeat), _p(dqt), _p(dXa), _wo_ptr(dWo), _wo_ld(dWo), _p(dbo), _p(workspace),
                                      C.c_int64(workspace.numel() * 4), G, N.stream_ptr())
    N.check(rc, "dgppo_attn_bwd_xo_dw")


def gnn_prep(Wq, bq, Wk, Wv, bv, We, Wu, Mcat, cvec, Wout, F, Fp, D, H, Kp):
    rc = N.lib().dgppo_gnn_prep(_p(Wq), _p(bq), _p(Wk), _p(Wv), _p(bv), _p(We), _p(Wu), _p(Mcat), _p(cvec), _p(Wout),
                                F, Fp, D, H, Kp, N.stream_ptr())
    N.check(rc, "dgppo_gnn_prep")


def gnn_unprep(dMcat, dcvec, dWout, Wq, bq, Wk, dWq, dbq, dWk, dWv, dbv, dWe, dWu, F, Fp, D, H, Kp):
    rc = N.lib().dgppo_gnn_unprep(_p(dMcat), _p(dcvec), _p(dWout), _p(Wq), _p(bq), _p(Wk), _p(dWq), _p(dbq), _p(dWk),
                                  _p(dWv), _p(dbv), _p(dWe), _p(dWu), F, Fp, D, H, Kp, N.stream_ptr())
    N.check(rc, "dgppo_gnn_unprep")


def ln_relu_fwd(x, gamma, beta, y, stats):
    M = x.shape[0]
    N.expect_shape(x, (M, 64), "x")
    N.expect_shape(y, (M, 64), "y")
    rc = N.lib().dgppo_ln_relu_fwd(_p(x), _p(gamma), _p(beta), _p(y), _p(stats), M, N.stream_ptr())
    N.check(rc, "dgppo_ln_relu_fwd")


def ln_relu_bwd(x, y, stats, gamma, dy, dx, dgamma, dbeta):
    M = x.shape[0]
    rc = N.lib().dgppo_ln_relu_bwd(_p(x), _p(y), _p(stats), _p(gamma), _p(dy), _p(dx), _p(dgamma), _p(dbeta), M,
                                   N.stream_ptr())
    N.check(rc, "dgppo_ln_relu_bwd")


def gru_fwd(gi, Wh, bhn, h0, hs, hprev, gates, n_seq, T, n_inner):
    rows = n_seq * T
    N.expect_shape(gi, (rows, 192), "gi")
    N.expect_shape(hs, (rows, 64), "hs")
    N.expect_shape(Wh, (64, 192), "Wh")
    if h0 is not None:
        N.expect_shape(h0, (n_seq, 64), "h0")
    FLOPS[0] += 2.0 * rows * 64 * 192
    rc = N.lib().dgppo_gru_fwd(_p(gi), _p(Wh), _p(bhn), _p(h0), _p(hs), _p(hprev), _p(gates), n_seq, T, n_inner,
                               N.stream_ptr())
    N.check(rc, "dgppo_gru_fwd")


def gru_bwd(dhs, Wh, hprev, gates, dgi, dgh, n_seq, T, n_inner):
    rows = n_seq * T
    N.expect_shape(dhs, (rows, 64), "dhs")
    N.expect_shape(dgi, (rows, 192), "dgi")
    N.expect_shape(dgh, (rows, 192), "dgh")
    FLOPS[0] += 2.0 * rows * 64 * 192
    rc = N.lib().dgppo_gru_bwd(_p(dhs), _p(Wh), _p(hprev), _p(gates), _p(dgi), _p(dgh), n_seq, T, n_inner, N.stream_ptr())
    N.check(rc, "dgppo_gru_bwd")


def policy_head(ms, eps, action_in, action, log_pi, entropy, n_agents, mode, log_pi_old=None, adv=None, dms=None,
                stats=None, clip_eps=0.25, coef_ent=0.01):
    rows = ms.shape[0]
    N.expect_shape(ms, (rows, 4), "ms")
    rc = N.lib().dgppo_policy_head(_p(ms), _p(eps), _p(action_in), _p(action), _p(log_pi), _p(entropy), rows, n_agents,
                                   mode, _p(log_pi_old), _p(adv), _p(dms), _p(stats), C.c_float(clip_eps),
                                   C.c_float(coef_ent), N.stream_ptr())
    N.check(rc, "dgppo_policy_head")


def value_loss(v, target, dv, stats):
    rc = N.lib().dgppo_value_loss(_p(v), _p(target), _p(dv), _p(stats), v.numel(), N.stream_ptr())
    N.check(rc, "dgppo_value_loss")


def mean_agents(x, y, G, n, D, backward=False, relu_mask=None):
    rc = N.lib().dgppo_mean_agents(_p(x), _p(y), G, n, D, int(backward), _p(relu_mask), N.stream_ptr())
    N.check(rc, "dgppo_mean_agents")


def relu_bwd(dy, y):
    rc = N.lib().dgppo_relu_bwd(_p(dy), _p(y), C.c_int64(dy.numel()), N.stream_ptr())
    N.check(rc, "dgppo_relu_bwd")


def lstm_fwd(zi, Wh, bh, c0, h0, cs, hs, cprev, hprev, gates, n_seq, T, n_inner):
    rows = n_seq * T
    N.expect_shape(zi, (rows, 256), "zi"); N.expect_shape(Wh, (64, 256), "Wh"); N.expect_shape(bh, (256,), "bh")
    N.expect_shape(cs, (rows, 64), "cs"); N.expect_shape(hs, (rows, 64), "hs")
    for t, nm in ((c0, "c0"), (h0, "h0")):
        if t is not None:
            N.expect_shape(t, (n_seq, 64), nm)
    FLOPS[0] += 2.0 * rows * 64 * 256
    rc = N.lib().dgppo_lstm_fwd(_p(zi), _p(Wh), _p(bh), _p(c0), _p(h0), _p(cs), _p(hs), _p(cprev), _p(hprev), _p(gates),
                                n_seq, T, n_inner, N.stream_ptr())
    N.check(rc, "dgppo_lstm_fwd")


def lstm_bwd(dhs, Wh, cprev, gates, dz, n_seq, T, n_inner):
    rows = n_seq * T
    N.expect_shape(dhs, (rows, 64), "dhs"); N.expect_shape(dz, (rows, 256), "dz")
    FLOPS[0] += 2.0 * rows * 64 * 256
    rc = N.lib().dgppo_lstm_bwd(_p(dhs), _p(Wh), _p(cprev), _p(gates), _p(dz), n_seq, T, n_inner, N.stream_ptr())
    N.check(rc, "dgppo_lstm_bwd")
```

include/dgppo_hip.h:

```cpp
#ifndef DGPPO_HIP_H
#define DGPPO_HIP_H

#include <stdint.h>

#ifdef __cplusplus
extern "C" {
#endif

#define DGPPO_ABI_VERSION 3

enum {
  DGPPO_ENV_LIDAR_SPREAD = 0,
  DGPPO_ENV_LIDAR_TARGET = 1,
  DGPPO_ENV_LIDAR_BICYCLE_TARGET = 2,
  DGPPO_ENV_MPE_SPREAD = 3,
  DGPPO_ENV_MPE_TARGET = 4,
  DGPPO_ENV_LIDAR_LINE = 5,
  DGPPO_ENV_MPE_LINE = 6,
  DGPPO_ENV_MPE_FORMATION = 7,
  DGPPO_ENV_MPE_CORRIDOR = 8,
  DGPPO_ENV_MPE_CONNECT_SPREAD = 9
};
enum {
  DGPPO_GOALS_NODES = 0,
  DGPPO_GOALS_LINE = 1,
  DGPPO_GOALS_LINE_INTERIOR = 2,
  DGPPO_GOALS_CIRCLE = 3
};

#define DGPPO_RECT_STRIDE 16

typedef struct dgppo_env_cfg {
  int32_t kind;
  int32_t n_agents;
  int32_t n_goals;
  int32_t n_obs;
  int32_t n_rays;
  int32_t top_k;
  int32_t state_dim;
  int32_t node_dim;
  float area_size;
  float dt;
  float car_radius;
  float comm_radius;
  float obs_radius;
  float dist2goal;
  float two_car_radius;
  float lidar_mask_radius;
  float eye_offset;
  float car_plus_obs;
  float vel_limit;
  float reset_min_dist;
  int32_t reward_goals;
  int32_t n_cost;
  float obs_mask_radius;
  float y_limit;
  float connect_radius;
  float reset_side_y;
  float goal_shift_y;
  float line_min_dist;
} dgppo_env_cfg;

typedef struct dgppo_graph_out {
  float*   nodes;
  float*   edges;
  float*   states;
  int32_t* receivers;
  int32_t* senders;
  int32_t* node_type;
  int32_t* n_node;
  int32_t* n_edge;
} dgppo_graph_out;

int32_t     dgppo_abi_version(void);
const char* dgppo_last_error(void);

int32_t dgppo_env_num_nodes(const dgppo_env_cfg* cfg);
int32_t dgppo_env_num_edges(const dgppo_env_cfg* cfg);


int32_t dgppo_env_step(const dgppo_env_cfg* cfg,
                       const float* agent, const float* action, const float* goal,
                       const float* obst, const float* hits,
                       const float* ray_cos, const float* ray_sin,
                       float* next_agent, float* next_hits, float* reward, float* cost,
                       const dgppo_graph_out* gout, int32_t B, void* stream);

int32_t dgppo_graph_materialize(const dgppo_env_cfg* cfg,
                                const float* agent, const float* goal,
                                const float* obst, const float* hits,
                                const dgppo_graph_out* gout, int32_t B, void* stream);

int32_t dgppo_env_reset(const dgppo_env_cfg* cfg, const uint64_t* seeds,
                        float* agent, float* goal, float* obst, int32_t B, void* stream);
int32_t dgppo_env_reset_checked(const dgppo_env_cfg* cfg, const uint64_t* seeds, float* agent, float* goal, float* obst,
                                int32_t* n_failed, int32_t B, void* stream);

int32_t dgppo_randn(uint64_t seed, uint64_t offset, float* out, int64_t n_elem, void* stream);
int32_t dgppo_randn_rows(uint64_t seed, float* out, int64_t rows, int64_t row_len, int64_t global_row_len,
                         int64_t col_offset, void* stream);


int32_t dgppo_dense_fwd(const float* X, int32_t ldx, const float* W, int32_t ldw, const float* bias, float* Y,
                        int32_t ldy, int32_t M, int32_t K, int32_t N, int32_t act, int32_t accumulate,
                        int32_t trans_w, const float* relu_mask, int32_t ldm, void* stream);
int32_t dgppo_dense_bwd_w(const float* X, int32_t ldx, const float* dY, int32_t ldy, float* dW, int32_t ldw,
                          float* db, int32_t M, int32_t K, int32_t N, float* workspace, int64_t workspace_bytes,
                          void* stream);
int32_t dgppo_mlp_gi_fwd(const float* X, int32_t ldx, const float* W1, const float* b1, const float* g1, const float* be1,
                         const float* W2, const float* b2, const float* g2, const float* be2, const float* Wi,
                         const float* bi, float* p1, float* y1, float* st1, float* p2, float* y2, float* st2, float* gi,
                         int32_t M, void* stream);
int32_t dgppo_mlp_gi_bwd(const float* dgi, const float* Wi, const float* W2, const float* W1, const float* g2,
                         const float* g1, const float* p2, const float* y2, const float* st2, const float* p1,
                         const float* y1, const float* st1, const float* relu_mask, int32_t ldm, float* dpre2, float* dpre1,
                         float* dx, int32_t lddx, float* dg2, float* db2, float* dg1, float* db1, int32_t M, void* stream);
#define DGPPO_REDUCE_BATCH 16
typedef struct dgppo_reduce_desc {
  const float* part;
  float* dW;
  float* db;
  int32_t part_stride, slabs, ldw, K, N;
  int32_t pending;
} dgppo_reduce_desc;
int32_t dgppo_dense_bwd_w_deferred(const float* X, int32_t ldx, const float* dY, int32_t ldy, float* dW, int32_t ldw,
                                   float* db, int32_t M, int32_t K, int32_t N, float* workspace, int64_t workspace_bytes,
                                   dgppo_reduce_desc* pending, void* stream);
int32_t dgppo_dense_bwd_w_reduce_batch(const dgppo_reduce_desc* descs, int32_t n, void* stream);
int32_t dgppo_gru1_head_fwd(const float* gi, const float* Wh, const float* bhn, const float* h0, const float* W1,
                            const float* b1, const float* W2, const float* b2, float* hs, float* hprev, float* gates,
                            float* u, float* out, int32_t M, int32_t n_out, void* stream);
int64_t dgppo_dense_bwd_w_workspace_bytes(int32_t K, int32_t N);

int32_t dgppo_graph_feats(const dgppo_env_cfg* cfg, const float* agent, int64_t agent_se, int64_t agent_st,
                          const float* goal, const float* obst, const float* hits, int64_t hits_se, int64_t hits_st,
                          const int32_t* env_ids, int32_t n_env, int32_t n_time, float* Xa, float* Xo, float* efeat,
                          float* emask, int32_t Fp, void* stream);

int32_t dgppo_attn_fwd(const dgppo_env_cfg* cfg, int32_t F, int32_t H, int32_t Kp, const float* qt, const float* Xa,
                       const float* Xo, const float* efeat, const float* emask, float* zcat, float* attn, int32_t G,
                       void* stream);
int32_t dgppo_attn_bwd(const dgppo_env_cfg* cfg, int32_t F, int32_t H, int32_t Kp, const float* dzcat,
                       const float* attn, const float* qt, const float* Xa, const float* Xo, const float* efeat,
                       float* dqt, float* dXa, float* dXo, int32_t relu_xo, int32_t G, void* stream);
int32_t dgppo_attn_xo_supported(const dgppo_env_cfg* cfg, int32_t F, int32_t H, int32_t Kp);
int32_t dgppo_attn_fwd_xo(const dgppo_env_cfg* cfg, int32_t F, int32_t H, int32_t Kp, const float* qt, const float* Xa,
                          const float* Xo_raw, const float* Wo, int32_t ldwo, const float* bo, const float* efeat,
                          const float* emask, float* zcat, float* attn, int32_t G, void* stream);
int32_t dgppo_attn_bwd_xo(const dgppo_env_cfg* cfg, int32_t F, int32_t H, int32_t Kp, const float* dzcat,
                          const float* attn, const float* qt, const float* Xa, const float* Xo_raw, const float* Wo,
                          int32_t ldwo, const float* bo, const float* efeat, float* dqt, float* dXa, float* dXo,
                          int32_t relu_xo, int32_t G, void* stream);
int64_t dgppo_attn_xo_workspace_bytes(int32_t G);
int32_t dgppo_attn_bwd_xo_dw(const dgppo_env_cfg* cfg, int32_t F, int32_t H, int32_t Kp, const float* dzcat,
                             const float* attn, const float* qt, const float* Xa, const float* Xo_raw, const float* Wo,
                             int32_t ldwo, const float* bo, const float* efeat, float* dqt, float* dXa, float* dWo,
                             int32_t lddwo, float* dbo, float* workspace, int64_t workspace_bytes, int32_t G, void* stream);

int32_t dgppo_gnn_prep(const float* Wq, const float* bq, const float* Wk, const float* Wv, const float* bv,
                       const float* We, const float* Wu, float* Mcat, float* cvec, float* Wout, int32_t F, int32_t Fp,
                       int32_t D, int32_t H, int32_t Kp, void* stream);
int32_t dgppo_gnn_unprep(const float* dMcat, const float* dcvec, const float* dWout, const float* Wq, const float* bq,
                         const float* Wk, float* dWq, float* dbq, float* dWk, float* dWv, float* dbv, float* dWe,
                         float* dWu, int32_t F, int32_t Fp, int32_t D, int32_t H, int32_t Kp, void* stream);

int32_t dgppo_ln_relu_fwd(const float* x, const float* gamma, const float* beta, float* y, float* stats, int32_t M,
                          void* stream);
int32_t dgppo_ln_relu_bwd(const float* x, const float* y, const float* stats, const float* gamma, const float* dy,
                          float* dx, float* dgamma, float* dbeta, int32_t M, void* stream);

int32_t dgppo_gru_fwd(const float* gi, const float* Wh, const float* bhn, const float* h0, float* hs, float* hprev,
                      float* gates, int32_t n_seq, int32_t T, int32_t n_inner, void* stream);
int32_t dgppo_gru_bwd(const float* dhs, const float* Wh, const float* hprev, const float* gates, float* dgi,
                      float* dgh, int32_t n_seq, int32_t T, int32_t n_inner, void* stream);

int32_t dgppo_lstm_fwd(const float* zi, const float* Wh, const float* bh, const float* c0, const float* h0, float* cs,
                       float* hs, float* cprev, float* hprev, float* gates, int32_t n_seq, int32_t T, int32_t n_inner,
                       void* stream);
int32_t dgppo_lstm_bwd(const float* dhs, const float* Wh, const float* cprev, const float* gates, float* dz,
                       int32_t n_seq, int32_t T, int32_t n_inner, void* stream);

int32_t dgppo_policy_head(const float* ms, const float* eps, const float* action_in, float* action, float* log_pi,
                          float* entropy, int32_t rows, int32_t n_agents, int32_t mode, const float* log_pi_old,
                          const float* adv, float* dms, float* stats, float clip_eps, float coef_ent, void* stream);

int32_t dgppo_value_loss(const float* v, const float* target, float* dv, float* stats, int32_t count, void* stream);
int32_t dgppo_mean_agents(const float* x, float* y, int32_t G, int32_t n, int32_t D, int32_t backward,
                          const float* relu_mask, void* stream);
int32_t dgppo_relu_bwd(float* dy, const float* y, int64_t count, void* stream);


int32_t dgppo_gae(const float* costs, const float* rewards, const float* Vh, const float* Vl, const float* lam_pow,
                  float gamma, float one_minus_gamma, float one_minus_lam, float* Qh, float* Ql, int32_t B, int32_t T,
                  int32_t n, int32_t nh, void* stream);
int32_t dgppo_advantage(const float* Ql, const float* Vl, const float* Vh, float dt, float alpha, float cbf_eps,
                        float cbf_weight, float* adv, float* stats, int32_t B, int32_t T, int32_t n, int32_t nh,
                        void* stream);
int32_t dgppo_advantage_lagr(const float* Ql, const float* Vl, const float* Qh, const float* Vh, const float* lagr,
                             float* adv, float* Ah, int32_t B, int32_t T, int32_t n, int32_t nh, void* stream);
int32_t dgppo_lagr_update(const float* lp_new, const float* lp_old, const float* Vh, int64_t vh_env_stride,
                          const float* Ah, float* lagr, float* sums, int32_t n_env, int32_t T, int32_t n, int32_t nh,
                          float one_minus_gamma, float lr, void* stream);
int32_t dgppo_lagr_sums(const float* lp_new, const float* lp_old, const float* Vh, int64_t vh_env_stride, const float* Ah,
                        float* sums, int32_t n_env, int32_t T, int32_t n, int32_t nh, float one_minus_gamma, void* stream);
int32_t dgppo_lagr_apply(float* lagr, float* sums, int32_t count, int64_t rows_total, float lr, void* stream);
int32_t dgppo_relu_fwd(const float* x, float* out, int64_t count, void* stream);
int32_t dgppo_shaped_reward(const float* reward, const float* cost, float cost_weight, float* out, int64_t rows,
                            int32_t n, int32_t nh, void* stream);
#define DGPPO_OPT_PARTIALS 256
#define DGPPO_OPT_STATE_FLOATS (8 + 2 * DGPPO_OPT_PARTIALS)
int32_t dgppo_clip_adam_step(float* params, const float* grads, float* m, float* v, int64_t n, float* state, float lr,
                             float b1, float b2, float eps, float max_norm, float grad_scale, void* stream);

#define DGPPO_COMM_ID_BYTES 128
int32_t dgppo_comm_unique_id(uint8_t* id_out);
int32_t dgppo_comm_version(int32_t* version_out);
int32_t dgppo_comm_init(const uint8_t* id, int32_t rank, int32_t world, void** comm_out);
int32_t dgppo_comm_allreduce_sum_f32(void* comm, float* buf, int64_t count, void* stream);
int32_t dgppo_comm_destroy(void* comm);

#ifdef __cplusplus
}
#endif
#endif
```

Before: 4.037 million.

## Fuse graph feature construction into slot8 attention kernels via raw state records

Adds a record path where the slot8 attention forward and backward kernels rebuild node features, edge features and masks directly from raw agent, goal and LiDAR hit buffers. This avoids materializing and re-reading the Xa/Xo/efeat/emask tensors for first-layer attention. The aim is to cut global memory traffic and possibly the graph_feats kernel launch. The cost is recomputing the features inside both kernels, plus extra register pressure and template variants.

```diff
diff --git a/dgppo_amd/csrc/nn_graph.hip b/dgppo_amd/csrc/nn_graph.hip
--- a/dgppo_amd/csrc/nn_graph.hip
+++ b/dgppo_amd/csrc/nn_graph.hip
@@ -50,6 +50,27 @@
 };
 
 __device__ inline float dist_rn(float dx, float dy) { return __fsqrt_rn(__fadd_rn(__fmul_rn(dx, dx), __fmul_rn(dy, dy))); }
+
+enum NodeKind { NODE_OBS = 0, NODE_GOAL = 1, NODE_AGENT = 2 };
+template <int SD> __device__ inline float node_col(const float* s, int kind, int col) {
+  return (col < SD) ? s[col] : ((col == SD + kind) ? 1.0f : 0.0f);
+}
+template <int SD> __device__ inline float4 edge_node_feat(const float* s) {
+  if constexpr (SD == 5) return make_float4(s[0], s[1], __fmul_rn(s[4], s[2]), __fmul_rn(s[4], s[3]));
+  else return make_float4(s[0], s[1], s[2], s[3]);
+}
+__device__ inline float4 edge_sub(const float4& fi, const float4& fj) {
+  return make_float4(__fsub_rn(fi.x, fj.x), __fsub_rn(fi.y, fj.y), __fsub_rn(fi.z, fj.z), __fsub_rn(fi.w, fj.w));
+}
+__device__ inline bool edge_agent_mask(const dgppo_env_cfg& c, float px, float py, float qx, float qy, bool self) {
+  return __fadd_rn(dist_rn(__fsub_rn(px, qx), __fsub_rn(py, qy)), self ? c.eye_offset : 0.0f) < c.comm_radius;
+}
+__device__ inline float4 edge_hit_feat(float px, float py, float hx, float hy) {
+  return make_float4(__fsub_rn(px, hx), __fsub_rn(py, hy), 0.0f, 0.0f);
+}
+__device__ inline bool edge_hit_mask(const dgppo_env_cfg& c, const float4& f) { return dist_rn(f.x, f.y) < c.lidar_mask_radius; }
+
+__device__ inline float4 ld4_lds(const float* p) { return make_float4(p[0], p[1], p[2], p[3]); }
 
 template <int SD>
 __global__ void graph_feats_kernel(FeatArgs a) {
@@ -89,21 +110,16 @@
   for (int i = tid; i < n + ng; i += nt) {
     const float* s = (i < n) ? s_ag + i * SD : s_go + (i - n) * SD;
     float* f = (i < n) ? s_fa + i * 4 : s_fg + (i - n) * 4;
-    if constexpr (SD == 5) {
-      f[0] = s[0]; f[1] = s[1]; f[2] = __fmul_rn(s[4], s[2]); f[3] = __fmul_rn(s[4], s[3]);
-    } else {
-      f[0] = s[0]; f[1] = s[1]; f[2] = s[2]; f[3] = s[3];
-    }
+    const float4 v = edge_node_feat<SD>(s);
+    f[0] = v.x; f[1] = v.y; f[2] = v.z; f[3] = v.w;
   }
   __syncthreads();
-  constexpr int ND = SD + 3;
   for (int idx = tid; idx < t.Ns * Fp; idx += nt) {
     const int nd = (int)__umulhi((uint32_t)idx, a.rcp_fp), col = idx - nd * Fp;
-    float v = 0.0f;
-    if (nd < n) v = (col < SD) ? s_ag[nd * SD + col] : ((col == SD + 2) ? 1.0f : 0.0f);
-    else if (nd < n + ng) v = (col < SD) ? s_go[(nd - n) * SD + col] : ((col == SD + 1) ? 1.0f : 0.0f);
-    else v = (col < SD) ? s_ob[(nd - n - ng) * SD + col] : ((col == SD) ? 1.0f : 0.0f);
-    if (col >= ND) v = 0.0f;
+    float v;
+    if (nd < n) v = node_col<SD>(s_ag + nd * SD, NODE_AGENT, col);
+    else if (nd < n + ng) v = node_col<SD>(s_go + (nd - n) * SD, NODE_GOAL, col);
+    else v = node_col<SD>(s_ob + (nd - n - ng) * SD, NODE_OBS, col);
     if (nd < n) a.Xa[((size_t)g * n + nd) * Fp + col] = v;
     else a.Xo[((size_t)g * (t.Ns - n) + (nd - n)) * Fp + col] = v;
   }
@@ -111,25 +127,21 @@
     const int i = (int)__umulhi((uint32_t)idx, a.rcp_S), s = idx - i * S;
     float4 f;
     bool mask;
-    const float* fi = s_fa + i * 4;
+    const float4 fi = ld4_lds(s_fa + i * 4);
     const float px = s_ag[i * SD], py = s_ag[i * SD + 1];
     if (s < n) {
-      const float* fj = s_fa + s * 4;
-      f = make_float4(__fsub_rn(fi[0], fj[0]), __fsub_rn(fi[1], fj[1]), __fsub_rn(fi[2], fj[2]), __fsub_rn(fi[3], fj[3]));
-      float d = __fadd_rn(dist_rn(__fsub_rn(px, s_ag[s * SD]), __fsub_rn(py, s_ag[s * SD + 1])), (i == s) ? c.eye_offset : 0.0f);
-      mask = d < c.comm_radius;
+      f = edge_sub(fi, ld4_lds(s_fa + s * 4));
+      mask = edge_agent_mask(c, px, py, s_ag[s * SD], s_ag[s * SD + 1], i == s);
     } else if (s < n + t.gs) {
       const int gi = t.spread ? (s - n) : i;
-      const float* fg = s_fg + gi * 4;
-      f = make_float4(__fsub_rn(fi[0], fg[0]), __fsub_rn(fi[1], fg[1]), __fsub_rn(fi[2], fg[2]), __fsub_rn(fi[3], fg[3]));
+      f = edge_sub(fi, ld4_lds(s_fg + gi * 4));
       mask = true;
     } else {
       const int m = s - n - t.gs;
       if (t.lidar) {
         const float* hp = s_ob + (i * t.per + m) * SD;
-        const float lx = __fsub_rn(px, hp[0]), ly = __fsub_rn(py, hp[1]);
-        f = make_float4(lx, ly, 0.0f, 0.0f);
-        mask = dist_rn(lx, ly) < c.lidar_mask_radius;
+        f = edge_hit_feat(px, py, hp[0], hp[1]);
+        mask = edge_hit_mask(c, f);
       } else {
         const float* xo = s_ob + m * SD;
         const float* xi = s_ag + i * SD;
@@ -195,6 +207,8 @@
   int G;
   const float* Xo_raw; const float* Wo; const float* bo; int ldwo;
   float* dwo_slab;
+  dgppo_graph_rec rec;
+  dgppo_env_cfg cfg;
 };
 
 __global__ void __launch_bounds__(256) attn_fwd_valu_kernel(AttnArgs a) {
@@ -579,7 +593,65 @@
   return v;
 }
 
-template <int H, int NPA, int SJ>
+struct RecBase { const float* ag; const float* go; const float* hp; };
+template <int SD> __device__ inline RecBase rec_base(const AttnArgs& a, int g) {
+  const dgppo_graph_rec& r = a.rec;
+  const int e = g / r.n_time, tt = g - e * r.n_time;
+  const int env = r.env_ids ? r.env_ids[e] : e;
+  return {r.agent + (size_t)env * r.agent_se + (size_t)tt * r.agent_st, r.goal + (size_t)env * a.t.ng * SD,
+          r.hits + (size_t)env * r.hits_se + (size_t)tt * r.hits_st};
+}
+template <int SD> __device__ inline void ld_state(const float* p, float (&v)[SD]) {
+  if constexpr (SD == 4) {
+    const float4 q = *reinterpret_cast<const float4*>(p);
+    v[0] = q.x; v[1] = q.y; v[2] = q.z; v[3] = q.w;
+  } else {
+#pragma unroll
+    for (int c = 0; c < SD; ++c) v[c] = p[c];
+  }
+}
+__device__ inline void opaque4(float4& v) { asm("" : "+v"(v.x), "+v"(v.y), "+v"(v.z), "+v"(v.w)); }
+template <int SD, int SJ>
+__device__ inline void rec_slot_rows(const AttnArgs& a, const RecBase& b, int i, int sub, float (&own)[SD],
+                                     float4 (&x)[SJ][2], float4 (&e)[SJ], float (&m)[SJ]) {
+  const Topo& t = a.t;
+  const int n = t.n, nn = t.n + t.ng, S = t.S;
+  float st[SJ][SD];
+  float2 hp[SJ];
+  int nd[SJ];
+  ld_state<SD>(b.ag + i * SD, own);
+#pragma unroll
+  for (int j = 0; j < SJ; ++j) {
+    int sl = sub + 8 * j;
+    sl = sl < S ? sl : S - 1;
+    nd[j] = sender_node(t, i, sl);
+    const float* ps = (nd[j] < n) ? b.ag + nd[j] * SD : ((nd[j] < nn) ? b.go + (nd[j] - n) * SD : b.ag + i * SD);
+    const int q = (nd[j] >= nn) ? nd[j] - nn : i * t.per;
+    ld_state<SD>(ps, st[j]);
+    hp[j] = *reinterpret_cast<const float2*>(b.hp + 2 * q);
+  }
+  float4 fi = edge_node_feat<SD>(own);
+  opaque4(fi);
+#pragma unroll
+  for (int j = 0; j < SJ; ++j) {
+    const bool isa = nd[j] < n, ish = nd[j] >= nn;
+    float sv[SD];
+#pragma unroll
+    for (int c = 0; c < SD; ++c) sv[c] = ish ? (c == 0 ? hp[j].x : (c == 1 ? hp[j].y : 0.0f)) : st[j][c];
+    const int kind = isa ? NODE_AGENT : (ish ? NODE_OBS : NODE_GOAL);
+    x[j][0] = make_float4(node_col<SD>(sv, kind, 0), node_col<SD>(sv, kind, 1), node_col<SD>(sv, kind, 2), node_col<SD>(sv, kind, 3));
+    x[j][1] = make_float4(node_col<SD>(sv, kind, 4), node_col<SD>(sv, kind, 5), node_col<SD>(sv, kind, 6), node_col<SD>(sv, kind, 7));
+    const float4 eh = edge_hit_feat(own[0], own[1], hp[j].x, hp[j].y);
+    float4 fj = edge_node_feat<SD>(st[j]);
+    opaque4(fj);
+    e[j] = ish ? eh : edge_sub(fi, fj);
+    const bool mk = ish ? edge_hit_mask(a.cfg, eh) : (isa ? edge_agent_mask(a.cfg, own[0], own[1], st[j][0], st[j][1], nd[j] == i) : true);
+    m[j] = mk ? 1.0f : 0.0f;
+    opaque4(x[j][0]); opaque4(x[j][1]); opaque4(e[j]);
+  }
+}
+
+template <int H, int NPA, int SJ, int RSD>
 __global__ void __launch_bounds__(256) attn_fwd_slot8_kernel(AttnArgs a) {
   constexpr int F = 8, Wd = F + 4;
   const Topo& t = a.t;
@@ -594,8 +666,11 @@
   const float* mk = a.emask + (size_t)g * n * S;
   float* zc = a.zcat + (size_t)g * n * Kp;
   float* at = a.attn + (size_t)g * n * S * H;
-  for (int idx = lane; idx < n * 2; idx += 64)
-    *reinterpret_cast<float4*>(zc + (idx >> 1) * Kp + 4 * (idx & 1)) = reinterpret_cast<const float4*>(Xa)[idx];
+  RecBase rb{};
+  if constexpr (RSD > 0) rb = rec_base<RSD>(a, g);
+  if constexpr (RSD == 0)
+    for (int idx = lane; idx < n * 2; idx += 64)
+      *reinterpret_cast<float4*>(zc + (idx >> 1) * Kp + 4 * (idx & 1)) = reinterpret_cast<const float4*>(Xa)[idx];
   for (int i = lane; i < n; i += 64)
     for (int c = kc; c < Kp; ++c) zc[i * Kp + c] = (c == kc) ? 1.0f : 0.0f;
 #pragma unroll
@@ -610,15 +685,26 @@
       const float4* qp = reinterpret_cast<const float4*>(qt + (i * H + h) * F);
       q[h][0] = qp[0]; q[h][1] = qp[1];
     }
-#pragma unroll
-    for (int j = 0; j < SJ; ++j) {
-      int sl = sub + 8 * j;
-      sl = sl < S ? sl : S - 1;
-      const int nd = sender_node(t, i, sl);
-      const float4* xp = reinterpret_cast<const float4*>((nd < n ? Xa : Xo) + (size_t)nd * F);
-      x[j][0] = xp[0]; x[j][1] = xp[1];
-      e[j] = reinterpret_cast<const float4*>(ef)[i * S + sl];
-      m[j] = mk[i * S + sl];
+    if constexpr (RSD > 0) {
+      float own[RSD];
+      rec_slot_rows<RSD, SJ>(a, rb, i, sub, own, x, e, m);
+      if (live && sub < 2) {
+        const int c0 = 4 * sub;
+        *reinterpret_cast<float4*>(zc + i * Kp + c0) =
+            make_float4(node_col<RSD>(own, NODE_AGENT, c0), node_col<RSD>(own, NODE_AGENT, c0 + 1),
+                        node_col<RSD>(own, NODE_AGENT, c0 + 2), node_col<RSD>(own, NODE_AGENT, c0 + 3));
+      }
+    } else {
+#pragma unroll
+      for (int j = 0; j < SJ; ++j) {
+        int sl = sub + 8 * j;
+        sl = sl < S ? sl : S - 1;
+        const int nd = sender_node(t, i, sl);
+        const float4* xp = reinterpret_cast<const float4*>((nd < n ? Xa : Xo) + (size_t)nd * F);
+        x[j][0] = xp[0]; x[j][1] = xp[1];
+        e[j] = reinterpret_cast<const float4*>(ef)[i * S + sl];
+        m[j] = mk[i * S + sl];
+      }
     }
     float av[SJ][H];
 #pragma unroll
@@ -681,7 +767,7 @@
   }
 }
 
-template <int H, int NPA, int SJ>
+template <int H, int NPA, int SJ, int RSD>
 __global__ void __launch_bounds__(256) attn_bwd_slot8_kernel(AttnArgs a) {
   constexpr int F = 8, Wd = F + 4;
   const Topo& t = a.t;
@@ -695,6 +781,8 @@
   const float* at = a.attn + (size_t)g * n * S * H;
   const float* dzc = a.dzcat + (size_t)g * n * Kp;
   float* dq = a.dqt + (size_t)g * n * H * F;
+  RecBase rb{};
+  if constexpr (RSD > 0) rb = rec_base<RSD>(a, g);
 #pragma unroll
   for (int p = 0; p < NPA; ++p) {
     const int ia = grp + 8 * p;
@@ -707,15 +795,21 @@
       const float4* zp = reinterpret_cast<const float4*>(dzc + i * Kp + F + h * Wd);
       dz[h][0] = zp[0]; dz[h][1] = zp[1]; dz[h][2] = zp[2];
     }
+    if constexpr (RSD > 0) {
+      float own[RSD], m[SJ];
+      rec_slot_rows<RSD, SJ>(a, rb, i, sub, own, x, e, m);
+    }
 #pragma unroll
     for (int j = 0; j < SJ; ++j) {
       int sl = sub + 8 * j;
       const bool in = live && sl < S;
       sl = sl < S ? sl : S - 1;
-      const int nd = sender_node(t, i, sl);
-      const float4* xp = reinterpret_cast<const float4*>((nd < n ? Xa : Xo) + (size_t)nd * F);
-      x[j][0] = xp[0]; x[j][1] = xp[1];
-      e[j] = reinterpret_cast<const float4*>(ef)[i * S + sl];
+      if constexpr (RSD == 0) {
+        const int nd = sender_node(t, i, sl);
+        const float4* xp = reinterpret_cast<const float4*>((nd < n ? Xa : Xo) + (size_t)nd * F);
+        x[j][0] = xp[0]; x[j][1] = xp[1];
+        e[j] = reinterpret_cast<const float4*>(ef)[i * S + sl];
+      }
 #pragma unroll
       for (int h = 0; h < H; ++h) {
         const float w = at[(i * S + sl) * H + h];
@@ -763,12 +857,12 @@
   }
 }
 
-template <int H, int NPA>
+template <int H, int NPA, int RSD>
 static bool launch_attn_slot8_sj(const AttnArgs& a, int SJ, int grid, hipStream_t s, bool bwd) {
 #define DGPPO_SJ(J)                                                                                              \
   case J:                                                                                                        \
-    if (bwd) hipLaunchKernelGGL((attn_bwd_slot8_kernel<H, NPA, J>), dim3(grid), dim3(256), 0, s, a);             \
-    else hipLaunchKernelGGL((attn_fwd_slot8_kernel<H, NPA, J>), dim3(grid), dim3(256), 0, s, a);                 \
+    if (bwd) hipLaunchKernelGGL((attn_bwd_slot8_kernel<H, NPA, J, RSD>), dim3(grid), dim3(256), 0, s, a);        \
+    else hipLaunchKernelGGL((attn_fwd_slot8_kernel<H, NPA, J, RSD>), dim3(grid), dim3(256), 0, s, a);            \
     return true;
   switch (SJ) {
     DGPPO_SJ(1) DGPPO_SJ(2) DGPPO_SJ(3) DGPPO_SJ(4) DGPPO_SJ(5) DGPPO_SJ(6) DGPPO_SJ(7) DGPPO_SJ(8)
@@ -777,14 +871,23 @@
 #undef DGPPO_SJ
 }
 static bool attn_slot8_shape(const Topo& t, int F, int H) { return F == 8 && H == 3 && t.n <= 32 && t.S <= 64; }
-static bool launch_attn_slot8(const AttnArgs& a, hipStream_t s, bool bwd) {
-  if (!attn_slot8_shape(a.t, a.F, a.H)) return false;
+template <int RSD>
+static bool launch_attn_slot8_rsd(const AttnArgs& a, hipStream_t s, bool bwd) {
   const int grid = (a.G + 3) / 4, NPA = (a.t.n + 7) / 8, SJ = (a.t.S + 7) / 8;
   switch (NPA) {
-    case 1: return launch_attn_slot8_sj<3, 1>(a, SJ, grid, s, bwd);
-    case 2: return launch_attn_slot8_sj<3, 2>(a, SJ, grid, s, bwd);
-    case 3: return launch_attn_slot8_sj<3, 3>(a, SJ, grid, s, bwd);
-    case 4: return launch_attn_slot8_sj<3, 4>(a, SJ, grid, s, bwd);
+    case 1: return launch_attn_slot8_sj<3, 1, RSD>(a, SJ, grid, s, bwd);
+    case 2: return launch_attn_slot8_sj<3, 2, RSD>(a, SJ, grid, s, bwd);
+    case 3: return launch_attn_slot8_sj<3, 3, RSD>(a, SJ, grid, s, bwd);
+    case 4: return launch_attn_slot8_sj<3, 4, RSD>(a, SJ, grid, s, bwd);
+    default: return false;
+  }
+}
+static bool launch_attn_slot8(const AttnArgs& a, hipStream_t s, bool bwd, int rsd = 0) {
+  if (!attn_slot8_shape(a.t, a.F, a.H)) return false;
+  switch (rsd) {
+    case 0: return launch_attn_slot8_rsd<0>(a, s, bwd);
+    case 4: return launch_attn_slot8_rsd<4>(a, s, bwd);
+    case 5: return launch_attn_slot8_rsd<5>(a, s, bwd);
     default: return false;
   }
 }
@@ -1974,6 +2077,55 @@
   return 0;
 }
 
+static bool attn_rec_ok(const dgppo_env_cfg& c, const Topo& t, int F, int H, int Kp) {
+  return t.lidar && t.os > 0 && (c.state_dim == 4 || c.state_dim == 5) && c.node_dim == c.state_dim + 3 &&
+         attn_family(t, F, H, Kp, false, false) == AttnFamily::SLOT8;
+}
+extern "C" int32_t dgppo_attn_rec_supported(const dgppo_env_cfg* cfg, int32_t F, int32_t H, int32_t Kp) {
+  if (dgppo_validate_cfg(cfg)) return 0;
+  return attn_rec_ok(*cfg, make_topo(*cfg), F, H, Kp) ? 1 : 0;
+}
+static int32_t attn_rec_check(const dgppo_env_cfg* cfg, int F, int H, int Kp, int G, const dgppo_graph_rec* rec, AttnArgs& a) {
+  int32_t rc = attn_check(cfg, F, H, Kp, G, a);
+  if (rc) return rc;
+  DGPPO_REQUIRE(attn_rec_ok(*cfg, a.t, F, H, Kp), "attn_rec: topology / shape not supported (dgppo_attn_rec_supported)");
+  DGPPO_REQUIRE(rec && rec->agent && rec->goal && rec->hits, "attn_rec: NULL record operand");
+  DGPPO_REQUIRE(rec->n_time >= 1 && G % rec->n_time == 0, "attn_rec: G=%d is not a multiple of n_time=%d", G, rec->n_time);
+  const int SD = cfg->state_dim;
+  const bool a16 = SD != 4 || ((((uintptr_t)rec->agent | (uintptr_t)rec->goal) & 15) == 0 && ((rec->agent_se | rec->agent_st) & 3) == 0);
+  DGPPO_REQUIRE(a16, "attn_rec: agent / goal rows must be 16-byte aligned");
+  DGPPO_REQUIRE(((uintptr_t)rec->hits & 7) == 0 && ((rec->hits_se | rec->hits_st) & 1) == 0, "attn_rec: hit points must be 8-byte aligned");
+  a.rec = *rec; a.cfg = *cfg;
+  return 0;
+}
+
+extern "C" int32_t dgppo_attn_fwd_rec(const dgppo_env_cfg* cfg, int32_t F, int32_t H, int32_t Kp, const float* qt,
+                                      const dgppo_graph_rec* rec, float* zcat, float* attn, int32_t G, void* stream) {
+  AttnArgs a{};
+  int32_t rc = attn_rec_check(cfg, F, H, Kp, G, rec, a);
+  if (rc) return rc;
+  if (G == 0) return 0;
+  DGPPO_REQUIRE(qt && zcat, "attn_fwd_rec: NULL operand");
+  a.qt = qt; a.zcat = zcat; a.attn = attn;
+  DGPPO_REQUIRE(launch_attn_slot8(a, (hipStream_t)stream, false, cfg->state_dim), "attn_fwd_rec: dispatch failed");
+  DGPPO_LAUNCH_CHECK();
+  return 0;
+}
+
+extern "C" int32_t dgppo_attn_bwd_rec(const dgppo_env_cfg* cfg, int32_t F, int32_t H, int32_t Kp, const float* dzcat,
+                                      const float* attn, const float* qt, const dgppo_graph_rec* rec, float* dqt, int32_t G,
+                                      void* stream) {
+  AttnArgs a{};
+  int32_t rc = attn_rec_check(cfg, F, H, Kp, G, rec, a);
+  if (rc) return rc;
+  if (G == 0) return 0;
+  DGPPO_REQUIRE(dzcat && attn && qt && dqt, "attn_bwd_rec: NULL operand");
+  a.dzcat = dzcat; a.attn = (float*)attn; a.qt = qt; a.dqt = dqt;
+  DGPPO_REQUIRE(launch_attn_slot8(a, (hipStream_t)stream, true, cfg->state_dim), "attn_bwd_rec: dispatch failed");
+  DGPPO_LAUNCH_CHECK();
+  return 0;
+}
+
 static bool attn_xo_ok(const Topo& t, int F, int H, int Kp) {
   return t.Ns > t.n && attn_family(t, F, H, Kp, true, true) == AttnFamily::BD;
 }
diff --git a/dgppo_amd/nets.py b/dgppo_amd/nets.py
--- a/dgppo_amd/nets.py
+++ b/dgppo_amd/nets.py
@@ -95,8 +95,10 @@
 
 class GraphFeats:
 
-    def __init__(self, cfg: N.EnvCfg, G: int, arena: Arena, tag: str):
+    def __init__(self, cfg: N.EnvCfg, G: int, arena: Arena, tag: str, materialised: bool = False):
         self.cfg, self.G = cfg, G
+        self.materialised = materialised
+        self.rec, self._rec_refs = None, None
         n, S = cfg.n_agents, cfg.fan_in
         self.n_other = cfg.num_nodes - 1 - n
         self.Fp = 8
@@ -109,6 +111,9 @@
         assert n_env * n_time == self.G
         K.graph_feats(self.cfg, agent, agent_se, agent_st, goal, obst, hits, hits_se, hits_st, env_ids, n_env, n_time,
                       self.Xa, self.Xo if self.n_other > 0 else None, self.efeat, self.emask, self.Fp)
+        if not self.materialised and self.cfg.is_lidar and hits is not None:
+            self.rec = K.graph_rec(self.cfg, agent, agent_se, agent_st, goal, hits, hits_se, hits_st, env_ids, n_env, n_time)
+            self._rec_refs = (agent, goal, hits, env_ids)
         return self
 
 
@@ -170,6 +175,14 @@
             K.gnn_prep(q("Wq"), q("bq"), q("Wk"), q("Wv"), q("bv"), q("We"), q("Wu"), self.pp(f"gnn{l}.Mcat"),
                        self.pp(f"gnn{l}.cvec"), self.pp(f"gnn{l}.Wout"), f, fp, d, H_HEADS, kp)
 
+    def _rec_ok(self, feats: GraphFeats, l: int) -> bool:
+        if l != 0 or feats.rec is None:
+            return False
+        if not hasattr(self, "_rec_sup"):
+            f0, fp0, d0, kp0 = self.dims[0]
+            self._rec_sup = K.attn_rec_supported(self.cfg, fp0, H_HEADS, kp0)
+        return self._rec_sup
+
     def _xo_fusable(self, l: int) -> bool:
         if l != 0 or self.gnn_layers != 2:
             return False
@@ -197,7 +210,9 @@
             K.dense_fwd(Xa, self.pp(f"gnn{l}.Mcat"), self.pp(f"gnn{l}.cvec"), qt)
             zcat = A.get(f"{tag}.zcat{l}", R, kp)
             attn = A.get(f"{tag}.attn{l}", R, cfg.fan_in, H_HEADS) if train else None
-            if xo_fused is not None:
+            if self._rec_ok(feats, l):
+                K.attn_fwd_rec(cfg, fp, H_HEADS, kp, qt, feats.rec, zcat, attn, G)
+            elif xo_fused is not None:
                 K.attn_fwd_xo(cfg, fp, H_HEADS, kp, qt, Xa, xo_fused[0], xo_fused[1], xo_fused[2], feats.efeat, feats.emask, zcat, attn, G)
             else:
                 K.attn_fwd(cfg, fp, H_HEADS, kp, qt, Xa, Xo if Ro > 0 else None, feats.efeat, feats.emask, zcat, attn, G)
@@ -460,7 +475,9 @@
             dXo_l = A.get(f"{tag}.dXo{l}", Ro, fp) if (need_dx and Ro > 0) else None
             more_dXo = dXo_prev is not None and dXo_l is not None
             xf = act.get(f"xo_fused{l}")
-            if xf is not None and dXa_l is not None and not more_dXo:
+            if dXa_l is None and dXo_l is None and self._rec_ok(feats, l):
+                K.attn_bwd_rec(cfg, fp, H_HEADS, kp, dz, act[f"attn{l}"], act[f"qt{l}"], feats.rec, dqt, G)
+            elif xf is not None and dXa_l is not None and not more_dXo:
                 ws = A.get(f"{tag}.xo_ws", K.attn_xo_workspace_floats(G), 1).view(-1)
                 K.attn_bwd_xo_dw(cfg, fp, H_HEADS, kp, dz, act[f"attn{l}"], act[f"qt{l}"], act[f"Xa{l}"], xf[0], xf[1], xf[2],
                                  feats.efeat, dqt, dXa_l, self.pg(f"gnn{l - 1}.Wout")[:self.dims[l - 1][1]], self.g(f"gnn{l - 1}.bu"), ws, G)
diff --git a/dgppo_amd/ops_nn.py b/dgppo_amd/ops_nn.py
--- a/dgppo_amd/ops_nn.py
+++ b/dgppo_amd/ops_nn.py
@@ -200,6 +200,26 @@
     N.check(rc, "dgppo_dense_bwd_w")
 
 
+def _check_records(what, cfg, agent, agent_se, agent_st, hits, hits_se, hits_st, env_ids, n_env, n_time):
+    n = cfg.n_agents
+    for name, t_, se, st, inner in (("agent", agent, agent_se, agent_st, (n, cfg.state_dim)),
+                                    ("hits", hits, hits_se, hits_st, (n, cfg.top_k, 2))):
+        if t_ is None:
+            continue
+        if not (t_.is_cuda and t_.dtype == torch.float32):
+            raise ValueError(f"{what}: {name} must be a float32 CUDA tensor")
+        want, acc = [], 1
+        for d in reversed(inner):
+            want.append(acc)
+            acc *= d
+        if tuple(t_.shape[-len(inner):]) != tuple(inner) or list(t_.stride()[-len(inner):]) != want[::-1]:
+            raise ValueError(f"{what}: the trailing {inner} block of {name} must be dense (got shape {tuple(t_.shape)}, "
+                             f"strides {t_.stride()})")
+        avail = t_.untyped_storage().nbytes() // 4 - t_.storage_offset()
+        if env_ids is None and (n_env - 1) * se + (n_time - 1) * st + acc > avail:
+            raise ValueError(f"{what}: {name}: the strides reach beyond its storage")
+
+
 def graph_feats(cfg: N.EnvCfg, agent, agent_se, agent_st, goal, obst, hits, hits_se, hits_st, env_ids, n_env, n_time,
                 Xa, Xo, efeat, emask, Fp):
     G = n_env * n_time
@@ -210,22 +230,7 @@
         N.expect_shape(Xo, (G * n_other, Fp), "Xo")
     N.expect_shape(efeat, (G * n, S, 4), "efeat")
     N.expect_shape(emask, (G * n, S), "emask")
-    for name, t_, se, st, inner in (("agent", agent, agent_se, agent_st, (n, cfg.state_dim)),
-                                    ("hits", hits, hits_se, hits_st, (n, cfg.top_k, 2))):
-        if t_ is None:
-            continue
-        if not (t_.is_cuda and t_.dtype == torch.float32):
-            raise ValueError(f"graph_feats: {name} must be a float32 CUDA tensor")
-        want, acc = [], 1
-        for d in reversed(inner):
-            want.append(acc)
-            acc *= d
-        if tuple(t_.shape[-len(inner):]) != tuple(inner) or list(t_.stride()[-len(inner):]) != want[::-1]:
-            raise ValueError(f"graph_feats: the trailing {inner} block of {name} must be dense (got shape {tuple(t_.shape)}, "
-                             f"strides {t_.stride()})")
-        avail = t_.untyped_storage().nbytes() // 4 - t_.storage_offset()
-        if env_ids is None and (n_env - 1) * se + (n_time - 1) * st + acc > avail:
-            raise ValueError(f"graph_feats: {name}: the strides reach beyond its storage")
+    _check_records("graph_feats", cfg, agent, agent_se, agent_st, hits, hits_se, hits_st, env_ids, n_env, n_time)
     rc = N.lib().dgppo_graph_feats(
         C.byref(cfg), C.c_void_p(agent.data_ptr()), C.c_int64(agent_se), C.c_int64(agent_st), _p(goal, "goal"),
         _p(obst, "obst") if (obst is not None and not cfg.is_lidar) else C.c_void_p(0),
@@ -258,6 +263,45 @@
     rc = N.lib().dgppo_attn_bwd(C.byref(cfg), F, H, Kp, _p(dzcat), _p(attn), _p(qt), _p(Xa), _p(Xo), _p(efeat), _p(dqt),
                                 _p(dXa), _p(dXo), int(relu_xo), G, N.stream_ptr())
     N.check(rc, "dgppo_attn_bwd")
+
+
+class GraphRec(C.Structure):
+    _fields_ = [("agent", C.c_void_p), ("agent_se", C.c_int64), ("agent_st", C.c_int64), ("goal", C.c_void_p),
+                ("hits", C.c_void_p), ("hits_se", C.c_int64), ("hits_st", C.c_int64), ("env_ids", C.c_void_p),
+                ("n_time", C.c_int32)]
+
+
+def graph_rec(cfg: N.EnvCfg, agent, agent_se, agent_st, goal, hits, hits_se, hits_st, env_ids, n_env, n_time) -> GraphRec:
+    _check_records("graph_rec", cfg, agent, agent_se, agent_st, hits, hits_se, hits_st, env_ids, n_env, n_time)
+    if hits is None:
+        raise ValueError("graph_rec: the record path needs LiDAR hit points")
+    return GraphRec(agent.data_ptr(), agent_se, agent_st, _p(goal, "goal").value, hits.data_ptr(), hits_se, hits_st,
+                    _p(env_ids, "env_ids", torch.int32).value, n_time)
+
+
+def attn_rec_supported(cfg, F, H, Kp) -> bool:
+    return bool(N.lib().dgppo_attn_rec_supported(C.byref(cfg), F, H, Kp))
+
+
+def attn_fwd_rec(cfg, F, H, Kp, qt, rec: GraphRec, zcat, attn, G):
+    n, S = cfg.n_agents, cfg.fan_in
+    N.expect_shape(qt, (G * n, H * F), "qt")
+    N.expect_shape(zcat, (G * n, Kp), "zcat")
+    if attn is not None:
+        N.expect_shape(attn, (G * n, S, H), "attn")
+    FLOPS[0] += 2.0 * G * n * H * S * (2 * F + 4)
+    rc = N.lib().dgppo_attn_fwd_rec(C.byref(cfg), F, H, Kp, _p(qt), C.byref(rec), _p(zcat), _p(attn), G, N.stream_ptr())
+    N.check(rc, "dgppo_attn_fwd_rec")
+
+
+def attn_bwd_rec(cfg, F, H, Kp, dzcat, attn, qt, rec: GraphRec, dqt, G):
+    n = cfg.n_agents
+    N.expect_shape(dzcat, (G * n, Kp), "dzcat")
+    N.expect_shape(dqt, (G * n, H * F), "dqt")
+    FLOPS[0] += 4.0 * G * n * H * cfg.fan_in * (2 * F + 4)
+    rc = N.lib().dgppo_attn_bwd_rec(C.byref(cfg), F, H, Kp, _p(dzcat), _p(attn), _p(qt), C.byref(rec), _p(dqt), G,
+                                    N.stream_ptr())
+    N.check(rc, "dgppo_attn_bwd_rec")
 
 
 def attn_xo_supported(cfg, F, H, Kp) -> bool:
diff --git a/include/dgppo_hip.h b/include/dgppo_hip.h
--- a/include/dgppo_hip.h
+++ b/include/dgppo_hip.h
@@ -137,12 +137,29 @@
                           const int32_t* env_ids, int32_t n_env, int32_t n_time, float* Xa, float* Xo, float* efeat,
                           float* emask, int32_t Fp, void* stream);
 
+typedef struct dgppo_graph_rec {
+  const float* agent;
+  int64_t agent_se, agent_st;
+  const float* goal;
+  const float* hits;
+  int64_t hits_se, hits_st;
+  const int32_t* env_ids;
+  int32_t n_time;
+} dgppo_graph_rec;
+
 int32_t dgppo_attn_fwd(const dgppo_env_cfg* cfg, int32_t F, int32_t H, int32_t Kp, const float* qt, const float* Xa,
                        const float* Xo, const float* efeat, const float* emask, float* zcat, float* attn, int32_t G,
                        void* stream);
 int32_t dgppo_attn_bwd(const dgppo_env_cfg* cfg, int32_t F, int32_t H, int32_t Kp, const float* dzcat,
                        const float* attn, const float* qt, const float* Xa, const float* Xo, const float* efeat,
                        float* dqt, float* dXa, float* dXo, int32_t relu_xo, int32_t G, void* stream);
+int32_t dgppo_attn_rec_supported(const dgppo_env_cfg* cfg, int32_t F, int32_t H, int32_t Kp);
+int32_t dgppo_attn_fwd_rec(const dgppo_env_cfg* cfg, int32_t F, int32_t H, int32_t Kp, const float* qt,
+                           const dgppo_graph_rec* rec, float* zcat, float* attn, int32_t G, void* stream);
+int32_t dgppo_attn_bwd_rec(const dgppo_env_cfg* cfg, int32_t F, int32_t H, int32_t Kp, const float* dzcat,
+                           const float* attn, const float* qt, const dgppo_graph_rec* rec, float* dqt, int32_t G,
+                           void* stream);
+
 int32_t dgppo_attn_xo_supported(const dgppo_env_cfg* cfg, int32_t F, int32_t H, int32_t Kp);
 int32_t dgppo_attn_fwd_xo(const dgppo_env_cfg* cfg, int32_t F, int32_t H, int32_t Kp, const float* qt, const float* Xa,
                           const float* Xo_raw, const float* Wo, int32_t ldwo, const float* bo, const float* efeat,
```

Result: faster. 4.148 million, median of 6 (+2.8%).
